# kiwicampus/multicamera_stitching

Hardware: AMD Instinct MI355X
Metric: stitched MPix/sec (4-cam 1080p rig) (higher is better)
Workload: dtype u8; 1 GPU; C2 rig: 4 x 1920x1080 BGR cameras, precomputed homographies, linear warpPerspective + 3-level multi-band blend (SURVEY.md 8 NS-1); blend=multiband, super_mode=False

## Files before the change

### multicamera_stitching_amd/_capi.py

```python
from __future__ import annotations

import ctypes
import os
import threading

import numpy as np

_HERE = os.path.dirname(os.path.abspath(__file__))
LIB_PATH = os.environ.get("MCS_LIBRARY", os.path.join(_HERE, "libmcs.so"))

MCS_OK = 0
MCS_E_INVALID = -1
MCS_E_HIP = -2
MCS_E_NOMEM = -3
MCS_E_SHAPE = -4
MCS_E_UNSUPPORTED = -5
MCS_INTER_NEAREST = 0
MCS_INTER_LINEAR = 1
MCS_BLEND_NONE = 0
MCS_BLEND_FEATHER = 1
MCS_BLEND_MULTIBAND = 2
MCS_BLEND_SEAM = 3
MCS_SEAM_DISTANCE = 0
MCS_SEAM_GRAPHCUT = 1
# ... 380 lines not shown

    @classmethod
    def warp(cls, M, src_w: int, src_h: int, dst_w: int, dst_h: int, channels: int,
             interp: int = MCS_INTER_LINEAR, device: int = 0):
        L = load()
        m = np.ascontiguousarray(np.asarray(M, np.float64).reshape(9))
        h = ctypes.c_void_p()
        check(L.mcs_plan_create_warp(m.ctypes.data_as(ctypes.c_void_p), int(src_w), int(src_h),
                                     int(dst_w), int(dst_h), int(channels), int(interp),
                                     int(device), ctypes.byref(h)))
        return cls(None, 0, 0, channels, interp, device, _handle=h)

    @classmethod
    def undistort(cls, K, dist, w: int, h: int, channels: int, device: int = 0):
        L = load()
        k = np.ascontiguousarray(np.asarray(K, np.float64).reshape(9))
        d = np.ascontiguousarray(np.asarray(dist if dist is not None else [], np.float64)
                                 .reshape(-1))
        hd = ctypes.c_void_p()
        check(L.mcs_plan_create_undistort(k.ctypes.data_as(ctypes.c_void_p),
                                          d.ctypes.data_as(ctypes.c_void_p) if d.size else None,
                                          int(d.size), int(w), int(h), int(channels),
                                          int(device), ctypes.byref(hd)))
        return cls(None, 0, 0, channels, MCS_INTER_LINEAR, device, _handle=hd)

    @property
    def handle(self):
        return self._h

    def close(self):
        if getattr(self, "_h", None) is not None and self._h.value:
            self._lib.mcs_plan_destroy(self._h)
            self._h = None

    def __del__(self):
        try:
            self.close()
        except Exception:
            pass

    def out_shape(self):
        if self.channels == 1:
            return (self.out_h, self.out_w)
        return (self.out_h, self.out_w, self.channels)

    def describe(self) -> dict:
        fd = self.flat
        n = fd.n_stages
        return {
            "n_stages": n,
            "out_w": fd.out_w, "out_h": fd.out_h, "channels": fd.channels,
            "off_x": [fd.st[j].off_x for j in range(n)] + [fd.cam0_off_x],
            "off_y": [fd.st[j].off_y for j in range(n)] + [fd.cam0_off_y],
            "rect": [list(fd.st[j].rect) for j in range(n)],
            "minv": [list(fd.st[j].minv) for j in range(n)],
            "bw0": [fd.st[j].bw0 for j in range(n)],
            "cam": [fd.st[j].cam for j in range(n)],
            "cam_w": [fd.cam_w[i] for i in range(fd.n_cams)],
            "cam_h": [fd.cam_h[i] for i in range(fd.n_cams)],
        }

    def stitch_host(self, cams, sizes=None) -> np.ndarray:
        cams = [np.ascontiguousarray(c, dtype=np.uint8) for c in cams]
        out = np.empty(self.out_shape(), np.uint8)
        ptrs = (ctypes.c_void_p * len(cams))(*[c.ctypes.data for c in cams])
        outp = out.ctypes.data_as(ctypes.c_void_p)
        fd = self.flat
        if sizes is None or all((w, h) == (fd.cam_w[i], fd.cam_h[i])
                                for i, (w, h) in enumerate(sizes)):
            check(self._lib.mcs_stitch_host(self._h, ptrs, outp))
        else:
            ws = (ctypes.c_int * len(sizes))(*[int(w) for w, _ in sizes])
            hs = (ctypes.c_int * len(sizes))(*[int(h) for _, h in sizes])
            check(self._lib.mcs_stitch_host_sized(self._h, ptrs, ws, hs, outp))
        return out

    def find_seams(self, cams=None, method: int = MCS_SEAM_GRAPHCUT, scale_log2: int = 2):
        if cams is None:
            check(self._lib.mcs_plan_find_seams(self._h, None, int(method), int(scale_log2)))
            return
        cams = [np.ascontiguousarray(c, dtype=np.uint8) for c in cams]
        ptrs = (ctypes.c_void_p * len(cams))(*[c.ctypes.data for c in cams])
        check(self._lib.mcs_plan_find_seams(self._h, ptrs, int(method), int(scale_log2)))

    def seam_labels(self):
        w, h = ctypes.c_int(), ctypes.c_int()
        check(self._lib.mcs_plan_seam_labels(self._h, None, ctypes.byref(w), ctypes.byref(h)))
        if w.value == 0:
            return None
        out = np.empty((h.value, w.value), np.uint8)
        check(self._lib.mcs_plan_seam_labels(self._h, out.ctypes.data_as(ctypes.c_void_p),
                                             ctypes.byref(w), ctypes.byref(h)))
        return out

    def seam_stats(self):
        st = np.zeros(5, np.int64)
        check(self._lib.mcs_plan_seam_stats(self._h, st.ctypes.data_as(ctypes.c_void_p)))
        return tuple(int(v) for v in st)

    def stitch_device(self, cam_ptrs, cam_frame_strides, out_ptr: int, out_pitch: int,
                      out_frame_stride: int, n_frames: int, stream: int = 0):
        n = len(cam_ptrs)
        ptrs = (ctypes.c_void_p * n)(*[int(p) for p in cam_ptrs])
        strides = (ctypes.c_int64 * n)(*[int(s) for s in cam_frame_strides])
        check(self._lib.mcs_stitch_device(self._h, ptrs, strides, ctypes.c_void_p(int(out_ptr)),
                                          int(out_pitch), int(out_frame_stride), int(n_frames),
                                          ctypes.c_void_p(int(stream))))

    def stitch_direct(self, cam_ptrs, cam_frame_strides, out_ptr: int, out_pitch: int,
                      out_frame_stride: int, n_frames: int, stream: int = 0):
        n = len(cam_ptrs)
        ptrs = (ctypes.c_void_p * n)(*[int(p) for p in cam_ptrs])
        strides = (ctypes.c_int64 * n)(*[int(s) for s in cam_frame_strides])
        check(self._lib.mcs_stitch_direct(self._h, ptrs, strides, ctypes.c_void_p(int(out_ptr)),
                                          int(out_pitch), int(out_frame_stride), int(n_frames),
                                          ctypes.c_void_p(int(stream))))

    def stitch_device_gained(self, cam_ptrs, cam_frame_strides, out_ptr: int, out_pitch: int,
                             out_frame_stride: int, n_frames: int, stream: int = 0):
        n = len(cam_ptrs)
        ptrs = (ctypes.c_void_p * n)(*[int(p) for p in cam_ptrs])
        strides = (ctypes.c_int64 * n)(*[int(s) for s in cam_frame_strides])
        check(self._lib.mcs_stitch_device_gained(
            self._h, ptrs, strides, ctypes.c_void_p(int(out_ptr)), int(out_pitch),
            int(out_frame_stride), int(n_frames), ctypes.c_void_p(int(stream))))

    def stitch_direct_gained(self, cam_ptrs, cam_frame_strides, out_ptr: int, out_pitch: int,
                             out_frame_stride: int, n_frames: int, stream: int = 0):
        n = len(cam_ptrs)
        ptrs = (ctypes.c_void_p * n)(*[int(p) for p in cam_ptrs])
        strides = (ctypes.c_int64 * n)(*[int(s) for s in cam_frame_strides])
        check(self._lib.mcs_stitch_direct_gained(
            self._h, ptrs, strides, ctypes.c_void_p(int(out_ptr)), int(out_pitch),
            int(out_frame_stride), int(n_frames), ctypes.c_void_p(int(stream))))

    def prepare(self, stream: int = 0):
        check(self._lib.mcs_plan_prepare(self._h, ctypes.c_void_p(int(stream))))

    def tile_tables(self):
        n = self._lib.mcs__plan_tile_tables(self._h, None, None, None, 0)
        if n < 0:
            check(n)
        tiles = (TileHdr * max(n, 1))()
        spans = np.zeros((n, TILE_MAX_JOBS), np.uint16)
        desc = np.zeros((n, TILE_W * TILE_H, TILE_DESC_WORDS), np.uint32)
        if n:
            rc = self._lib.mcs__plan_tile_tables(self._h, ctypes.byref(tiles), spans.ctypes.data,
                                                 desc.ctypes.data, n)
            if rc < 0:
                check(rc)
        return tiles, spans, desc

    def stats(self) -> dict:
        arr = (ctypes.c_int64 * 21)()
        check(self._lib.mcs_plan_stats(self._h, arr, 21))
        return {"prepared": bool(arr[0]), "tiles": arr[1], "lds_tiles": arr[2],
                "direct_tiles": arr[3], "table_bytes": arr[4], "blend": arr[5],
                "blend_tiles": arr[6], "mb_owners": arr[7], "mb_degraded_tiles": arr[8],
                "mb_bands": arr[9], "mb_bands_lds": arr[10], "big_tiles": arr[11],
                "mb_mixed_px": arr[12], "mb_r1_entries": arr[13],
                "dma_bytes_per_capture": arr[14], "box_bytes_per_capture": arr[15],
                "mb_sweep_strips": arr[16], "mb_sweep_px": arr[17],
                "mb_sweep_threads": arr[18], "mb_sweep_desc_rows": arr[19],
                "lens_cams": arr[20]}

    def set_blend(self, mode: int):
        check(self._lib.mcs_plan_set_blend(self._h, int(mode)))
        return self

    def set_lens(self, cam: int, K, dist=None):
        if K is None:
            check(self._lib.mcs_plan_set_lens(self._h, int(cam), None, None, 0))
            return self
        k, d = _lens_args(K, dist)
        check(self._lib.mcs_plan_set_lens(self._h, int(cam), k.ctypes.data_as(ctypes.c_void_p),
                                          d.ctypes.data_as(ctypes.c_void_p) if d.size else None,
                                          int(d.size)))
        return self

    def overlap_stats(self, cam_ptrs, cam_frame_strides, n_frames: int, step_log2: int = 2,
                      stream: int = 0):
        n = self.n_cams
        ptrs = (ctypes.c_void_p * n)(*[int(p) if p else None for p in cam_ptrs])
        strides = (ctypes.c_int64 * n)(*[int(s) for s in cam_frame_strides])
        N = np.zeros((n, n), np.int64)
        S = np.zeros((max(int(n_frames), 0), n, n), np.int64)
        check(self._lib.mcs_plan_overlap_stats(self._h, ptrs, strides, int(n_frames),
                                               int(step_log2), N.ctypes.data, S.ctypes.data,
                                               ctypes.c_void_p(int(stream))))
        return N, S

    def overlap_stats_host(self, cams, step_log2: int = 2):
        cams = [np.ascontiguousarray(c, dtype=np.uint8) for c in cams]
        ptrs = (ctypes.c_void_p * len(cams))(*[c.ctypes.data for c in cams])
        n = self.n_cams
        N = np.zeros((n, n), np.int64)
        S = np.zeros((n, n), np.int64)
        check(self._lib.mcs_plan_overlap_stats_host(self._h, ptrs, int(step_log2), N.ctypes.data,
                                                    S.ctypes.data))
        return N, S

    def set_gains(self, gains):
        if gains is None:
            check(self._lib.mcs_plan_set_gains(self._h, None))
            return self
        g = np.ascontiguousarray(np.asarray(gains, np.float64).reshape(-1))
        if g.size != self.n_cams:
            raise ValueError(f"{g.size} gains for a plan of {self.n_cams} cameras")
        check(self._lib.mcs_plan_set_gains(self._h, g.ctypes.data))
        return self

    def gains(self):
        q = np.zeros(self.n_cams, np.uint16)
        on = ctypes.c_int(0)
        check(self._lib.mcs_plan_gains(self._h, q.ctypes.data, ctypes.byref(on)))
        return q, bool(on.value)

    def footprint(self):
        arr = (ctypes.c_int64 * MCS_MAX_CAMS)()
        check(self._lib.mcs_plan_footprint(self._h, arr, MCS_MAX_CAMS))
        return [int(arr[i]) for i in range(self.n_cams)]


def resize_linear_device(src_ptr: int, src_w: int, src_h: int, dst_ptr: int, dst_w: int,
                         dst_h: int, channels: int, n_frames: int = 1, src_pitch: int = 0,
                         dst_pitch: int = 0, src_frame_stride: int = 0,
                         dst_frame_stride: int = 0, device: int = 0, stream: int = 0):
    L = load()
    check(L.mcs_resize_linear_device(
        src_ptr, src_w, src_h, src_pitch or src_w * channels, src_frame_stride, dst_ptr, dst_w,
        dst_h, dst_pitch or dst_w * channels, dst_frame_stride, channels, n_frames, device,
        stream or None))


def gain_solve(N, S, channels: int, alpha: float = 0.01, beta: float = 100.0) -> np.ndarray:
    N = np.ascontiguousarray(N, dtype=np.int64)
    S = np.ascontiguousarray(S, dtype=np.int64)
    n = N.shape[0]
    if N.shape != (n, n) or S.shape != (n, n):
        raise ValueError(f"N {N.shape} and S {S.shape} must both be (n_cams, n_cams)")
    g = np.ones(n, np.float64)
    check(load().mcs_gain_solve_host(n, N.ctypes.data, S.ctypes.data, int(channels),
                                     float(alpha), float(beta), g.ctypes.data))
    return g


def gain_apply_device(src_ptr: int, dst_ptr: int, nbytes: int, q: int, n_frames: int = 1,
                      src_frame_stride: int = 0, dst_frame_stride: int = 0, device: int = 0,
                      stream: int = 0):
    if not 0 <= int(q) <= 65535:
        raise ValueError(f"q {q} outside 0..65535")
    check(load().mcs_gain_apply_device(src_ptr, dst_ptr, int(nbytes), int(src_frame_stride),
                                       int(dst_frame_stride), int(n_frames), int(q), int(device),
                                       stream or None))


def match_hamming_knn2(query, train, device: int = 0):
    L = load()
    q = np.ascontiguousarray(query, dtype=np.uint8).reshape(-1, 32)
    t = np.ascontiguousarray(train, dtype=np.uint8).reshape(-1, 32)
    idx = np.empty((q.shape[0], 2), np.int32)
    dist = np.empty((q.shape[0], 2), np.int32)
    check(L.mcs_match_hamming_knn2_host(q.ctypes.data, q.shape[0], t.ctypes.data, t.shape[0],
                                        idx.ctypes.data, dist.ctypes.data, device))
    return idx, dist


def match_hamming_knn2_device(q_ptr: int, nq: int, t_ptr: int, nt: int, idx_ptr: int,
                              dist_ptr: int, device: int = 0, stream: int = 0):
    check(load().mcs_match_hamming_knn2(q_ptr, nq, t_ptr, nt, idx_ptr, dist_ptr, device,
                                        stream or None))


def homography_refine(src, dst, mask, H):
    L = load()
    src = np.ascontiguousarray(src, np.float32).reshape(-1, 2)
    dst = np.ascontiguousarray(dst, np.float32).reshape(-1, 2)
    m = np.ascontiguousarray(np.asarray(mask).reshape(-1), np.uint8)
    h = np.ascontiguousarray(np.asarray(H, np.float64).reshape(9)).copy()
    check(L.mcs_homography_refine_host(src.ctypes.data, dst.ctypes.data, src.shape[0],
                                       m.ctypes.data, h.ctypes.data))
    return h.reshape(3, 3)


def ransac_homography(src, dst, thresh: float, iters: int = 2000, seed: int = 0,
                      device: int = 0):
    L = load()
    src = np.ascontiguousarray(src, np.float32).reshape(-1, 2)
    dst = np.ascontiguousarray(dst, np.float32).reshape(-1, 2)
    n = src.shape[0]
    H = np.zeros(9, np.float64)
    mask = np.zeros(n, np.uint8)
    ninl = ctypes.c_int(0)
    check(L.mcs_ransac_homography_host(src.ctypes.data, dst.ctypes.data, n, float(thresh),
                                       int(iters), int(seed) & 0xffffffff, H.ctypes.data,
                                       mask.ctypes.data, ctypes.byref(ninl), device))
    return (H.reshape(3, 3) if ninl.value > 0 else None), mask.reshape(-1, 1)


class StreamPipeline:

    def __init__(self, plan: "Plan", depth: int = 3, use_graphs: bool = True):
        self._lib = load()
        self.plan = plan
        self.depth = depth
        h = ctypes.c_void_p()
        check(self._lib.mcs_stream_create(plan._h, depth, 1 if use_graphs else 0,
                                          ctypes.byref(h)))
        self._h = h

    def _check_frames(self, cams):
        C = self.plan.channels
        if len(cams) != self.plan.n_cams:
            raise ValueError(f"{len(cams)} frames for a plan of {self.plan.n_cams} cameras")
        out = []
        for i, (c, (h, w)) in enumerate(zip(cams, self.plan.cam_shapes)):
            c = np.asarray(c)
# ... 354 lines not shown
```

### multicamera_stitching_amd/build.py

```python
from __future__ import annotations

import hashlib
import os
import struct
import subprocess
import sys

HERE = os.path.dirname(os.path.abspath(__file__))
ROOT = os.path.dirname(HERE)
CSRC = os.path.join(HERE, "csrc")
LIB = os.path.join(HERE, "libmcs.so")
ARCH = os.environ.get("MCS_OFFLOAD_ARCH", "gfx950")
DEVICE = {"stitch": "mcs_kernels.hip", "features": "mcs_features.hip", "sweep": "mcs_sweep.hip"}
HSACO = os.path.join(HERE, f"mcs_kernels.{ARCH}.hsaco")
ROCM = os.environ.get("ROCM_PATH", "/opt/rocm")
HIPCC = os.environ.get("HIPCC", os.path.join(ROCM, "bin", "hipcc"))
CXX = os.environ.get("CXX", "g++")
HOST_SRC = ["mcs_plan.cpp", "hip_rt.cpp", "mcs_runtime.cpp", "mcs_capi.cpp", "mcs_prepare.cpp",
            "mcs_sweep_host.cpp", "mcs_launch.cpp", "mcs_features.cpp", "mcs_stream.cpp",
            "mcs_seam.cpp", "mcs_refine.cpp", "mcs_group.cpp", "mcs_rig.cpp", "mcs_chain.cpp",
            "mcs_gain.cpp"]
HEADERS = ["mcs_kparams.h", "mcs_dev.h", "mcs_fparams.h", "mcs_common.h", "hip_rt.h", "mcs_blend.h",
           "mcs_gain.h", "mcs_ransac_core.h",
           "mcs_orb_core.h", "mcs_orb_pattern.h", "mcs_feat_int.h", "mcs_lens_core.h",
           "mcs_plan_state.h"]
INC = ["-I" + os.path.join(ROOT, "include"), "-I" + CSRC]

DEVICE_FLAGS = [
    f"--offload-arch={ARCH}", "--offload-device-only", "--no-gpu-bundle-output",
    "-O3", "-std=c++17",
    "-ffp-contract=off", "-fno-fast-math", "-Wall",
    "-mllvm", "-instcombine-max-copied-from-constant-users=4096",
]
HOST_FLAGS = [
    "-O2", "-std=c++17", "-fPIC", "-shared", "-Wall", "-Wextra", "-Wno-unused-parameter",
    "-ffp-contract=off", "-fno-fast-math",
    "-D__HIP_PLATFORM_AMD__", "-I" + os.path.join(ROCM, "include"),
]


def _elf_sections(path: str) -> dict:
    with open(path, "rb") as f:
        b = f.read()
    if b[:4] != b"\x7fELF" or b[4] != 2 or b[5] != 1:
        raise ValueError(f"{path}: not an ELF64 little-endian object")
    shoff, = struct.unpack_from("<Q", b, 0x28)
    shentsize, shnum, shstrndx = struct.unpack_from("<HHH", b, 0x3A)
    hdrs = [struct.unpack_from("<IIQQQQIIQQ", b, shoff + i * shentsize) for i in range(shnum)]
    names = hdrs[shstrndx]
    strtab = b[names[4]:names[4] + names[5]]
    out = {}
    for h in hdrs:
        name = strtab[h[0]:strtab.index(b"\0", h[0])].decode()
        out[name] = b"" if h[1] == 8 else b[h[4]:h[4] + h[5]]
    return out


CODE_SECTIONS = (".text", ".rodata", ".note")


def code_id(paths) -> str:
    digest = hashlib.sha256()
    for p in paths:
        secs = _elf_sections(p)
        for name in CODE_SECTIONS:
            data = secs.get(name, b"")
            digest.update(name.encode() + struct.pack("<Q", len(data)) + data)
    return digest.hexdigest()[:16]


def _stale() -> bool:
    if not (os.path.exists(LIB) and os.path.exists(HSACO)):
        return True
    t = os.path.getmtime(LIB)
    deps = [os.path.join(CSRC, s) for s in [*DEVICE.values(), *HOST_SRC, *HEADERS]]
    deps += [os.path.join(ROOT, "include", "mcs.h"), __file__]
    return any(os.path.getmtime(d) > t for d in deps)


def _run(cmd, verbose):
    if verbose:
        print(" ".join(cmd), flush=True)
    subprocess.check_call(cmd)


def build(force: bool = False, verbose: bool = False, lib: str = None, defines=()) -> str:
    if lib is not None:
        return _build_to(lib, HSACO + "." + os.path.basename(lib), list(defines), verbose)
    if not force and not _stale():
        return LIB
    return _build_to(LIB, HSACO, [], verbose)


def _fresh(out: str, src: str) -> bool:
    if not os.path.exists(out):
        return False
    deps = [os.path.join(CSRC, src)] + [os.path.join(CSRC, h) for h in HEADERS]
    deps += [os.path.join(ROOT, "include", "mcs.h"), __file__]
    return all(os.path.getmtime(d) <= os.path.getmtime(out) for d in deps)


def _build_to(LIB: str, HSACO: str, defines, verbose: bool) -> str:
    objs = {}
    for name, src in DEVICE.items():
        out = HSACO if name == "stitch" else HSACO.replace("mcs_kernels", "mcs_" + name)
        if defines or not _fresh(out, src):
            _run([HIPCC, *DEVICE_FLAGS, *["-D" + d for d in defines], *INC, "-o", out + ".tmp",
                  os.path.join(CSRC, src)], verbose)
            os.replace(out + ".tmp", out)
        objs[name] = out
    build_id = code_id([objs[name] for name in sorted(objs)])
    blob = LIB + ".blob.S"
    with open(blob, "w") as f:
        f.write("    .section .rodata\n")
        for name, path in objs.items():
            f.write('    .balign 4096\n    .globl mcs_hsaco_%s_start\nmcs_hsaco_%s_start:\n'
                    '    .incbin "%s"\n    .byte 0\n' % (name, name, path))
        f.write('    .section .note.GNU-stack,"",@progbits\n')
    try:
        _run([CXX, *HOST_FLAGS, *["-D" + d for d in defines], f'-DMCS_BUILD_ID="{build_id}"',
              *INC, "-o", LIB + ".tmp",
              *[os.path.join(CSRC, s) for s in HOST_SRC], blob, "-ldl", "-lpthread"], verbose)
    finally:
        os.remove(blob)
    os.replace(LIB + ".tmp", LIB)
    return LIB


if __name__ == "__main__":
    print(build(force="--force" in sys.argv, verbose=True))
```

### multicamera_stitching_amd/csrc/mcs_blend.h

```cpp
#pragma once

namespace mcs {

template <int INTERP>
__device__ __forceinline__ void slot_xy(const KParams &P, int s, int x, int y, int &x32, int &y32,
                                        int &cam, int &w, int &h)
{
    int X, Y;
    if (s == 0) {
        cam = 0;
        w = P.cam0_w;
        h = P.cam0_h;
        if (!cam0_lensed(P)) {
            x32 = (x + P.cam0_offx) * 32;
            y32 = (y + P.cam0_offy) * 32;
            return;
        }
        cam0_lens_map<INTERP>(P, x, y, X, Y);
    } else {
        const KStage &S = P.st[s - 1];
        cam = S.cam;
        w = S.src_w;
        h = S.src_h;
        stage_map<INTERP>(P, S, x, y, X, Y);
// ... 73 lines not shown
    w = s == 0 ? P.cam0_w : P.st[s - 1].src_w;
    h = s == 0 ? P.cam0_h : P.st[s - 1].src_h;
}

__device__ __forceinline__ int refl(int i, int n)
{
    if (n == 1) return 0;
    while (i < 0 || i >= n) {
        if (i < 0) i = -i;
        if (i >= n) i = 2 * n - 2 - i;
    }
    return i;
}

template <int CN, int INTERP>
__device__ __forceinline__ void seam_sample(const KSeamArgs &a)
{
    const KParams &P = a.P;
    const int q = blockIdx.x * blockDim.x + threadIdx.x;
    if (q >= a.gw * a.gh) return;
    const int x = (q % a.gw) << a.k, y = (q / a.gw) << a.k;
    const int64_t np = (int64_t)a.gw * a.gh;
    const int o = blend_owner<INTERP>(P, x, y, nullptr);
    uint32_t cov = 0;
    for (int s = 0; s <= P.n_stages; s++) {
        int x32, y32, cam, w, h;
        slot_xy<INTERP>(P, s, x, y, x32, y32, cam, w, h);
        if (slot_dist(x32, y32, w, h) < 0) continue;
        cov |= 1u << cam;
        const uint8_t *fb = P.cams[cam];
        const uint32_t v = sample_replicate<CN>(fb, w, h, x32, y32);
        uint8_t *d = a.samples + ((int64_t)cam * np + q) * CN;
#pragma unroll
        for (int k = 0; k < CN; k++) d[k] = (uint8_t)(v >> (8 * k));
    }
    a.cov[q] = (uint16_t)cov;
    int ocam = kBlendNone;
    if (o != kBlendNone) {
        int c, w, h;
        slot_info(P, o, c, w, h);
        ocam = c;
    }
    a.label[q] = (uint8_t)ocam;
}

template <int INTERP>
__device__ __forceinline__ void blend_owner_tile(const KParams &P, uint8_t *owner_map,
                                                 uint32_t *info)
{
    __shared__ uint32_t s_own, s_feather;
    if (threadIdx.x == 0) s_own = s_feather = 0;
    __syncthreads();
    const int X0 = blockIdx.x * kBlendTileW, Y0 = blockIdx.y * kBlendTileH;
    uint32_t own = 0, fea = 0;
    for (int i = threadIdx.x; i < kMbTilePx; i += blockDim.x) {
        const int x = X0 + (i % kBlendTileW), y = Y0 + i / kBlendTileW;
        if (x >= P.out_w || y >= P.out_h) continue;
        uint32_t pm;
        const int o = blend_owner<INTERP>(P, x, y, &pm);
        owner_map[(int64_t)y * P.out_w + x] = (uint8_t)o;
        if (o != kBlendNone) own |= 1u << o;
        if (__popc(pm) >= 2) fea |= pm;
    }
    atomicOr(&s_own, own);
    atomicOr(&s_feather, fea);
    __syncthreads();
    if (threadIdx.x == 0) {
        const int t = blockIdx.y * gridDim.x + blockIdx.x;
        info[2 * t] = s_own;
        info[2 * t + 1] = s_feather;
    }
}

__device__ __forceinline__ void blend_classify(const KParams &P, int mode, const uint8_t *owner,
                                               const uint32_t *info, int *list, int *overflow,
                                               int *list2)
{
    __shared__ uint32_t s_mask;
    const int gx = (P.out_w + kBlendTileW - 1) / kBlendTileW;
    const int t = blockIdx.x, tx = t % gx, ty = t / gx;
    uint32_t mask;
    if (mode == MCS_BLEND_FEATHER) {
        mask = info[2 * t + 1];
    } else {
        if (threadIdx.x == 0) s_mask = 0;
        __syncthreads();
        const int x0 = max(tx * kBlendTileW - kBlendHalo, 0);
        const int x1 = min(tx * kBlendTileW + kBlendTileW + kBlendHalo, P.out_w);
        const int y0 = max(ty * kBlendTileH - kBlendHalo, 0);
        const int y1 = min(ty * kBlendTileH + kBlendTileH + kBlendHalo, P.out_h);
        const int rw = x1 - x0, n = rw * (y1 - y0);
        uint32_t m = 0;
        for (int i = threadIdx.x; i < n; i += blockDim.x) {
            const int o = owner[(int64_t)(y0 + i / rw) * P.out_w + x0 + i % rw];
            if (o != kBlendNone) m |= 1u << o;
        }
        atomicOr(&s_mask, m);
        __syncthreads();
        mask = s_mask;
        if (__popc(mask) < 2) mask = 0;
    }
    if (threadIdx.x == 0 && mode == MCS_BLEND_MULTIBAND && __popc(mask) > kBlendSlots) {
        atomicAdd(overflow, 1);
        const uint32_t fea = info[2 * t + 1];
        if (fea) {
            const int i = atomicAdd(&list2[0], 1);
            list2[1 + 2 * i] = t;
            list2[2 + 2 * i] = (int)fea;
        }
        return;
    }
    if (threadIdx.x == 0 && mask) {
        atomicMax(overflow + 1, __popc(mask));
        const int i = atomicAdd(&list[0], 1);
        list[1 + 2 * i] = t;
        list[2 + 2 * i] = (int)mask;
    }
}

template <int CN, int INTERP, bool GAIN = false>
__device__ __forceinline__ void feather_tile(const KBlendArgs &a)
{
    const KParams &P = a.P;
    const int gx = (P.out_w + kBlendTileW - 1) / kBlendTileW;
    const int t = a.list[1 + 2 * blockIdx.x];
    const uint32_t mask = (uint32_t)a.list[2 + 2 * blockIdx.x];
    const int X0 = (t % gx) * kBlendTileW, Y0 = (t / gx) * kBlendTileH, f = blockIdx.y;
    for (int i = threadIdx.x; i < kMbTilePx; i += blockDim.x) {
        const int x = X0 + (i % kBlendTileW), y = Y0 + i / kBlendTileW;
        if (x >= P.out_w || y >= P.out_h) continue;
        int den = 0, num[CN];
#pragma unroll
        for (int k = 0; k < CN; k++) num[k] = 0;
        for (uint32_t m = mask; m; m &= m - 1) {
            const int s = __ffs(m) - 1;
            int x32, y32, cam, w, h;
            slot_xy<INTERP>(P, s, x, y, x32, y32, cam, w, h);
            const int d = slot_dist(x32, y32, w, h);
            if (d <= 0) continue;
            const uint32_t v = sample_replicate<CN, GAIN>(
                P.cams[cam] + (int64_t)f * P.cam_fstride[cam], w, h, x32, y32,
                GAIN ? gain_q_of(P, cam) : 256u);
            den += d;
#pragma unroll
            for (int k = 0; k < CN; k++) num[k] += d * (int)((v >> (8 * k)) & 0xffu);
        }
        if (den == 0) continue;
        uint8_t *o = P.out + (int64_t)f * P.out_fstride + (int64_t)y * P.out_pitch + x * CN;
#pragma unroll
        for (int k = 0; k < CN; k++) o[k] = (uint8_t)((num[k] + den / 2) / den);
    }
}

constexpr int kMbO1 = 6, kMbO2 = 2, kMbOR = 1;
constexpr int kMbU = kMbUsedX * kMbUsedY;
constexpr int kMbFoot = 28672;
constexpr int kMbFootBufs = 1;
constexpr int kMbRS = kMbO1 - kMbOR;
__device__ __forceinline__ int mb_g1_at(int col, int row) { return row * kMbNRX + col; }
template <int CN>
__device__ __forceinline__ int mb_g2_at(int col, int row, int k)
{
    return (row * kMbN2X + col) * CN + k;
}

template <bool IN>
__device__ __forceinline__ void exp_taps(int x, int n, int *idx, int *wt)
{
    if ((x & 1) == 0) {
        idx[0] = IN ? x / 2 - 1 : refl(x / 2 - 1, n), wt[0] = 1;
        idx[1] = IN ? x / 2 : refl(x / 2, n), wt[1] = 6;
        idx[2] = IN ? x / 2 + 1 : refl(x / 2 + 1, n), wt[2] = 1;
        return;
    }
    idx[0] = IN ? (x - 1) / 2 : refl((x - 1) / 2, n), wt[0] = 4;
    idx[1] = IN ? (x + 1) / 2 : refl((x + 1) / 2, n), wt[1] = 4;
    idx[2] = idx[1], wt[2] = 0;
}

__device__ __forceinline__ int mb_cls(int x, int y) { return (x & 1) | ((y & 1) << 1); }

struct MbGeo {
    int W, H, w1, h1, w2, h2;
    int X0, Y0, RX, RY, X1, Y1, X2, Y2, XR, YR;
    bool interior;
};

__device__ __forceinline__ MbGeo mb_geo(const KParams &P, int t)
{
    MbGeo G;
    G.W = P.out_w;
    G.H = P.out_h;
    G.w1 = (G.W + 1) / 2, G.h1 = (G.H + 1) / 2, G.w2 = (G.w1 + 1) / 2, G.h2 = (G.h1 + 1) / 2;
    const int gx = (G.W + kBlendTileW - 1) / kBlendTileW;
    G.X0 = (t % gx) * kBlendTileW, G.Y0 = (t / gx) * kBlendTileH;
    G.RX = G.X0 - kBlendHalo, G.RY = G.Y0 - kBlendHalo;
    G.X1 = G.X0 / 2 - kMbO1, G.Y1 = G.Y0 / 2 - kMbO1;
    G.X2 = G.X0 / 4 - kMbO2, G.Y2 = G.Y0 / 4 - kMbO2;
    G.XR = G.X0 / 2 - kMbOR, G.YR = G.Y0 / 2 - kMbOR;
    G.interior = G.RX >= 0 && G.RY >= 0 && G.RX + kBlendTileW + 2 * kBlendHalo <= G.W &&
                 G.RY + kBlendTileH + 2 * kBlendHalo <= G.H;
    return G;
}

template <bool IN>
__device__ __forceinline__ int rf(int i, int n) { return IN ? i : refl(i, n); }
template <bool IN>
__device__ __forceinline__ int ix2(int c, int o, int n)
{
    return IN ? c - o : min(max(c - o, 0), n - 1);
}

struct MbSrc {
    int ya, yb, c;
    uint32_t meta;
};

template <int INTERP>
__device__ __forceinline__ MbSrc mb_src(const KParams &P, int s, int x, int y)
{
    int x32, y32, cam, w, h;
    slot_xy<INTERP>(P, s, x, y, x32, y32, cam, w, h);
    const int sx = x32 >> 5, sy = y32 >> 5;
    MbSrc r;
    r.c = w >= 2 ? min(max(sx, 0), w - 2) : 0;
    const bool a_hi = min(max(sx, 0), w - 1) > r.c;
    const bool b_hi = min(max(sx + 1, 0), w - 1) > r.c;
    const uint32_t fx = a_hi ? 32u : (b_hi ? (uint32_t)(x32 & 31) : 0u);
    r.ya = min(max(sy, 0), h - 1);
    r.yb = min(max(sy + 1, 0), h - 1);
    r.meta = fx | ((uint32_t)(y32 & 31) << 6);
    return r;
}

template <int CN>
__device__ __forceinline__ uint2 mb_desc(const MbSrc &q, int w, int h)
{
    const int64_t pitch = (int64_t)w * CN, fbytes = pitch * h;
    const int64_t oa = q.ya * pitch + (int64_t)q.c * CN, ob = oa + (q.yb > q.ya ? pitch : 0);
    const uint32_t d = (uint32_t)min(max(ob + 8 - fbytes, (int64_t)0), (int64_t)7);
    const int64_t e = fbytes - (ob - oa) - 12;
    int64_t o4 = oa & ~(int64_t)3;
    if (o4 > e) o4 = e & ~(int64_t)3;
    const uint32_t sh = (e >= 0 && oa - o4 <= 12 - 2 * CN) ? (uint32_t)(oa - o4) : 15u;
    return make_uint2((uint32_t)oa | (q.yb > q.ya ? 0x80000000u : 0u),
                      q.meta | (d << 12) | (sh << 15));
}

__device__ __forceinline__ uint32_t mad6_u32(uint32_t a, uint32_t b)
{
    uint32_t t, r;
    asm("v_lshl_add_u32 %0, %1, 1, %2" : "=v"(t) : "v"(a), "v"(b));
    asm("v_lshl_add_u32 %0, %1, 2, %2" : "=v"(r) : "v"(a), "v"(t));
    return r;
}

__device__ __forceinline__ uint2 mb_win_shift4(uint3 v, uint32_t sh)
{
    return make_uint2(__builtin_amdgcn_alignbyte(v.y, v.x, sh & 3u),
                      __builtin_amdgcn_alignbyte(v.z, v.y, sh & 3u));
}

template <int CN>
__device__ __forceinline__ uint2 mb_win_shift(uint3 v, uint32_t sh)
{
    const uint32_t s = sh & 3u;
    const uint32_t a = __builtin_amdgcn_alignbyte(v.y, v.x, s);
    const uint32_t b = __builtin_amdgcn_alignbyte(v.z, v.y, s);
    const uint32_t c = __builtin_amdgcn_alignbyte(0u, v.z, s);
    if (CN <= 2 && (sh & 8u)) return make_uint2(c, 0u);
    return (sh & 4u) ? make_uint2(b, c) : make_uint2(a, b);
}

struct MbFoot {
    int rmin, rows, cal, stride, e, fits, pad0, pad1;
};

__device__ __forceinline__ uint32_t mb_foot_off(const MbFoot &F, int row, int byte, int h)
{
    return (uint32_t)((row - F.rmin) * F.stride + byte - F.cal + (row == h - 1 ? F.e : 0));
}

__device__ __forceinline__ void mb_weights(uint32_t meta, uint32_t &wa, uint32_t &wb)
{
    const uint32_t fx = meta & 63u, fy = (meta >> 6) & 31u;
    const uint32_t wx = (32u - fx) | (fx << 16);
    wa = wx * ((32u - fy) << 5);
    wb = wx * (fy << 5);
}

__device__ __forceinline__ void mb_weights2(uint32_t meta, uint32_t &wa, uint32_t &wb)
{
    const uint32_t fx = meta & 63u, fy = (meta >> 6) & 31u;
    const uint32_t ya = (32u - fy) << 6, yb = fy << 6;
    wa = min((32u - fx) * ya, 65535u) | (min(fx * ya, 65535u) << 16);
    wb = min((32u - fx) * yb, 65535u) | (min(fx * yb, 65535u) << 16);
}

template <int CN, bool GAIN = false>
__device__ __forceinline__ uint32_t mb_tap(uint2 r0, uint2 r1, uint32_t wa, uint32_t wb, int k,
                                           uint32_t d, GainQ g = GainQ())
{
    typedef unsigned short us2 __attribute__((ext_vector_type(2)));
    const uint32_t sel = ((uint32_t)k | (0x0cu << 8) | ((uint32_t)(CN + k) << 16) | (0x0cu << 24)) +
                         d * 0x00010001u;
    uint32_t a0 = __builtin_amdgcn_perm(r0.y, r0.x, sel);
    uint32_t a1 = __builtin_amdgcn_perm(r1.y, r1.x, sel);
// ... 448 lines not shown
        } else {
            for (int i = tid; i < n_s; i += NT) {
                const uint64_t v = dsc[i];
                const uint32_t o = (uint32_t)v & 0x7fffffffu;
                const uint32_t ob = o + (((uint32_t)v >> 31) ? (uint32_t)pitch : 0u);
                const uint2 r0 = load8<2 * CN>(fb, o, fbytes), r1 = load8<2 * CN>(fb, ob, fbytes);
                uint32_t wa, wb, px = 0;
                mb_weights((uint32_t)(v >> 32), wa, wb);
#pragma unroll
                for (int k = 0; k < CN; k++) px |= mb_tap<CN, GAIN>(r0, r1, wa, wb, k, 0u, gq) << (8 * k);
                L.g0[(uint32_t)(v >> 48) & 0x1fffu] = px;
            }
        }
        __syncthreads();
        if (kMbFootBufs == 1 && staged && fl + 1 < fl1) stage(fl + 1, 0);
        const int64_t job = ((int64_t)bt * a.slots + j) * a.chunk + fl;
        uint2 *og1 = reinterpret_cast<uint2 *>(a.g1) + job * (kMbNRX * kMbNRY);
        int32_t *og2 = a.g2 + job * (kMbN2X * kMbN2Y * CN);
        if (G.interior) {
            {
                constexpr int IT = (kMbUsedY * kMbN1X + NT - 1) / NT;
                const int n = kMbUsedY * w1;
                uint2 res[IT];
#pragma unroll
                for (int q = 0; q < IT; q++) {
                    const int i = min(tid + q * NT, n - 1);
                    const int r = (int)(__umul24((unsigned)i, d1m) >> 16);
                    const int e = a1 + i - (int)__umul24((unsigned)r, (unsigned)w1);
                    const uint32_t *g = &L.g0[r * kMbUsedX + 2 * e];
                    uint32_t lo = 0, hi = 0;
#pragma unroll
                    for (int v = 0; v < 5; v++) {
                        const uint32_t t = g[v];
                        lo += (uint32_t)w5[v] * (t & 0x00ff00ffu);
                        hi += (uint32_t)w5[v] * ((t >> 8) & 0x00ff00ffu);
                    }
                    res[q] = make_uint2(lo, hi);
                }
#pragma unroll
                for (int q = 0; q < IT; q++) {
                    const int i = tid + q * NT;
                    const int r = (int)(__umul24((unsigned)i, d1m) >> 16);
                    L.hs[i < n ? r * kMbN1X + a1 + i - (int)__umul24((unsigned)r, (unsigned)w1)
                               : kMbUsedY * kMbN1X] = res[q];
                }
            }
            __syncthreads();
            {
                constexpr int IT = (kMbN1Y * kMbN1X + NT - 1) / NT;
                const int n = kMbN1Y * w1;
                uint2 res[IT];
#pragma unroll
                for (int q = 0; q < IT; q++) {
                    const int i = min(tid + q * NT, n - 1);
                    const int ey = (int)(__umul24((unsigned)i, d1m) >> 16);
                    const int ex = a1 + i - (int)__umul24((unsigned)ey, (unsigned)w1);
                    uint32_t lo = 0, hi = 0;
#pragma unroll
                    for (int u = 0; u < 5; u++) {
                        const uint2 t = L.hs[(2 * ey + u) * kMbN1X + ex];
                        lo += (uint32_t)w5[u] * t.x;
                        hi += (uint32_t)w5[u] * t.y;
                    }
                    res[q] = make_uint2(lo, hi);
                }
#pragma unroll
                for (int q = 0; q < IT; q++) {
                    const int i = tid + q * NT;
                    const int ey = (int)(__umul24((unsigned)i, d1m) >> 16);
                    L.g1[i < n ? ey * kMbN1X + a1 + i - (int)__umul24((unsigned)ey, (unsigned)w1)
                               : kMbN1X * kMbN1Y] = res[q];
                }
            }
            __syncthreads();
            for (int i = tid; i < kMbN1Y * w2; i += NT) {
                const int r = (int)(__umul24((unsigned)i, d2m) >> 16);
                const int e = a2 + i - (int)__umul24((unsigned)r, (unsigned)w2);
                int acc[4] = {0, 0, 0, 0};
#pragma unroll
                for (int v = 0; v < 5; v++) {
                    const uint2 t = L.g1[r * kMbN1X + 2 * e + v];
#pragma unroll
                    for (int k = 0; k < CN; k++) acc[k] += w5[v] * ch16(t, k);
                }
                L.hs2[r * kMbN2X + e] = make_int4(acc[0], acc[1], acc[2], acc[3]);
            }
            __syncthreads();
            for (int i = tid; i < kMbN2Y * w2; i += NT) {
                const int ey = (int)(__umul24((unsigned)i, d2m) >> 16);
                const int ex = a2 + i - (int)__umul24((unsigned)ey, (unsigned)w2);
                int acc[4] = {0, 0, 0, 0};
#pragma unroll
                for (int u = 0; u < 5; u++) {
                    const int4 t = L.hs2[(2 * ey + u) * kMbN2X + ex];
                    acc[0] += w5[u] * t.x;
                    acc[1] += w5[u] * t.y;
                    acc[2] += w5[u] * t.z;
                    acc[3] += w5[u] * t.w;
                }
#pragma unroll
                for (int k = 0; k < CN; k++) og2[mb_g2_at<CN>(ex, ey, k)] = acc[k];
            }
        } else {
            const int RX2 = G.RX + kMbFirst, RY2 = G.RY + kMbFirst;
            for (int e = tid; e < kMbN1X * kMbN1Y; e += NT) {
                const int qx = refl(G.X1 + e % kMbN1X, G.w1), qy = refl(G.Y1 + e / kMbN1X, G.h1);
                uint32_t lo = 0, hi = 0;
                for (int u = 0; u < 5; u++) {
                    const int cy = ix2<false>(refl(2 * qy + u - 2, G.H), RY2, kMbUsedY);
#pragma unroll
                    for (int v = 0; v < 5; v++) {
                        const int cx = ix2<false>(refl(2 * qx + v - 2, G.W), RX2, kMbUsedX);
                        const uint32_t t = L.g0[cy * kMbUsedX + cx], wt = w5[u] * w5[v];
                        lo += wt * (t & 0x00ff00ffu);
                        hi += wt * ((t >> 8) & 0x00ff00ffu);
                    }
                }
                L.g1[e] = make_uint2(lo, hi);
            }
            __syncthreads();
            for (int e = tid; e < kMbN2X * kMbN2Y; e += NT) {
                const int zx = refl(G.X2 + e % kMbN2X, G.w2), zy = refl(G.Y2 + e / kMbN2X, G.h2);
                int acc[4] = {0, 0, 0, 0};
                for (int u = 0; u < 5; u++) {
                    const int qy = ix2<false>(refl(2 * zy + u - 2, G.h1), G.Y1, kMbN1Y);
#pragma unroll
                    for (int v = 0; v < 5; v++) {
                        const int qx = ix2<false>(refl(2 * zx + v - 2, G.w1), G.X1, kMbN1X);
                        const uint2 t = L.g1[qy * kMbN1X + qx];
                        const int wt = w5[u] * w5[v];
#pragma unroll
                        for (int k = 0; k < CN; k++) acc[k] += wt * ch16(t, k);
                    }
                }
#pragma unroll
                for (int k = 0; k < CN; k++) og2[mb_g2_at<CN>(e % kMbN2X, e / kMbN2X, k)] = acc[k];
            }
        }
        for (int e = tid; e < kMbNRX * kMbNRY; e += NT)
            og1[mb_g1_at(e % kMbNRX, e / kMbNRX)] =
                L.g1[(e / kMbNRX + kMbRS) * kMbN1X + e % kMbNRX + kMbRS];
        __syncthreads();
    }
}

template <int CN, int INTERP>
__device__ __forceinline__ void mb_bdesc(const KMbBandArgs &a)
{
    const KParams &P = a.P;
    const MbBand B = a.bands[blockIdx.x];
    int cam, w, h;
    slot_info(P, B.slot, cam, w, h);
    const int y0 = B.row * kBlendTileH - kBlendHalo + kMbFirst;
    uint64_t *o = a.bdesc + (int64_t)blockIdx.x * kMbBandDescRows * kMbBandLanes;
    for (int i = threadIdx.x; i < kMbBandDescRows * kMbBandLanes; i += blockDim.x) {
        const int r = i / kMbBandLanes, l = i % kMbBandLanes;
        const int x = refl(B.c0 + l, P.out_w), y = refl(y0 + r, P.out_h);
        const uint2 v = mb_desc<CN>(mb_src<INTERP>(P, B.slot, x, y), w, h);
        o[i] = (uint64_t)v.x | ((uint64_t)v.y << 32);
    }
}

__device__ __forceinline__ uint32_t lane_next(uint32_t v)
{
    return (uint32_t)__builtin_amdgcn_update_dpp(0, (int)v, 0x130, 0xf, 0xf, true);
}
__device__ __forceinline__ uint32_t lane_prev(uint32_t v)
{
    return (uint32_t)__builtin_amdgcn_update_dpp(0, (int)v, 0x138, 0xf, 0xf, true);
}
__device__ __forceinline__ int lane_at(int v, int src4)
{
    return __builtin_amdgcn_ds_bpermute(src4, v);
}

template <int I, int N, class F>
__device__ __forceinline__ void static_for_(F &&f)
{
    if constexpr (I < N) {
        f(std::integral_constant<int, I>());
        static_for_<I + 1, N>(f);
    }
}
template <int N, class F>
__device__ __forceinline__ void static_for(F &&f) { static_for_<0, N>(f); }

template <int CN>
__device__ __forceinline__ void mb_store_ch(__attribute__((address_space(1))) uint8_t *p,
                                            const int (&v)[CN])
{
    typedef __attribute__((address_space(1))) int gi;
    typedef int i3 __attribute__((ext_vector_type(3), aligned(4)));
    typedef int i4 __attribute__((ext_vector_type(4), aligned(4)));
    if (CN == 3) {
        i3 t;
        t.x = v[0], t.y = v[CN > 1 ? 1 : 0], t.z = v[CN > 2 ? 2 : 0];
        *(__attribute__((address_space(1))) i3 *)p = t;
    } else if (CN == 4) {
        i4 t;
        t.x = v[0], t.y = v[CN > 1 ? 1 : 0], t.z = v[CN > 2 ? 2 : 0], t.w = v[CN > 3 ? 3 : 0];
        *(__attribute__((address_space(1))) i4 *)p = t;
    } else {
#pragma unroll
        for (int k = 0; k < CN; k++) ((gi *)p)[k] = v[k];
    }
}

struct MbTarget {
    int base[2], col[2];
};
static_assert(kBlendTileW == 32, "mb_bands: tile columns are found by shifts");

__device__ __forceinline__ void mb_target(const KMbBandArgs &a, int s, int row, int tx, int col,
                                          MbTarget &T, int k)
{
    T.base[k] = -1;
    T.col[k] = 0;
    if (tx < 0 || tx >= a.gxb) return;
    const int bt = a.tile_bt[row * a.gxb + tx];
    if (bt < 0) return;
    const uint32_t mask = (uint32_t)a.list[2 + 2 * bt];
    if (!((mask >> s) & 1u)) return;
    const int j = __popc(mask & ((1u << s) - 1u));
    T.base[k] = (bt * a.slots + j) * a.chunk;
    T.col[k] = col;
}

__device__ __forceinline__ bool xcd_unit(int nx, int ny, int &x, int &y)
{
    const int n = nx * ny, per = (n + 7) >> 3;
    const int u = (int)(blockIdx.x & 7) * per + (int)(blockIdx.x >> 3);
    if (u >= n) return false;
    x = u / ny;
    y = u - x * ny;
    return true;
}

template <int CN>
__device__ __forceinline__ void mb_buffer_store_ch(__amdgpu_buffer_rsrc_t rs, uint32_t off,
                                                   const int (&v)[CN])
{
    typedef unsigned int u2v __attribute__((ext_vector_type(2)));
    typedef unsigned int u3v __attribute__((ext_vector_type(3)));
    typedef unsigned int u4v __attribute__((ext_vector_type(4)));
    if constexpr (CN == 1) {
        __builtin_amdgcn_raw_buffer_store_b32((uint32_t)v[0], rs, off, 0, 0);
    } else if constexpr (CN == 2) {
        const u2v t = {(uint32_t)v[0], (uint32_t)v[CN > 1 ? 1 : 0]};
        __builtin_amdgcn_raw_buffer_store_b64(t, rs, off, 0, 0);
    } else if constexpr (CN == 3) {
        const u3v t = {(uint32_t)v[0], (uint32_t)v[CN > 1 ? 1 : 0], (uint32_t)v[CN > 2 ? 2 : 0]};
        __builtin_amdgcn_raw_buffer_store_b96(t, rs, off, 0, 0);
    } else {
        const u4v t = {(uint32_t)v[0], (uint32_t)v[CN > 1 ? 1 : 0], (uint32_t)v[CN > 2 ? 2 : 0],
                       (uint32_t)v[CN > 3 ? 3 : 0]};
        __builtin_amdgcn_raw_buffer_store_b128(t, rs, off, 0, 0);
    }
}

template <int FR>
constexpr int mb_lds_ops(int ph)
{
    return ((ph & 1) ? 2 * FR : 0) + (ph % 4 == 1 ? 2 * FR : 0) + (ph % 4 == 0 ? FR : 0) + 1;
}
template <int FR, int NL>
constexpr int mb_lds_wait(int ph, bool first)
{
    int d = 0, g = 1;
    for (int j = 1; j < NL; j++) d += mb_lds_ops<FR>((ph - j + 12) % 12);
    for (int j = 1; j < kMbLdsGLead; j++) g += mb_lds_ops<FR>((ph - j + 12) % 12);
    int w = d < g ? d : g;
    if (first) {
        int w0 = NL - 1 - ph;
        for (int j = 0; j < ph; j++) w0 += mb_lds_ops<FR>(j);
        w = w0 < w ? w0 : w;
    }
    return w > 63 ? 63 : w;
}

template <int CN, int FR, bool BR, int WM, bool GAIN = false>
__device__ __forceinline__ void mb_bands_body(const KMbBandArgs &a, int bi, lds_u8 *ring, int pr)
{
    constexpr bool AL = WM >= 1, LD = WM == 2;
    typedef __attribute__((address_space(1))) const uint8_t gu8;
    struct __attribute__((packed)) U2 {
        uint32_t x, y;
    };
    struct U3 {
        uint32_t x, y, z;
    };
    typedef __attribute__((address_space(1))) const U2 gu2;
    typedef __attribute__((address_space(1))) const U3 gu3;
    typedef std::conditional_t<AL, uint3, uint2> Win;
    typedef __attribute__((address_space(1))) uint2 g2u;
    const KParams &P = a.P;
    const int l = threadIdx.x;
    const MbBand B = a.bands[bi];
    const int fl0 = pr * FR;
    if (fl0 >= a.nf) return;
    int cam, w, h;
    slot_info(P, B.slot, cam, w, h);
    const GainQ gq = GAIN ? gain_pair(gain_q_of(P, cam)) : GainQ();
    const uint32_t pitch = (uint32_t)(w * CN);
    const gu8 *fb[FR];
#pragma unroll
    for (int i = 0; i < FR; i++)
        fb[i] = (const gu8 *)(P.cams[cam] +
                              (int64_t)(a.f0 + min(fl0 + i, a.nf - 1)) * P.cam_fstride[cam]);
    const int W = P.out_w, H = P.out_h;
    const int w1 = (W + 1) / 2, h1 = (H + 1) / 2, w2 = (w1 + 1) / 2, h2 = (h1 + 1) / 2;
    const int Y0 = B.row * kBlendTileH, Y1 = Y0 / 2 - kMbO1, Y2 = Y0 / 4 - kMbO2;
    const int x = B.c0 + l;
    MbTarget T1, T2;
    T1.base[0] = T1.base[1] = T2.base[0] = T2.base[1] = -1;
    T1.col[0] = T1.col[1] = T2.col[0] = T2.col[1] = 0;
    if ((l & 1) == 0 && l >= 2 && l <= 61 && x >= 0 && (x >> 1) < w1) {
        const int qx = x >> 1, tx = (qx + kMbOR) >> 4;
        mb_target(a, B.slot, B.row, tx, qx - (tx * (kBlendTileW / 2) - kMbOR), T1, 0);
        if (((qx + kMbOR) & 15) < kMbNRX - 16)
            mb_target(a, B.slot, B.row, tx - 1, qx - ((tx - 1) * (kBlendTileW / 2) - kMbOR), T1, 1);
    }
    if ((l & 3) == 0 && l >= 8 && l <= 56 && x >= 0 && (x >> 2) < w2) {
        const int z = x >> 2, tx = (z + kMbO2) >> 3;
        mb_target(a, B.slot, B.row, tx, z - (tx * (kBlendTileW / 4) - kMbO2), T2, 0);
        if (((z + kMbO2) & 7) < kMbN2X - 8)
            mb_target(a, B.slot, B.row, tx - 1, z - ((tx - 1) * (kBlendTileW / 4) - kMbO2), T2, 1);
    }
    int src[4];
#pragma unroll
    for (int t = 0; t < 4; t++) {
        int q = (x >> 1) + (t < 2 ? t - 2 : t - 1);
        if (BR && q >= w1) q = 2 * w1 - 2 - q;
        src[t] = min(max(2 * q - B.c0, 0), kMbBandLanes - 1) * 4;
    }
    uint32_t o1[2], o2[2];
#pragma unroll
    for (int k = 0; k < 2; k++) {
        o1[k] = T1.base[k] < 0 ? 0u : (uint32_t)((T1.base[k] + fl0) * (kMbNRX * kMbNRY) +
                                                 mb_g1_at(T1.col[k], 0)) * 8u;
        o2[k] = T2.base[k] < 0 ? 0u : (uint32_t)((T2.base[k] + fl0) * (kMbN2X * kMbN2Y * CN) +
                                                 mb_g2_at<CN>(T2.col[k], 0, 0)) * 4u;
    }
    typedef __attribute__((address_space(1))) uint8_t g8;
    g8 *const g1b = (g8 *)a.g1, *const g2b = (g8 *)a.g2;
    const uint64_t *dsc = a.bdesc + (int64_t)bi * kMbBandDescRows * kMbBandLanes + l;
    const int nst = min(FR, a.nf - fl0);
    uint32_t Vl[FR][3], Vh[FR][3];
    int V2[FR][3][CN];
    uint32_t hl[FR][BR ? 4 : 1], hh[FR][BR ? 4 : 1];
#pragma unroll
    for (int i = 0; i < FR; i++)
#pragma unroll
        for (int q = 0; q < 3; q++) {
            Vl[i][q] = Vh[i][q] = 0u;
#pragma unroll
            for (int k = 0; k < CN; k++) V2[i][q][k] = 0;
            if (q < (BR ? 4 : 1)) hl[i][q] = hh[i][q] = 0u;
        }
    if (BR) {
#pragma unroll
        for (int i = 0; i < FR; i++) hl[i][BR ? 3 : 0] = hh[i][BR ? 3 : 0] = 0u;
    }
    auto load_win = [&](uint64_t dv, Win (&r0)[FR], Win (&r1)[FR]) {
        if constexpr (LD) return;
        const uint32_t dx = (uint32_t)dv;
        const uint32_t d = AL ? (uint32_t)(dv >> 47) & 15u : (uint32_t)(dv >> 44) & 7u;
        uint32_t o = (dx & 0x7fffffffu) - d, ob = o + ((dx >> 31) ? pitch : 0u);
#pragma unroll
        for (int i = 0; i < FR; i++) {
            if constexpr (AL) {
                const U3 ra = *(const gu3 *)(fb[i] + o), rb = *(const gu3 *)(fb[i] + ob);
                r0[i] = make_uint3(ra.x, ra.y, ra.z);
                r1[i] = make_uint3(rb.x, rb.y, rb.z);
            } else {
                const U2 ra = *(const gu2 *)(fb[i] + o), rb = *(const gu2 *)(fb[i] + ob);
                r0[i] = make_uint2(ra.x, ra.y);
                r1[i] = make_uint2(rb.x, rb.y);
            }
        }
    };
    int pend1 = -1, pend2 = -1;
    uint32_t p1l[FR], p1h[FR];
    int p2[FR][CN];
    bool ok1 = false, ok2 = false;
    const __amdgpu_buffer_rsrc_t rs1 = __builtin_amdgcn_make_buffer_rsrc((void *)a.g1, 0, 0x7fffffff, 0x00020000);
    const __amdgpu_buffer_rsrc_t rs2 = __builtin_amdgcn_make_buffer_rsrc((void *)a.g2, 0, 0x7fffffff, 0x00020000);
    auto flush_ld = [&](auto PHc) {
        constexpr int ph = decltype(PHc)::value;
        constexpr uint32_t none = 0xfffffff0u;
        if constexpr (ph & 1) {
#pragma unroll
            for (int f = 0; f < FR; f++) {
                const uint32_t ro =
                    (uint32_t)(f * (kMbNRX * kMbNRY) + mb_g1_at(0, pend1 - kMbRS)) * 8u;
                typedef unsigned int u2v __attribute__((ext_vector_type(2)));
                const u2v v = {p1l[f], p1h[f]};
#pragma unroll
                for (int k = 0; k < 2; k++)
                    __builtin_amdgcn_raw_buffer_store_b64(
                        v, rs1, (ok1 && f < nst && T1.base[k] >= 0) ? o1[k] + ro : none, 0, 0);
            }
        }
        if constexpr (ph % 4 == 1) {
#pragma unroll
            for (int f = 0; f < FR; f++) {
                const uint32_t ro =
                    (uint32_t)(f * (kMbN2X * kMbN2Y * CN) + mb_g2_at<CN>(0, pend2, 0)) * 4u;
#pragma unroll
                for (int q = 0; q < 2; q++) {
                    const uint32_t off = (ok2 && f < nst && T2.base[q] >= 0) ? o2[q] + ro : none;
                    mb_buffer_store_ch<CN>(rs2, off, p2[f]);
                }
            }
        }
    };
    auto flush = [&]() {
        if (pend1 >= 0) {
#pragma unroll
            for (int f = 0; f < FR; f++) {
                if (f >= nst) break;
                const uint32_t ro =
                    (uint32_t)(f * (kMbNRX * kMbNRY) + mb_g1_at(0, pend1 - kMbRS)) * 8u;
#pragma unroll
                for (int k = 0; k < 2; k++)
                    if (T1.base[k] >= 0) *(g2u *)(g1b + (o1[k] + ro)) = make_uint2(p1l[f], p1h[f]);
            }
            pend1 = -1;
        }
        if (pend2 >= 0) {
#pragma unroll
            for (int f = 0; f < FR; f++) {
                if (f >= nst) break;
                const uint32_t ro =
                    (uint32_t)(f * (kMbN2X * kMbN2Y * CN) + mb_g2_at<CN>(0, pend2, 0)) * 4u;
#pragma unroll
                for (int q = 0; q < 2; q++)
                    if (T2.base[q] >= 0) mb_store_ch<CN>(g2b + (o2[q] + ro), p2[f]);
            }
            pend2 = -1;
        }
    };
    auto level1_done = [&](int i, auto P2c, auto M3c, int f, uint32_t vl, uint32_t vh) {
        constexpr int P2 = decltype(P2c)::value, M3 = decltype(M3c)::value;
        const uint32_t l1 = lane_prev(vl), l2 = lane_prev(l1), r1 = lane_next(vl),
                       r2 = lane_next(r1);
        const uint32_t h1_ = lane_prev(vh), h2_ = lane_prev(h1_), s1 = lane_next(vh),
                       s2 = lane_next(s1);
        uint32_t gl = mad6_u32(vl, (l2 + r2) + 4u * (l1 + r1));
        uint32_t gh = mad6_u32(vh, (h2_ + s2) + 4u * (h1_ + s1));
        const int qy = Y1 + i;
        if constexpr (LD) {
            pend1 = i;
            ok1 = qy >= 0 && qy < h1 && i >= kMbRS && i < kMbRS + kMbNRY;
            p1l[f] = gl;
            p1h[f] = gh;
        } else if (qy >= 0 && qy < h1 && i >= kMbRS && i < kMbRS + kMbNRY) {
            pend1 = i;
            p1l[f] = gl;
            p1h[f] = gh;
        }
        if (BR) {
            if (qy >= h1) {
                const bool d0 = qy == h1;
                gl = d0 ? hl[f][1] : hl[f][BR ? 3 : 0];
                gh = d0 ? hh[f][1] : hh[f][BR ? 3 : 0];
            }
#pragma unroll
            for (int q = (BR ? 3 : 0); q > 0; q--) hl[f][q] = hl[f][q - 1], hh[f][q] = hh[f][q - 1];
            hl[f][0] = gl, hh[f][0] = gh;
        }
        int g[CN];
#pragma unroll
        for (int k = 0; k < CN; k++)
            g[k] = (int)((((k & 1) ? gh : gl) >> ((k & 2) ? 16 : 0)) & 0xffffu);
        if (P2 == 0) {
#pragma unroll
            for (int k = 0; k < CN; k++) V2[f][(M3 + 1) % 3][k] += g[k];
            const int e = (i >> 1) - 2, zy = Y2 + e;
            if (LD) {
                pend2 = e;
                ok2 = e >= 0 && e < kMbN2Y && zy < h2;
            }
            if (LD || (e >= 0 && e < kMbN2Y && zy < h2)) {
                pend2 = e;
#pragma unroll
                for (int k = 0; k < CN; k++) {
                    const int v = V2[f][(M3 + 1) % 3][k];
                    p2[f][k] = (lane_at(v, src[0]) + lane_at(v, src[3])) +
                               4 * (lane_at(v, src[1]) + lane_at(v, src[2])) + 6 * v;
                }
            }
#pragma unroll
            for (int k = 0; k < CN; k++) {
                V2[f][(M3 + 2) % 3][k] += 6 * g[k];
                V2[f][M3][k] = g[k];
            }
        } else {
#pragma unroll
            for (int k = 0; k < CN; k++) {
                V2[f][(M3 + 2) % 3][k] += 4 * g[k];
                V2[f][M3][k] += 4 * g[k];
            }
        }
    };
    constexpr int NB = kMbBandBufs, A = kMbBandAhead, ND = kMbBandDescRing;
    uint64_t dq[ND];
    Win wq0[NB][FR], wq1[NB][FR];
    const uint32_t *grp = a.bgrp + (int64_t)bi * kMbLdsGroups * kMbBandLanes + l;
    typedef __attribute__((address_space(3))) const uint32_t lu32;
    lds_u8 *const dring = ring + kMbLdsDescOff;
    constexpr int NL = kMbLdsDescRing;
    const uint4 *d16 = a.bdesc16 + (int64_t)bi * kMbLdsDescRows * kMbBandLanes + l;
    auto issue_desc = [&](int row) {
        __builtin_amdgcn_global_load_lds(d16 + row * kMbBandLanes,
                                         dring + (row % NL) * kMbBandLanes * 16, 16, 0, 0);
        asm volatile("" ::: "memory");
    };
    __amdgpu_buffer_rsrc_t rsf[FR];
#pragma unroll
    for (int f = 0; f < FR; f++)
        rsf[f] = __builtin_amdgcn_make_buffer_rsrc((void *)fb[f], 0, (int)(pitch * (uint32_t)h),
                                                   0x00020000);
    auto issue_group = [&](int g, uint32_t off) {
#pragma unroll
        for (int f = 0; f < FR; f++)
            __builtin_amdgcn_raw_ptr_buffer_load_lds(
                rsf[f], ring + f * kMbLdsRingBytes + ((4 * g) % kMbLdsRows) * kMbLdsSpan, 16, off, 0,
                0, 0);
        asm volatile("" ::: "memory");
    };
    if constexpr (LD) {
        uint32_t go[kMbLdsLead / 4 + 1];
#pragma unroll
        for (int g = 0; g <= kMbLdsLead / 4; g++) go[g] = grp[g * kMbBandLanes];
#pragma unroll
        for (int g = 0; g <= kMbLdsLead / 4; g++) issue_group(g, go[g]);
#pragma unroll
        for (int i = 0; i < NL; i++) issue_desc(i);
    } else {
#pragma unroll
        for (int i = 0; i < ND; i++) dq[i] = dsc[i * kMbBandLanes];
    }
#pragma unroll
    for (int i = 0; i < A; i++) load_win(dq[i], wq0[i], wq1[i]);
    for (int r12 = 0; r12 < kMbBandRows; r12 += 12) {
        static_for<12>([&](auto PHc) {
            constexpr int ph = decltype(PHc)::value;
            const int r = r12 + ph;
            constexpr int b0 = ph % NB, bA = (ph + A) % NB, d0 = ph % ND, dA = (ph + A) % ND;
            uint32_t wa, wb, meta, dxr;
            if constexpr (LD) {
                if (ph < NL && r12 == 0)
                    asm volatile("s_waitcnt vmcnt(%0)" ::"n"(mb_lds_wait<FR, NL>(ph, true)) : "memory");
                else
                    asm volatile("s_waitcnt vmcnt(%0)" ::"n"(mb_lds_wait<FR, NL>(ph, false)) : "memory");
                const lu32 *dd = (const lu32 *)(dring + (ph % NL) * kMbBandLanes * 16 + l * 16);
                dxr = dd[0];
                wa = dd[1];
                wb = dd[3];
                meta = 0u;
            } else {
                dxr = (uint32_t)dq[d0];
                meta = (uint32_t)(dq[d0] >> 32);
                mb_weights2(meta, wa, wb);
            }
            const uint32_t dd = AL ? 0u : (meta >> 12) & 7u;
            uint32_t pls[FR], phs[FR];
#pragma unroll
            for (int f = 0; f < FR; f++) {
                uint2 r0, r1;
                if constexpr (LD) {
                    const uint32_t dx = dxr, sh = (dx >> 14) & 3u;
                    const lu32 *pa = (const lu32 *)(ring + f * kMbLdsRingBytes + (dx & 0x3fffu));
                    const lu32 *pb = (const lu32 *)(ring + f * kMbLdsRingBytes + (dx >> 16));
                    r0 = mb_win_shift4(make_uint3(pa[0], pa[1], pa[2]), sh);
                    r1 = mb_win_shift4(make_uint3(pb[0], pb[1], pb[2]), sh);
                } else if constexpr (AL) {
                    const uint32_t sh = (meta >> 15) & 15u;
                    r0 = mb_win_shift<CN>(wq0[b0][f], sh);
                    r1 = mb_win_shift<CN>(wq1[b0][f], sh);
                } else {
                    r0 = wq0[b0][f];
                    r1 = wq1[b0][f];
                }
                uint32_t t[4];
#pragma unroll
                for (int c = 0; c < 4; c++) t[c] = c < CN ? mb_tap2<CN, GAIN>(r0, r1, wa, wb, c, dd, gq) : 0u;
                if constexpr (CN >= 3) pls[f] = __builtin_amdgcn_perm(t[2], t[0], 0x0c060c02u);
                else pls[f] = (t[0] >> 16) & 0xffu;
                if constexpr (CN >= 4) phs[f] = __builtin_amdgcn_perm(t[3], t[1], 0x0c060c02u);
                else if constexpr (CN == 2 || CN == 3) phs[f] = (t[1] >> 16) & 0xffu;
                else phs[f] = 0u;
            }
            if constexpr (LD) flush_ld(PHc);
            else flush();
            load_win(dq[dA], wq0[bA], wq1[bA]);
            if constexpr (LD) {
                asm volatile("s_waitcnt lgkmcnt(0)" ::: "memory");
                if constexpr (ph % 4 == 0) {
                    const lu32 *dd = (const lu32 *)(dring + (ph % NL) * kMbBandLanes * 16 + l * 16);
                    issue_group(r / 4 + kMbLdsLead / 4 + 1, dd[2]);
                }
                issue_desc(r + NL);
            } else {
                dq[d0] = dsc[(r + ND) * kMbBandLanes];
            }
            constexpr int K3 = (ph / 2) % 3;
            constexpr int q = ph / 2 - 2, P2 = q & 1, M3 = ((q - P2) / 2 + 3) % 3;
            const int k = r >> 1;
#pragma unroll
            for (int f = 0; f < FR; f++) {
                const uint32_t pl = pls[f], ph_ = phs[f];
                if ((ph & 1) == 0) {
                    Vl[f][(K3 + 1) % 3] += pl;
                    Vh[f][(K3 + 1) % 3] += ph_;
                    level1_done(k - 2, std::integral_constant<int, P2>(),
                                std::integral_constant<int, M3>(), f, Vl[f][(K3 + 1) % 3],
                                Vh[f][(K3 + 1) % 3]);
                    Vl[f][(K3 + 2) % 3] += __umul24(pl, 6u);
                    Vh[f][(K3 + 2) % 3] += __umul24(ph_, 6u);
                    Vl[f][K3] = pl;
                    Vh[f][K3] = ph_;
                } else {
                    Vl[f][(K3 + 2) % 3] += 4u * pl;
                    Vh[f][(K3 + 2) % 3] += 4u * ph_;
                    Vl[f][K3] += 4u * pl;
                    Vh[f][K3] += 4u * ph_;
                }
            }
        });
    }
    if constexpr (!LD) flush();
}

template <int CN, int FR, bool BR, bool AL, bool GAIN = false>
__device__ __forceinline__ void mb_bands(const KMbBandArgs &a, int bi, lds_u8 *ring, int pr)
{
    if constexpr (AL) {
        const int lds = __builtin_amdgcn_readfirstlane(a.bands[bi].pad_) & 1;
        if (lds) mb_bands_body<CN, FR, BR, 2, GAIN>(a, bi, ring, pr);
        else mb_bands_body<CN, FR, BR, 1, GAIN>(a, bi, ring, pr);
    } else {
        mb_bands_body<CN, FR, BR, 0, GAIN>(a, bi, ring, pr);
    }
}

template <int CN, int S>
struct MbBlLds {
    uint2 g1[S][kMbNRX * kMbNRY];
    int32_t g2[S][CN][kMbN2X * kMbN2Y];
    double b2[CN][kMbN2X * kMbN2Y];
    double r1[CN][kMbNRX * kMbNRY];
};

constexpr int kMbPQ = kMbTilePx / kMbBlThreads;
template <int CN>
struct MbPix {
    int i[kMbPQ];
    int own[kMbPQ];
    uint32_t v[kMbPQ];
};

template <int CN, int S, bool IN>
__device__ __forceinline__ void mb_blend_tile(const KMbArgs &a, const MbGeo &G, MbBlLds<CN, S> &L,
                                              const MbPix<CN> &px, uint32_t mask, int ns, int f,
                                              int bt)
{
    const KParams &P = a.P;
    const int tid = threadIdx.x, nt = blockDim.x;
    const int32_t *tab = a.tab + (int64_t)bt * mb_tab_words(a.slots);
    const int32_t *t_m1 = tab, *t_m2 = tab + a.slots * kMbNRX * kMbNRY;
    const int32_t *t_d1 = t_m2 + a.slots * kMbN2X * kMbN2Y, *t_d2 = t_d1 + kMbNRX * kMbNRY;
    auto i2 = [&](int cx, int cy) {
        return (int)__umul24((unsigned)ix2<IN>(cy, G.Y2, kMbN2Y), kMbN2X) + ix2<IN>(cx, G.X2, kMbN2X);
    };
    auto ir = [&](int cx, int cy) {
        return (int)__umul24((unsigned)ix2<IN>(cy, G.YR, kMbNRY), kMbNRX) + ix2<IN>(cx, G.XR, kMbNRX);
    };
    const int n_r1 = t_d2[kMbN2X * kMbN2Y + 1];
    const uint16_t *t_r1 =
        reinterpret_cast<const uint16_t *>(t_d2 + kMbN2X * kMbN2Y + kMbTabCounts) + kMbTilePx;
    for (int e = tid; e < kMbN2X * kMbN2Y; e += nt) {
        double num[CN];
#pragma unroll
        for (int k = 0; k < CN; k++) num[k] = 0.0;
        for (int j = 0; j < ns; j++) {
            const double m = (double)t_m2[__umul24((unsigned)j, kMbN2X * kMbN2Y) + e];
#pragma unroll
            for (int k = 0; k < CN; k++) num[k] += m * (double)L.g2[j][k][e];
        }
        const int den = t_d2[e];
#pragma unroll
        for (int k = 0; k < CN; k++)
            L.b2[k][e] = den ? num[k] / ((double)den * 65536.0) : 0.0;
    }
    __syncthreads();
    for (int l = tid; l < n_r1; l += nt) {
        const int e = t_r1[l];
        const int ey = div_small<kMbNRX>(e), ex = e - (int)__umul24((unsigned)ey, kMbNRX);
        const int qx = rf<IN>(G.XR + ex, G.w1), qy = rf<IN>(G.YR + ey, G.h1);
        int iy[3], wy[3], ix[3], wx[3];
        exp_taps<IN>(qy, G.h2, iy, wy);
        exp_taps<IN>(qx, G.w2, ix, wx);
        const bool y3 = wy[2] != 0, x3 = wx[2] != 0;
        int tp[9], tw[9];
#pragma unroll
        for (int u = 0; u < 3; u++)
#pragma unroll
            for (int v = 0; v < 3; v++) {
                tp[3 * u + v] = i2(ix[v], iy[u]);
                tw[3 * u + v] = wy[u] * wx[v];
            }
        const int p1 = ir(qx, qy);
        double num[CN];
#pragma unroll
        for (int k = 0; k < CN; k++) num[k] = 0.0;
        for (int j = 0; j < ns; j++) {
            int e2[CN];
#pragma unroll
            for (int k = 0; k < CN; k++) e2[k] = 0;
#pragma unroll
            for (int t = 0; t < 9; t++) {
                if ((t >= 6 && !y3) || (t % 3 == 2 && !x3)) continue;
#pragma unroll
                for (int k = 0; k < CN; k++)
                    e2[k] += (int)__umul24((unsigned)tw[t], (unsigned)L.g2[j][k][tp[t]]);
            }
            const uint2 g1 = L.g1[j][p1];
            const double m = (double)t_m1[__umul24((unsigned)j, kMbNRX * kMbNRY) + p1];
#pragma unroll
            for (int k = 0; k < CN; k++) num[k] += m * (double)(16384 * ch16(g1, k) - e2[k]);
        }
        const int den = t_d1[p1];
        double acc[CN];
#pragma unroll
        for (int k = 0; k < CN; k++) acc[k] = 0.0;
#pragma unroll
        for (int t = 0; t < 9; t++) {
            if ((t >= 6 && !y3) || (t % 3 == 2 && !x3)) continue;
            const double wt = (double)tw[t];
#pragma unroll
            for (int k = 0; k < CN; k++) acc[k] += wt * L.b2[k][tp[t]];
        }
#pragma unroll
        for (int k = 0; k < CN; k++) {
            const double b1 = den ? num[k] / ((double)den * 4194304.0) : 0.0;
            L.r1[k][e] = b1 + acc[k] / 64.0;
        }
    }
    __syncthreads();
#pragma unroll
    for (int q = 0; q < kMbPQ; q++) {
        const int i = px.i[q];
        if (i < 0) continue;
        const int x = G.X0 + (i % kBlendTileW), y = G.Y0 + i / kBlendTileW;
        typedef __attribute__((address_space(1))) uint8_t gu8;
        gu8 *po = (gu8 *)(P.out + (int64_t)f * P.out_fstride + (int64_t)y * P.out_pitch + x * CN);
        const int o = px.own[q];
        if (o == kBlendNone) {
#pragma unroll
            for (int k = 0; k < CN; k++) po[k] = 0;
            continue;
        }
        const int s = __popc(mask & ((1u << o) - 1u));
        int iy[3], wy[3], ix[3], wx[3];
        exp_taps<IN>(y, G.h1, iy, wy);
        exp_taps<IN>(x, G.w1, ix, wx);
        int e1[CN];
        double acc[CN];
#pragma unroll
        for (int k = 0; k < CN; k++) e1[k] = 0, acc[k] = 0.0;
#pragma unroll
        for (int u = 0; u < 3; u++) {
            if (u == 2 && wy[2] == 0) break;
#pragma unroll
            for (int v = 0; v < 3; v++) {
                if (v == 2 && wx[2] == 0) break;
                const int p = ir(ix[v], iy[u]), wt = wy[u] * wx[v];
                const uint2 g1 = L.g1[s][p];
                const double wd = (double)wt;
#pragma unroll
                for (int k = 0; k < CN; k++) {
                    e1[k] += wt * ch16(g1, k);
                    acc[k] += wd * L.r1[k][p];
                }
            }
        }
#pragma unroll
        for (int k = 0; k < CN; k++) {
            const int l0 = 16384 * (int)((px.v[q] >> (8 * k)) & 0xffu) - e1[k];
            const double r0 = (double)l0 / 16384.0 + acc[k] / 64.0;
            const double vf = floor(r0 + 0.5);
            po[k] = (uint8_t)(vf < 0.0 ? 0.0 : (vf > 255.0 ? 255.0 : vf));
        }
    }
}

template <int CN, int S>
__device__ __forceinline__ void mb_blend(const KMbArgs &a, MbBlLds<CN, S> &L)
{
    typedef __attribute__((address_space(1))) const uint8_t cgu8;
    typedef __attribute__((address_space(1))) const uint2 cgu2;
    typedef __attribute__((address_space(1))) const int32_t cgi32;
    const KParams &P = a.P;
    int ux, fl;
    if (!xcd_unit(a.n_list, a.nf, ux, fl)) return;
    const int bt = a.list0 + ux, tid = threadIdx.x;
    const uint32_t mask = (uint32_t)a.list[2 + 2 * bt];
    const int ns = __popc(mask), f = a.f0 + fl;
    const MbGeo G = mb_geo(P, a.list[1 + 2 * bt]);
    MbPix<CN> px;
    int n_px;
    {
        const cgi32 *tc = (const cgi32 *)a.tab + (int64_t)bt * mb_tab_words(a.slots) +
                          a.slots * (kMbNRX * kMbNRY + kMbN2X * kMbN2Y) + kMbNRX * kMbNRY +
                          kMbN2X * kMbN2Y;
        typedef __attribute__((address_space(1))) const uint16_t cgu16;
        n_px = tc[0];
        const cgu16 *lp = (const cgu16 *)(tc + kMbTabCounts);
#pragma unroll
        for (int q = 0; q < kMbPQ; q++) {
            const int l = tid + q * kMbBlThreads;
            px.i[q] = l < n_px ? (int)lp[l] : -1;
        }
    }
    if (n_px == 0) return;
#pragma unroll
    for (int q = 0; q < kMbPQ; q++) {
        const int i = px.i[q];
        const int x = G.X0 + (i % kBlendTileW), y = G.Y0 + i / kBlendTileW;
        px.own[q] = kBlendNone;
        px.v[q] = 0;
        if (i >= 0) {
            px.own[q] = ((cgu8 *)a.owner)[(int64_t)y * G.W + x];
            const cgu8 *po = (const cgu8 *)(P.out + (int64_t)f * P.out_fstride +
                                            (int64_t)y * P.out_pitch + x * CN);
#pragma unroll
            for (int k = 0; k < CN; k++) px.v[q] |= (uint32_t)po[k] << (8 * k);
        }
    }
    constexpr int N1 = (kMbNRX * kMbNRY + kMbBlThreads - 1) / kMbBlThreads;
    constexpr int N2 = (kMbN2X * kMbN2Y * CN + kMbBlThreads - 1) / kMbBlThreads;
    uint2 r1[S][N1];
    int32_t r2[S][N2];
#pragma unroll
    for (int j = 0; j < S; j++) {
        if (j >= ns) break;
        const int64_t job = ((int64_t)bt * a.slots + j) * a.chunk + fl;
        const cgu2 *s1 = (const cgu2 *)a.g1 + job * (kMbNRX * kMbNRY);
        const cgi32 *s2 = (const cgi32 *)a.g2 + job * (kMbN2X * kMbN2Y * CN);
#pragma unroll
        for (int q = 0; q < N1; q++)
            r1[j][q] = s1[min(tid + q * kMbBlThreads, kMbNRX * kMbNRY - 1)];
#pragma unroll
        for (int q = 0; q < N2; q++)
            r2[j][q] = s2[min(tid + q * kMbBlThreads, kMbN2X * kMbN2Y * CN - 1)];
    }
#pragma unroll
    for (int j = 0; j < S; j++) {
        if (j >= ns) break;
#pragma unroll
        for (int q = 0; q < N1; q++)
            if (tid + q * kMbBlThreads < kMbNRX * kMbNRY) L.g1[j][tid + q * kMbBlThreads] = r1[j][q];
#pragma unroll
        for (int q = 0; q < N2; q++) {
            const int e = tid + q * kMbBlThreads;
            if (e < kMbN2X * kMbN2Y * CN) L.g2[j][e % CN][e / CN] = r2[j][q];
        }
    }
    __syncthreads();
    if (G.interior) mb_blend_tile<CN, S, true>(a, G, L, px, mask, ns, f, bt);
    else mb_blend_tile<CN, S, false>(a, G, L, px, mask, ns, f, bt);
}

}
```

### multicamera_stitching_amd/csrc/mcs_capi.cpp

```cpp
#include <cmath>
#include <cstdlib>
#include <cstring>
#include <new>
#include <vector>

#include "mcs_common.h"
#include "mcs_plan_state.h"

int mcs::plan_device(const mcs_plan *plan) { return plan ? plan->device : 0; }

#define MCS_VERSION_STRING "mcs 0.1.0 (gfx950 code object, HIP module launch)"

using namespace mcs::host;
using mcs::DeviceGuard;
using mcs::kMaxDevices;

namespace mcs {
namespace host {

int ensure_stream(const Api *A, mcs_plan *p)
{
    if (!p->stream) HIP_TRY(A->hipStreamCreateWithFlags(&p->stream, hipStreamNonBlocking));
    return MCS_OK;
}
// ... 679 lines not shown
    if (rc == MCS_OK) rc = ensure_host_buffers(A, p);
    if (rc == MCS_OK) rc = upload_plan_tables(A, p, p->stream);
    const Kernels *k = nullptr;
    if (rc == MCS_OK) rc = kernels(A, p->device, &k);
    if (rc) return rc;
    const int C = p->fd.channels, n = p->fd.n_cams;
    for (int i = 0; i < n; i++) {
        if (!cams[i]) return mcs::fail(MCS_E_INVALID, "NULL cams[%d]", i);
        HIP_TRY(A->hipMemcpyAsync(p->d_cams[i], cams[i],
                                  (size_t)p->fd.cam_w[i] * p->fd.cam_h[i] * C,
                                  hipMemcpyHostToDevice, p->stream));
    }
    const int kk = scale_log2;
    const int gw = (p->fd.out_w + (1 << kk) - 1) >> kk, gh = (p->fd.out_h + (1 << kk) - 1) >> kk;
    const size_t np = (size_t)gw * gh;
    mcs::KSeamArgs a;
    memset(&a, 0, sizeof(a));
    a.P = p->kp;
    for (int i = 0; i < n; i++) {
        a.P.cams[i] = p->d_cams[i];
        a.P.cam_fstride[i] = 0;
    }
    a.gw = gw;
    a.gh = gh;
    a.k = kk;
    std::vector<uint8_t> lab(np), smp;
    std::vector<uint16_t> cov(np);
    hipError_t e = A->hipMalloc((void **)&a.label, np);
    if (e == hipSuccess) e = A->hipMalloc((void **)&a.cov, np * sizeof(uint16_t));
    if (e == hipSuccess) e = A->hipMalloc((void **)&a.samples, np * C * n);
    if (e == hipSuccess) e = A->hipMemsetAsync(a.samples, 0, np * C * n, p->stream);
    if (e == hipSuccess) {
        rc = launch_args(A, k->seam_sample[C][p->fd.interp], (unsigned)((np + 255) / 256), 1,
                         256, 1, &a, sizeof(a), p->stream);
        if (rc) e = hipErrorLaunchFailure;
    }
    static const bool host_flow =
        getenv("MCS_SEAM_FLOW") && !strcmp(getenv("MCS_SEAM_FLOW"), "host");
    if (e == hipSuccess)
        e = A->hipMemcpyAsync(cov.data(), a.cov, np * 2, hipMemcpyDeviceToHost, p->stream);
    if (host_flow) {
        if (e == hipSuccess)
            e = A->hipMemcpyAsync(lab.data(), a.label, np, hipMemcpyDeviceToHost, p->stream);
        smp.resize(np * C * n);
        if (e == hipSuccess)
            e = A->hipMemcpyAsync(smp.data(), a.samples, np * C * n, hipMemcpyDeviceToHost,
                                  p->stream);
    }
    if (e == hipSuccess) e = A->hipStreamSynchronize(p->stream);
    if (e == hipSuccess && rc == MCS_OK) {
        if (host_flow) {
            rc = mcs::seam_graphcut(n, gw, gh, lab.data(), cov.data(), smp.data(), C);
            if (rc == MCS_OK)
                e = A->hipMemcpyAsync(a.label, lab.data(), np, hipMemcpyHostToDevice, p->stream);
        } else {
            rc = mcs::seam_graphcut_device(p->device, p->stream, n, gw, gh, a.label, a.cov,
                                           a.samples, C, cov.data(), p->seam_stats);
            if (rc == MCS_OK)
                e = A->hipMemcpyAsync(lab.data(), a.label, np, hipMemcpyDeviceToHost, p->stream);
        }
        if (e == hipSuccess) e = A->hipStreamSynchronize(p->stream);
    }
    for (void *q : {(void *)a.cov, (void *)a.samples})
        if (q) (void)A->hipFree(q);
    if (rc || e != hipSuccess) {
        if (a.label) (void)A->hipFree(a.label);
        if (rc) return rc;
        return mcs::fail(MCS_E_HIP, "seam finding: %s", A->hipGetErrorString(e));
    }
    p->d_seam = a.label;
    p->seam_lab.swap(lab);
    p->seam_w = gw;
    p->seam_h = gh;
    p->seam_k = kk;
    p->kp.seam_hint = p->d_seam;
    p->kp.seam_w = gw;
    p->kp.seam_shift = kk;
    return MCS_OK;
}

int mcs_seam_graphcut_host(int n_cams, int gw, int gh, uint8_t *labels, const uint16_t *cover,
                           const uint8_t *samples, int channels)
{
    mcs::clear_error();
    if (!labels || !cover || !samples) return mcs::fail(MCS_E_INVALID, "NULL input");
    if (n_cams < 1 || n_cams > 16 || gw < 1 || gh < 1 || channels < 1 || channels > 4 ||
        (int64_t)gw * gh > (int64_t)1 << 28)
        return mcs::fail(MCS_E_INVALID, "n_cams %d, grid %dx%d, channels %d", n_cams, gw, gh,
                         channels);
    return mcs::seam_graphcut(n_cams, gw, gh, labels, cover, samples, channels);
}

int mcs_seam_graphcut_device(int n_cams, int gw, int gh, uint8_t *labels, const uint16_t *cover,
                             const uint8_t *samples, int channels, int device, int64_t *stats)
{
    mcs::clear_error();
    if (!labels || !cover || !samples) return mcs::fail(MCS_E_INVALID, "NULL input");
    if (n_cams < 1 || n_cams > 16 || gw < 1 || gh < 1 || channels < 1 || channels > 4 ||
        (int64_t)gw * gh > (int64_t)1 << 28)
        return mcs::fail(MCS_E_INVALID, "n_cams %d, grid %dx%d, channels %d", n_cams, gw, gh,
                         channels);
    const Api *A = mcs::rt::api();
    if (!A) return MCS_E_HIP;
    DeviceGuard g(A, device);
    if (g.err != hipSuccess)
        return mcs::fail(MCS_E_HIP, "hipSetDevice(%d): %s", device, A->hipGetErrorString(g.err));
    const size_t np = (size_t)gw * gh, sb = np * n_cams * channels;
    uint8_t *buf = nullptr;
    hipStream_t s = nullptr;
    HIP_TRY(A->hipStreamCreateWithFlags(&s, hipStreamNonBlocking));
    hipError_t e = A->hipMalloc((void **)&buf, np * 3 + sb + 16);
    uint8_t *d_lab = buf, *d_smp = buf + np * 3 + 16;
    uint16_t *d_cov = reinterpret_cast<uint16_t *>(buf + ((np + 7) & ~(size_t)7));
    if (e == hipSuccess) e = A->hipMemcpyAsync(d_lab, labels, np, hipMemcpyHostToDevice, s);
    if (e == hipSuccess) e = A->hipMemcpyAsync(d_cov, cover, np * 2, hipMemcpyHostToDevice, s);
    if (e == hipSuccess) e = A->hipMemcpyAsync(d_smp, samples, sb, hipMemcpyHostToDevice, s);
    int rc = MCS_OK;
    if (e == hipSuccess)
        rc = mcs::seam_graphcut_device(device, s, n_cams, gw, gh, d_lab, d_cov, d_smp, channels,
                                       cover, stats);
    if (e == hipSuccess && rc == MCS_OK)
        e = A->hipMemcpyAsync(labels, d_lab, np, hipMemcpyDeviceToHost, s);
    if (e == hipSuccess) e = A->hipStreamSynchronize(s);
    (void)A->hipStreamSynchronize(s);
    if (buf) (void)A->hipFree(buf);
    (void)A->hipStreamDestroy(s);
    if (rc) return rc;
    if (e != hipSuccess) return mcs::fail(MCS_E_HIP, "seam graph cut: %s", A->hipGetErrorString(e));
    return MCS_OK;
}

int mcs_plan_seam_stats(const mcs_plan *p, int64_t *stats)
{
    if (!p || !stats) return mcs::fail(MCS_E_INVALID, "NULL plan/stats");
    for (int j = 0; j < 5; j++) stats[j] = p->seam_stats[j];
    return MCS_OK;
}

int mcs_plan_seam_labels(const mcs_plan *p, uint8_t *out, int *w, int *h)
{
    if (!p) return mcs::fail(MCS_E_INVALID, "NULL plan");
    if (w) *w = p->seam_w;
    if (h) *h = p->seam_h;
    if (out && !p->seam_lab.empty()) memcpy(out, p->seam_lab.data(), p->seam_lab.size());
    return MCS_OK;
}

int mcs_plan_stats(const mcs_plan *p, int64_t *stats, int n)
{
    if (!p || !stats) return mcs::fail(MCS_E_INVALID, "NULL plan/stats");
    const int64_t tiles = (int64_t)p->gx * p->gy;
    int lens_cams = 0;
    for (int c = 0; c < MCS_MAX_CAMS; c++) lens_cams += (p->kp.lens_mask >> c) & 1u;
    const int64_t v[21] = {p->t.prepared ? 1 : 0, tiles, tiles - p->t.n_fallback, p->t.n_fallback,
                           tiles * (int64_t)(sizeof(mcs::TileHdr) +
                                             mcs::kTilePx * (mcs::kDescWords + 1) * 4),
                           p->blend, p->t.n_blend, p->t.mb_slots, p->t.n_degraded, p->t.n_bands,
                           p->t.n_bands_lds, p->t.n_big, p->t.mb_mixed_px, p->t.mb_r1,
                           p->t.dma_bytes, p->t.box_bytes, p->t.n_strips, p->t.sw_px,
                           (int64_t)mcs::kSwCols * p->t.sw_jb, p->t.sw_desc_rows, lens_cams};
    for (int i = 0; i < n; i++) stats[i] = i < 21 ? v[i] : 0;
    return MCS_OK;
}

int mcs_plan_footprint(mcs_plan *p, int64_t *touched_px, int n_cams)
{
    if (!p || !touched_px) return mcs::fail(MCS_E_INVALID, "NULL plan/touched_px");
    if (n_cams < p->fd.n_cams)
        return mcs::fail(MCS_E_INVALID, "n_cams %d < %d", n_cams, p->fd.n_cams);
    const Api *A = mcs::rt::api();
    if (!A) return MCS_E_HIP;
    DeviceGuard g(A, p->device);
    if (g.err != hipSuccess)
        return mcs::fail(MCS_E_HIP, "hipSetDevice(%d): %s", p->device, A->hipGetErrorString(g.err));
    int rc = ensure_stream(A, p);
    if (rc) return rc;
    const Kernels *k = nullptr;
    rc = kernels(A, p->device, &k);
    if (rc) return rc;
    rc = upload_plan_tables(A, p, p->stream);
    if (rc) return rc;
    const int n = p->fd.n_cams;
    uint8_t *masks[MCS_MAX_CAMS] = {};
    uint8_t **d_masks = nullptr;
    unsigned long long *d_counts = nullptr;
    unsigned long long counts[MCS_MAX_CAMS] = {};
    hipError_t e = hipSuccess;
    for (int i = 0; i < n && e == hipSuccess; i++) {
        const size_t bytes = ((size_t)p->fd.cam_w[i] * p->fd.cam_h[i] + 3) / 4 * 4;
        e = A->hipMalloc((void **)&masks[i], bytes > 0 ? bytes : 4);
        if (e == hipSuccess) e = A->hipMemsetAsync(masks[i], 0, bytes > 0 ? bytes : 4, p->stream);
    }
    if (e == hipSuccess) e = A->hipMalloc((void **)&d_masks, sizeof(masks));
    if (e == hipSuccess) e = A->hipMalloc((void **)&d_counts, sizeof(counts));
    if (e == hipSuccess)
        e = A->hipMemcpyAsync(d_masks, masks, sizeof(masks), hipMemcpyHostToDevice, p->stream);
    if (e == hipSuccess) e = A->hipMemsetAsync(d_counts, 0, sizeof(counts), p->stream);
    if (e == hipSuccess && p->fd.out_w > 0 && p->fd.out_h > 0) {
        mcs::KFootprintArgs args;
        args.P = p->kp;
        args.masks = d_masks;
        args.counts = d_counts;
        rc = launch_args(A, k->footprint[p->fd.interp], (p->fd.out_w + 255) / 256, p->fd.out_h,
                         256, 1, &args, sizeof(args), p->stream);
    }
    if (rc) e = hipErrorLaunchFailure;
    if (e == hipSuccess)
        e = A->hipMemcpyAsync(counts, d_counts, sizeof(counts), hipMemcpyDeviceToHost, p->stream);
    if (e == hipSuccess) e = A->hipStreamSynchronize(p->stream);
    for (int i = 0; i < n; i++)
        if (masks[i]) (void)A->hipFree(masks[i]);
    if (d_masks) (void)A->hipFree(d_masks);
    if (d_counts) (void)A->hipFree(d_counts);
    if (rc) return rc;
    if (e != hipSuccess) return mcs::fail(MCS_E_HIP, "footprint: %s", A->hipGetErrorString(e));
    for (int i = 0; i < n_cams; i++) touched_px[i] = i < n ? (int64_t)counts[i] : 0;
    return MCS_OK;
}

}

extern "C" int mcs__plan_tile_tables(const mcs_plan *p, void *tiles_out, uint16_t *spans_out,
                                     uint32_t *desc_out, int max_tiles)
{
    mcs::clear_error();
    if (!p) return mcs::fail(MCS_E_INVALID, "NULL plan");
    if (!p->t.prepared) return mcs::fail(MCS_E_INVALID, "the plan is not prepared");
    const Api *A = mcs::rt::api();
    if (!A) return MCS_E_HIP;
    const size_t tiles = (size_t)p->gx * p->gy;
    if (!tiles_out || !spans_out || !desc_out || (size_t)std::max(max_tiles, 0) < tiles ||
        tiles == 0)
        return (int)tiles;
    DeviceGuard g(A, p->device);
    if (g.err != hipSuccess)
        return mcs::fail(MCS_E_HIP, "hipSetDevice(%d): %s", p->device, A->hipGetErrorString(g.err));
    HIP_TRY(A->hipMemcpyAsync(tiles_out, p->t.d_tiles, tiles * sizeof(mcs::TileHdr),
                              hipMemcpyDeviceToHost, nullptr));
    HIP_TRY(A->hipMemcpyAsync(spans_out, p->t.d_spans,
                              tiles * mcs::kMaxTileJobs * sizeof(uint16_t), hipMemcpyDeviceToHost,
                              nullptr));
    HIP_TRY(A->hipMemcpyAsync(desc_out, p->t.d_desc,
                              tiles * mcs::kTilePx * mcs::kDescWords * sizeof(uint32_t),
                              hipMemcpyDeviceToHost, nullptr));
    HIP_TRY(A->hipStreamSynchronize(nullptr));
    return (int)tiles;
}
```

### multicamera_stitching_amd/csrc/mcs_kparams.h

```cpp
#pragma once

#include <stdint.h>

#include "mcs.h"

namespace mcs {

struct KStage {
    double m[9];
    int rx0, ry0, rx1, ry1;
    int offx, offy;
    int bw0;
    int bw_shift;
    int cam;
    int src_w, src_h;
    int kind;
    double f, cx, cy;
};

constexpr int kStageHomography = 0;
constexpr int kStageCylinder = 1;
constexpr int kStageTable = 2;

struct KParams {
    int n_stages;
    int out_w, out_h;
    int cam0_offx, cam0_offy;
    int cam0_w, cam0_h;
    int blend;
    const double *cyl_tab;
    const uint8_t *seam_hint;
    int seam_w, seam_shift;
    const int32_t *map_tab;
    const uint8_t *skip;
    const uint8_t *cams[MCS_MAX_CAMS];
    int64_t cam_fstride[MCS_MAX_CAMS];
    uint8_t *out;
    int64_t out_pitch;
    int64_t out_fstride;
    const uint8_t *base;
    int cam_w[MCS_MAX_CAMS], cam_h[MCS_MAX_CAMS];
    KStage st[MCS_MAX_STAGES];
    const double *lens_tab;
    uint32_t lens_mask;
    int lens_pad_;
    uint16_t gain_q[MCS_MAX_CAMS];
};

struct KFootprintArgs {
    KParams P;
    uint8_t *const *masks;
    unsigned long long *counts;
};

#ifndef MCS_ROWS_PER_WAVE
#define MCS_ROWS_PER_WAVE 2
#endif
constexpr int kPx = 4;
constexpr int kWave = 64;
constexpr int kWavesPerBlock = 8;
constexpr int kRowsPerWave = MCS_ROWS_PER_WAVE;
constexpr int kLanesPerRow = kWave / kRowsPerWave;
constexpr int kTileW = kPx * kLanesPerRow;
constexpr int kTileH = kWavesPerBlock * kRowsPerWave;

constexpr int kTileCams = 4;
constexpr int kTilePx = kTileW * kTileH;
constexpr int kDescWords = 3;

constexpr uint32_t kCwLastRow1 = 1u << 28;
constexpr uint32_t kCwZero = 1u << 29;
constexpr uint32_t kCwFull = 1u << 30;
constexpr uint32_t kCwOneRow = 1u << 31;
constexpr uint32_t kCwSkip = 0xffffffffu;
struct TileHdr {
    int fits;
    int ncam, njobs, ring, buf_bytes;
    int cam[kTileCams], rmin[kTileCams], cal[kTileCams], stride[kTileCams], base[kTileCams];
    int jobstart[kTileCams + 1];
    int last_shift;
    int pad_;
};
static_assert(sizeof(TileHdr) == 128, "TileHdr layout");

constexpr int kMaxTileJobs = 128;
struct KPrepareArgs {
    KParams P;
    TileHdr *tiles;
    uint32_t *desc;
    uint32_t *desc4;
    int *fallback;
    int *big;
    uint16_t *spans;
};
struct KStreamArgs {
    KParams P;
    const TileHdr *tiles;
    const uint32_t *desc;
    const uint32_t *desc4;
    const uint16_t *spans;
    int n_frames;
    int parts;
    const int *order;
    int n_order;
    int pad2_;
};
struct KDirectArgs {
    KParams P;
    const int *fallback;
    int n_frames;
    int pad_;
};

struct KResizeArgs {
    const uint8_t *src;
    uint8_t *dst;
    int64_t src_pitch, src_fstride, dst_pitch, dst_fstride;
    double scale_x, scale_y;
    int sw, sh, dw, dh;
    int n_frames;
    int area2x;
};
constexpr int kResizeBlock = 256;

#ifndef MCS_BLEND_TILE_H
#define MCS_BLEND_TILE_H 64
#endif
constexpr int kBlendTileW = 32;
constexpr int kBlendTileH = MCS_BLEND_TILE_H;
constexpr int kBlendHalo = 16;
constexpr int kBlendSlots = 8;
constexpr int kBlendNone = 255;
constexpr int kMbPrepThreads = 256;
#ifndef MCS_MB_LV_THREADS
#define MCS_MB_LV_THREADS 512
#endif
constexpr int kMbLvThreads = MCS_MB_LV_THREADS;
#ifndef MCS_MB_LV_FRAMES
#define MCS_MB_LV_FRAMES 8
#endif
constexpr int kMbLvFrames = MCS_MB_LV_FRAMES;
#ifndef MCS_MB_BL_THREADS
#define MCS_MB_BL_THREADS 256
#endif
constexpr int kMbBlThreads = MCS_MB_BL_THREADS;
constexpr int64_t kMbScratchBytes = 1ll << 30;
constexpr int kMbUsedX = kBlendTileW + 25, kMbUsedY = kBlendTileH + 25;
constexpr int kMbFirst = 2;
constexpr int kMbN1X = kBlendTileW / 2 + 11, kMbN1Y = kBlendTileH / 2 + 11;
constexpr int kMbN2X = kBlendTileW / 4 + 4, kMbN2Y = kBlendTileH / 4 + 4;
constexpr int kMbNRX = kBlendTileW / 2 + 2, kMbNRY = kBlendTileH / 2 + 2;
constexpr int kMbTilePx = kBlendTileW * kBlendTileH;
constexpr int kMbTabRanges = 8;
constexpr int kMbTabCounts = kMbTabRanges + 4 * kBlendSlots;
constexpr int kMbTabLists = kMbTabCounts + kMbTilePx / 2 + (kMbNRX * kMbNRY + 1) / 2;
constexpr int mb_tab_words(int slots)
{
    return slots * (kMbNRX * kMbNRY + kMbN2X * kMbN2Y) + kMbNRX * kMbNRY + kMbN2X * kMbN2Y +
           kMbTabLists;
}
struct KBlendPrepArgs {
    KParams P;
    uint8_t *owner;
    uint32_t *info;
    int *list;
    int *overflow;
    int *list2;
    int mode, pad_;
};
struct KMbArgs {
    KParams P;
    const uint8_t *owner;
    const int *list;
    uint64_t *desc;
    int32_t *tab;
    int32_t *foot;
    uint16_t *g1;
    int32_t *g2;
    int slots;
    int chunk;
    int f0, nf;
    int list0;
    int n_list;
};

struct MbBand {
    int slot, row, c0, pad_;
};
constexpr int kMbBandLanes = 64;
constexpr int kMbBandRows = (kMbUsedY + 11) / 12 * 12;
#ifndef MCS_MB_BAND_AHEAD
#define MCS_MB_BAND_AHEAD 2
#endif
constexpr int kMbBandAhead = MCS_MB_BAND_AHEAD;
constexpr int kMbBandBufs = kMbBandAhead + 1;
static_assert(12 % kMbBandBufs == 0, "band pass: buffers must divide the 12-row body");
#ifndef MCS_MB_DESC_RING
#define MCS_MB_DESC_RING 3
#endif
constexpr int kMbBandDescRing = MCS_MB_DESC_RING;
static_assert(12 % kMbBandDescRing == 0 && kMbBandDescRing >= kMbBandBufs,
              "band pass: descriptor ring must divide the 12-row body and hold the window rows");
constexpr int kMbBandDescRows = kMbBandRows + kMbBandDescRing;
constexpr int kMbBandStride = 52;
#ifndef MCS_MB_BAND_FRAMES
#define MCS_MB_BAND_FRAMES 2
#endif
constexpr int kMbBandFrames = MCS_MB_BAND_FRAMES;
#define MCS_STR_(x) #x
#define MCS_STR(x) MCS_STR_(x)
#ifndef MCS_MB_LDS_DESC
#define MCS_MB_LDS_DESC 3
#endif
#ifndef MCS_MB_LDS_GLEAD
#define MCS_MB_LDS_GLEAD 3
#endif
constexpr int kMbLdsSpan = 256;
#ifndef MCS_MB_LDS_ROWS
#define MCS_MB_LDS_ROWS 16
#endif
#ifndef MCS_MB_LDS_LEAD
#define MCS_MB_LDS_LEAD 4
#endif
constexpr int kMbLdsRows = MCS_MB_LDS_ROWS;
constexpr int kMbLdsLead = MCS_MB_LDS_LEAD;
constexpr int kMbLdsGLead = MCS_MB_LDS_GLEAD;
constexpr int kMbLdsRingBytes = kMbLdsRows * kMbLdsSpan;
static_assert(kMbLdsRingBytes <= (1 << 14), "LDS band ring: offsets must fit the 14-bit field");
constexpr int kMbLdsDescRing = MCS_MB_LDS_DESC;
constexpr int kMbLdsDescRows = kMbBandRows + kMbLdsDescRing;
constexpr int kMbLdsDescOff = kMbBandFrames * kMbLdsRingBytes;
constexpr int kMbLdsBytes = kMbLdsDescOff + kMbLdsDescRing * kMbBandLanes * 16 + 16;
static_assert(12 % kMbLdsDescRing == 0 && kMbLdsGLead >= 1 && kMbLdsGLead <= kMbLdsDescRing,
              "LDS band ring: descriptor ring divides the 12-row body; groups led by <= its rows");
constexpr int kMbLdsGroups = kMbBandRows / 4 + kMbLdsLead / 4 + 3;
static_assert(kMbLdsRows % 4 == 0 && kMbLdsLead % 4 == 0 && kMbLdsRows / 4 > kMbLdsLead / 4 + 1,
              "LDS band ring: whole groups, the prologue's groups never evicted by the loop's first");
struct KMbBandArgs {
    KParams P;
    const int *list;
    const int *tile_bt;
    const MbBand *bands;
    uint64_t *bdesc;
    uint16_t *g1;
    int32_t *g2;
    const uint32_t *bgrp;
    const uint4 *bdesc16;
    int slots, chunk, f0, nf;
    int gxb;
    int band0;
    int n_in;
    int band1;
    int nb;
};
struct KBlendArgs {
    KParams P;
    const uint8_t *owner;
    const int *list;
    int n_frames, pad_;
};

constexpr int kSwCols = 128;
constexpr int kSwMaxOwners = 4;
constexpr int kSwMargin = 16;
constexpr int kSwValid = 100;
constexpr int kSwLead = 16;
constexpr int kSwDescPad = 12;
constexpr int kSwNG0 = 24, kSwNG1 = 10, kSwNG2 = 4, kSwNB2 = 4, kSwNR1 = 4;
constexpr int kSwMaxR1 = 64, kSwMaxB2 = 32;
struct MbStrip {
    int c0;
    int r0;
    int nsteps;
    int ya, yb;
    int ns;
    int reg;
    int dsc;
    int e1lo, e1n, z2lo, z2n;
    int slot[kSwMaxOwners];
};
static_assert(sizeof(MbStrip) == 64, "MbStrip layout");
struct KMbSweepArgs {
    KParams P;
    const MbStrip *strips;
    uint64_t *sdesc;
    const int *region;
    const uint8_t *owner;
    int n_strips, f0, nf, pad_;
};

constexpr int kDirectFrames = 4;
#ifndef MCS_JOBS_PER_WAVE
#define MCS_JOBS_PER_WAVE 8
#endif
constexpr int kJobsPerWave = MCS_JOBS_PER_WAVE;
constexpr int kLdsSlack = 16;
constexpr int kMaxRing = 6;
#ifndef MCS_STREAM_LDS
#define MCS_STREAM_LDS 40960
#endif
constexpr int lds_stream_bytes(int cn) { return cn >= 3 ? MCS_STREAM_LDS : 40960; }
constexpr int lds_ring_bytes(int cn) { return lds_stream_bytes(cn) - (int)sizeof(TileHdr); }
constexpr int kBigJobsPerWave = 16;
static_assert(kBigJobsPerWave * kWavesPerBlock <= kMaxTileJobs, "row spans per tile");
constexpr int kBigStreamLds = 120 * 1024;
constexpr int big_ring_bytes() { return kBigStreamLds - (int)sizeof(TileHdr); }
constexpr int lds_row_pitch(int bytes) { return (bytes + 127) & ~127; }


struct KSeamArgs {
    KParams P;
    uint8_t *label;
    uint16_t *cov;
    uint8_t *samples;
    int gw, gh, k, pad_;
};

constexpr int kOvSegs = MCS_MAX_CAMS * MCS_MAX_CAMS;
constexpr int kOvPrepThreads = 256;
struct KOverlapPrepArgs {
    KParams P;
    uint32_t *count;
    uint32_t *cursor;
    const int64_t *seg_off;
    uint8_t *table;
    int gw, gh, k, mode;
};
constexpr int kOvSumThreads = 256;
constexpr int kOvLaneEntries = 8;
constexpr int kOvUnitEntries = kOvSumThreads * kOvLaneEntries;
constexpr int kOvFrames = 4;
struct OvUnit {
    int64_t off;
    int cam_a, cam_b;
    int n;
    int pad_;
};
static_assert(sizeof(OvUnit) == 24, "OvUnit layout");
struct KOverlapSumArgs {
    const uint8_t *cams[MCS_MAX_CAMS];
    int64_t cam_fstride[MCS_MAX_CAMS];
    int cam_w[MCS_MAX_CAMS], cam_h[MCS_MAX_CAMS];
    const uint8_t *table;
    const OvUnit *units;
    unsigned long long *S;
    int n_cams, n_frames;
};

constexpr int kGainThreads = 256;
constexpr int kGainVecs = 4;
constexpr int kGainChunk = kGainThreads * kGainVecs * 16;
struct KGainArgs {
    const uint8_t *src;
    uint8_t *dst;
    int64_t bytes, src_fstride, dst_fstride;
    const uint16_t *q_tab;
    uint32_t q;
    int pad_;
};

}
```

### multicamera_stitching_amd/csrc/mcs_launch.cpp

```cpp
#include <algorithm>
#include <cstdlib>

#include "mcs_common.h"
#include "mcs_plan_state.h"

namespace mcs {
namespace host {

void need_mask(const mcs_flat_desc &fd, bool *need)
{
    for (int i = 0; i < MCS_MAX_CAMS; i++) need[i] = false;
    need[0] = true;
    for (int j = 0; j < fd.n_stages; j++) need[fd.st[j].cam] = true;
}

static int g_force_off64 = 0;

bool offset_base(const mcs_plan *p, const mcs::KParams &kp, const uint8_t **base)
{
    bool need[MCS_MAX_CAMS];
    need_mask(p->fd, need);
    uintptr_t lo = UINTPTR_MAX, hi = 0;
    for (int i = 0; i < p->fd.n_cams; i++) {
        if (!need[i]) continue;
        const uintptr_t a = (uintptr_t)kp.cams[i];
        const uintptr_t e = a + (uintptr_t)p->fd.cam_w[i] * p->fd.cam_h[i] * p->fd.channels;
        lo = a < lo ? a : lo;
        hi = e > hi ? e : hi;
    }
    const bool off32 = !g_force_off64 && hi - lo < (uintptr_t(1) << 32);
    *base = off32 ? (const uint8_t *)lo : nullptr;
    return off32;
}

static bool stream_base(const mcs_plan *p, const mcs::KParams &kp, int n_frames,
                        const uint8_t **base)
{
    bool need[MCS_MAX_CAMS];
    need_mask(p->fd, need);
    uintptr_t lo = UINTPTR_MAX, hi = 0;
    const uintptr_t span = (uintptr_t)(n_frames > 0 ? n_frames - 1 : 0) * kp.cam_fstride[0];
    for (int i = 0; i < p->fd.n_cams; i++) {
        if (!need[i]) continue;
        const uintptr_t a = (uintptr_t)kp.cams[i];
        const uintptr_t e = a + span + (uintptr_t)p->fd.cam_w[i] * p->fd.cam_h[i] * p->fd.channels;
        lo = a < lo ? a : lo;
        hi = e > hi ? e : hi;
    }
    const bool b32 = !g_force_off64 && lo <= hi && hi - lo < (uintptr_t(1) << 32);
    *base = b32 ? (const uint8_t *)lo : kp.base;
    return b32;
}

int launch_args(const Api *A, hipFunction_t f, unsigned gx, unsigned gy, unsigned bx,
                unsigned by, void *args, size_t sz, hipStream_t s, unsigned gz, unsigned lds)
{
    void *cfg[] = {HIP_LAUNCH_PARAM_BUFFER_POINTER, args, HIP_LAUNCH_PARAM_BUFFER_SIZE, &sz,
                   HIP_LAUNCH_PARAM_END};
    HIP_TRY(A->hipModuleLaunchKernel(f, gx, gy, gz, bx, by, 1, lds, s, nullptr, cfg));
    return MCS_OK;
}

void mb_args(const mcs_plan *p, const mcs::KParams &P, mcs::KMbArgs &a)
{
    a.P = P;
    a.owner = p->t.d_owner;
    a.list = p->t.d_blist;
    a.desc = p->t.d_mbdesc;
    a.tab = p->t.d_mbtab;
    a.foot = p->t.d_mbfoot;
    a.g1 = p->t.d_mbg1;
    a.g2 = p->t.d_mbg2;
    a.slots = p->t.mb_slots;
    a.chunk = p->t.mb_chunk;
    a.f0 = 0;
    a.nf = 0;
    a.list0 = 0;
    a.n_list = p->t.n_blend;
}

void band_args(const mcs_plan *p, const mcs::KParams &P, mcs::KMbBandArgs &a)
{
    a.P = P;
    a.list = p->t.d_blist;
    a.tile_bt = p->t.d_tile_bt;
    a.bands = p->t.d_bands;
    a.bdesc = p->t.d_bdesc;
    a.bgrp = p->t.d_bgrp;
    a.bdesc16 = p->t.d_bdesc16;
    a.g1 = p->t.d_mbg1;
    a.g2 = p->t.d_mbg2;
    a.slots = p->t.mb_slots;
    a.chunk = p->t.mb_chunk;
    a.f0 = 0;
    a.nf = 0;
    a.gxb = p->t.gxb;
    a.band0 = 0;
    a.n_in = p->t.n_bands_in;
    a.band1 = p->t.n_bands_in;
    a.nb = p->t.n_bands;
}

static unsigned xcd_grid(int64_t n) { return 8u * (unsigned)((n + 7) / 8); }

static int band_form(const mcs_plan *p, const mcs::KParams &P)
{
    bool need[MCS_MAX_CAMS];
    need_mask(p->fd, need);
    const int C = p->fd.channels;
    for (int i = 0; i < p->fd.n_cams; i++) {
        if (!need[i]) continue;
        const int64_t pitch = (int64_t)p->fd.cam_w[i] * C, fb = pitch * p->fd.cam_h[i];
        if (pitch % 4 || fb % 4 || fb < pitch + 12 || P.cam_fstride[i] % 4 ||
            (uintptr_t)P.cams[i] % 4)
            return 0;
    }
    return 1;
}

static int launch_mb_levels(const Api *A, const mcs_plan *p, const Kernels *k, mcs::KMbArgs &m,
                            int f0, int nf, hipStream_t s, bool gained)
{
    m.f0 = f0;
    m.nf = nf;
    if (p->t.n_bands > 0) {
        mcs::KMbBandArgs b;
        band_args(p, m.P, b);
        b.f0 = f0;
        b.nf = nf;
        const unsigned gy = (unsigned)((nf + mcs::kMbBandFrames - 1) / mcs::kMbBandFrames);
        const int form = band_form(p, b.P);
        const int kind = p->t.n_bands_in == 0 ? 1 : (p->t.n_bands > p->t.n_bands_in ? 2 : 0);
        if (kind == 1) b.band0 = 0;
        return launch_args(A, (gained ? k->mb_bands_g : k->mb_bands)[p->fd.channels][form][kind],
                           xcd_grid((int64_t)p->t.n_bands * gy), 1, mcs::kMbBandLanes, 1, &b,
                           sizeof(b), s);
    }
    const unsigned gz = (unsigned)((nf + mcs::kMbLvFrames - 1) / mcs::kMbLvFrames);
    return launch_args(A, (gained ? k->mb_levels_g : k->mb_levels)[p->fd.channels],
                       (unsigned)p->t.n_blend,
                       (unsigned)p->t.mb_slots, mcs::kMbLvThreads, 1, &m, sizeof(m), s, gz);
}

static int launch_dense(const Api *A, const mcs_plan *p, const Kernels *k, const mcs::KParams &P,
                        int n_frames, hipStream_t s, bool gained)
{
    if (p->blend != MCS_BLEND_MULTIBAND || p->t.n_dense <= 0) return MCS_OK;
    mcs::KBlendArgs b;
    b.P = P;
    b.owner = p->t.d_owner;
    b.list = p->t.d_dense;
    b.n_frames = n_frames;
    b.pad_ = 0;
    return launch_args(A, (gained ? k->feather_g : k->feather)[p->fd.channels][p->fd.interp],
                       p->t.n_dense, n_frames, 256, 1, &b, sizeof(b), s);
}

static int launch_mb_blend(const Api *A, const mcs_plan *p, const Kernels *k, mcs::KMbArgs &m,
                           int f0, int nf, hipStream_t s)
{
    m.f0 = f0;
    m.nf = nf;
    const int v = p->t.mb_slots <= 2 ? 0 : (p->t.mb_slots <= 4 ? 1 : 2);
    m.list0 = 0;
    m.n_list = p->t.n_blend;
    return launch_args(A, k->mb_blend[p->fd.channels][v], xcd_grid((int64_t)p->t.n_blend * nf), 1,
                       mcs::kMbBlThreads, 1, &m, sizeof(m), s);
}

static int big_parts(bool multiband)
{
    static const int v = [] {
        const char *e = getenv("MCS_BIG_PARTS");
        const int n = e ? atoi(e) : 0;
        return n >= 1 && n <= 64 ? n : 0;
    }();
    return v ? v : multiband ? 1 : 8;
}

static int launch_pair(const Api *A, const mcs_plan *p, const Kernels *k, mcs::KParams &P,
                       int n_frames, hipStream_t s, bool gained)
{
    const bool sweep = p->blend == MCS_BLEND_MULTIBAND && p->t.n_strips > 0;
    const bool mb = !sweep && p->blend == MCS_BLEND_MULTIBAND && p->t.n_blend > 0;
    const bool aside = p->t.n_fallback > 0 || p->t.n_big > 0;
    const bool fork = aside || mb || sweep;
    mcs::KMbArgs m;
    if (mb) mb_args(p, P, m);
    mcs::KStreamArgs args;
    args.P = P;
    const bool b32 = stream_base(p, P, n_frames, &args.P.base);
    args.tiles = p->t.d_tiles;
    args.desc = p->t.d_desc;
    args.desc4 = p->t.d_desc4;
    args.spans = p->t.d_spans;
    args.n_frames = n_frames;
    args.parts = 1;
    args.pad2_ = 0;
    if (fork) HIP_TRY(A->hipEventRecord(p->ev_fork, s));
    if (aside) HIP_TRY(A->hipStreamWaitEvent(p->side, p->ev_fork, 0));
    auto big_launch = [&](hipStream_t q) -> int {
        mcs::KStreamArgs bg = args;
        bg.order = p->t.d_big + 1;
        bg.n_order = p->t.n_big;
        bg.parts = std::max(1, std::min(big_parts(mb || sweep), n_frames));
        const auto &big = gained ? k->stream_big_g : k->stream_big;
        return launch_args(A, big[p->fd.channels][b32 ? 1 : 0],
                           8u * (((unsigned)(p->t.n_big * bg.parts) + 7u) / 8u), 1, mcs::kWave,
                           mcs::kWavesPerBlock, &bg, sizeof(bg), q, 1,
                           (unsigned)mcs::kBigStreamLds);
    };
    if (p->t.n_big > 0) {
        const int rc = big_launch(p->side);
        if (rc) return rc;
    }
    if (p->t.n_fallback > 0) {
        mcs::KDirectArgs da;
        da.P = P;
        const bool off32 = offset_base(p, da.P, &da.P.base);
        da.fallback = p->t.d_fallback;
        da.n_frames = n_frames;
        da.pad_ = 0;
        const unsigned gy = (unsigned)((n_frames + mcs::kDirectFrames - 1) / mcs::kDirectFrames);
        const int rc = launch_args(
            A, (gained ? k->direct_g : k->direct)[p->fd.channels][p->fd.interp][off32 ? 1 : 0],
            p->t.n_fallback, gy, mcs::kWave, mcs::kWavesPerBlock, &da, sizeof(da), p->side);
        if (rc) return rc;
    }
    if (aside) HIP_TRY(A->hipEventRecord(p->ev_join, p->side));
    const bool split = mb && p->t.d_order && p->t.n_early > 0 && n_frames <= p->t.mb_chunk;
    if (sweep) {
        HIP_TRY(A->hipStreamWaitEvent(p->side2, p->ev_fork, 0));
        mcs::KMbSweepArgs a;
        a.P = P;
        a.strips = p->t.d_strips;
        a.sdesc = p->t.d_sdesc;
        a.region = p->t.d_region;
        a.owner = p->t.d_owner;
        a.n_strips = p->t.n_strips;
        a.f0 = 0;
        a.nf = n_frames;
        a.pad_ = 0;
        const int al = band_form(p, P);
        int rc = launch_args(A, k->mb_sweep[p->fd.channels][al][p->t.sw_jb == 4 ? 1 : 0],
                             xcd_grid((int64_t)p->t.n_strips * n_frames), 1,
                             (unsigned)(mcs::kSwCols * p->t.sw_jb), 1, &a, sizeof(a), p->side2);
        if (rc) return rc;
        HIP_TRY(A->hipEventRecord(p->ev_join2, p->side2));
    }
    if (mb) {
        HIP_TRY(A->hipStreamWaitEvent(p->side2, p->ev_fork, 0));
        int rc = launch_mb_levels(A, p, k, m, 0, std::min(p->t.mb_chunk, n_frames), p->side2,
                                  gained);
// ... 168 lines not shown
```

### multicamera_stitching_amd/csrc/mcs_plan_state.h

```cpp
#pragma once

#include <stdint.h>

#include <algorithm>
#include <vector>

#include "hip_rt.h"
#include "mcs.h"
#include "mcs_kparams.h"
#include "mcs_lens_core.h"

struct mcs_plan {
    struct Tables {
        std::vector<void *> owned;
        bool prepared = false;
        int n_fallback = 0;
        int n_big = 0;
        int *d_big = nullptr;
        mcs::TileHdr *d_tiles = nullptr;
        uint32_t *d_desc = nullptr;
        uint32_t *d_desc4 = nullptr;
        uint16_t *d_spans = nullptr;
        int *d_fallback = nullptr;
        int *d_order = nullptr;
        int n_early = 0;
        int n_list = 0;
        int n_blend = 0, mb_slots = 0;
        int n_dense = 0, n_degraded = 0;
        int *d_dense = nullptr;
        uint8_t *d_owner = nullptr;
        uint32_t *d_binfo = nullptr;
        int *d_blist = nullptr;
        uint64_t *d_mbdesc = nullptr;
        int32_t *d_mbtab = nullptr;
        int32_t *d_mbfoot = nullptr;
        uint16_t *d_mbg1 = nullptr;
        int32_t *d_mbg2 = nullptr;
        int mb_chunk = 0;
        int n_bands = 0, n_bands_in = 0, gxb = 0;
        mcs::MbBand *d_bands = nullptr;
        int *d_tile_bt = nullptr;
        uint64_t *d_bdesc = nullptr;
        uint32_t *d_bgrp = nullptr;
        uint4 *d_bdesc16 = nullptr;
        int n_bands_lds = 0;
        int64_t mb_mixed_px = 0, mb_r1 = 0;
        int n_strips = 0, sw_jb = 0;
        mcs::MbStrip *d_strips = nullptr;
        int *d_region = nullptr;
        uint64_t *d_sdesc = nullptr;
        uint8_t *d_skip = nullptr;
        int64_t sw_px = 0, sw_desc_rows = 0;
        int64_t dma_bytes = 0, box_bytes = 0;

        template <class T>
        hipError_t alloc(const mcs::rt::Api *A, T **ptr, size_t count)
        {
            void *q = nullptr;
            const hipError_t e = A->hipMalloc(&q, count * sizeof(T));
            if (e != hipSuccess) return e;
            owned.push_back(q);
            *ptr = static_cast<T *>(q);
            return hipSuccess;
        }
        template <class T>
        void drop(const mcs::rt::Api *A, T **ptr)
        {
            const auto it = std::find(owned.begin(), owned.end(), static_cast<void *>(*ptr));
            if (it != owned.end()) {
                (void)A->hipFree(*it);
                owned.erase(it);
            }
            *ptr = nullptr;
        }
    };

    mcs_flat_desc fd;
    mcs::KParams kp;
    int device = 0;
    hipStream_t stream = nullptr;
    uint8_t *d_cams[MCS_MAX_CAMS] = {};
    uint8_t *d_out = nullptr;
    int64_t out_pitch = 0;
    Tables t;
    int gx = 0, gy = 0;
    hipStream_t side = nullptr;
    hipEvent_t ev_fork = nullptr, ev_join = nullptr;
    hipStream_t side2 = nullptr;
    hipEvent_t ev_join2 = nullptr;
    hipEvent_t ev_early = nullptr;
    uint8_t *d_raw[MCS_MAX_CAMS] = {};
    size_t raw_bytes[MCS_MAX_CAMS] = {};
    int blend = MCS_BLEND_NONE;
    bool cyl = false;
    std::vector<double> cyl_tab;
    double *d_cyl = nullptr;
    std::vector<uint8_t> seam_lab;
    int seam_w = 0, seam_h = 0, seam_k = 0;
    int64_t seam_stats[5] = {0, 0, 0, 0, 0};
    uint8_t *d_seam = nullptr;
    bool single = false;
    std::vector<int32_t> map_tab;
    int32_t *d_map = nullptr;
    mcs::Lens lens[MCS_MAX_CAMS] = {};
    double *d_lens = nullptr;
    bool lens_stale = false;
    bool gains_on = false;
    uint16_t gain_q[MCS_MAX_CAMS] = {};
    struct Overlap {
        int step = -1;
        uint8_t *d_table = nullptr;
        mcs::OvUnit *d_units = nullptr;
        int n_units = 0;
        int64_t table_bytes = 0;
        int64_t N[MCS_MAX_CAMS * MCS_MAX_CAMS] = {};
        unsigned long long *d_S = nullptr;
        size_t s_bytes = 0;
    } ov;
};

namespace mcs {
namespace host {

using rt::Api;

struct Kernels {
    bool loaded = false;
    hipFunction_t prepare[5][2] = {};
    hipFunction_t stream[5][2] = {};
    hipFunction_t stream_big[5][2] = {};
    hipFunction_t direct[5][2][2] = {};
    hipFunction_t footprint[2] = {};
    hipFunction_t resize[5] = {};
    hipFunction_t blend_owner[2] = {};
    hipFunction_t blend_classify = nullptr;
    hipFunction_t seam_sample[5][2] = {};
    hipFunction_t feather[5][2] = {};
    hipFunction_t mb_prep[5][2] = {};
    hipFunction_t mb_levels[5] = {};
    hipFunction_t mb_blend[5][3] = {};
    hipFunction_t mb_bands[5][2][3] = {};
    hipFunction_t mb_bdesc[5][2] = {};
    hipFunction_t mb_sweep[4][2][2] = {};
    hipFunction_t mb_sweep_desc[4][2] = {};
    hipFunction_t overlap_prep[2] = {};
    hipFunction_t overlap_sum[5] = {};
    hipFunction_t gain_apply = nullptr;
    hipFunction_t stream_g[5][2] = {};
    hipFunction_t stream_big_g[5][2] = {};
    hipFunction_t direct_g[5][2][2] = {};
    hipFunction_t feather_g[5][2] = {};
    hipFunction_t mb_levels_g[5] = {};
    hipFunction_t mb_bands_g[5][2][3] = {};
};

int kernels(const Api *A, int device, const Kernels **out);
int upload_plan_tables(const Api *A, mcs_plan *p, hipStream_t s);
int prepare(const Api *A, mcs_plan *p, hipStream_t s);
void release_tables(const Api *A, mcs_plan *p);

int ensure_stream(const Api *A, mcs_plan *p);
int ensure_host_buffers(const Api *A, mcs_plan *p);

void drop_overlap(const Api *A, mcs_plan *p);
int launch_gain(const Api *A, const Kernels *k, const uint8_t *src, uint8_t *dst, int64_t bytes,
                int64_t src_fstride, int64_t dst_fstride, int n_frames, uint32_t q,
                const uint16_t *d_q, hipStream_t s);

int prepare_sweep(const Api *A, mcs_plan *p, const Kernels *k, hipStream_t s);

int launch_args(const Api *A, hipFunction_t f, unsigned gx, unsigned gy, unsigned bx, unsigned by,
                void *args, size_t sz, hipStream_t s, unsigned gz = 1, unsigned lds = 0);
void need_mask(const mcs_flat_desc &fd, bool *need);
bool offset_base(const mcs_plan *p, const KParams &kp, const uint8_t **base);
void mb_args(const mcs_plan *p, const KParams &P, KMbArgs &a);
void band_args(const mcs_plan *p, const KParams &P, KMbBandArgs &a);
int launch_resize(const Api *A, const Kernels *k, const uint8_t *src, int sw, int sh,
                  int64_t src_pitch, int64_t src_fstride, uint8_t *dst, int dw, int dh,
                  int64_t dst_pitch, int64_t dst_fstride, int C, int n_frames, hipStream_t s);
int launch_stitch(const Api *A, mcs_plan *p, const KParams &kp, int n_frames, hipStream_t s,
                  bool gained = false);
bool gains_active(const mcs_plan *p);
void fill_gain_q(const mcs_plan *p, KParams *kp);

}
}
```

### multicamera_stitching_amd/csrc/mcs_prepare.cpp

```cpp
#include <algorithm>
#include <cstdio>
#include <mutex>
#include <vector>

#include "mcs_common.h"
#include "mcs_plan_state.h"

namespace mcs {
namespace host {

static Kernels g_k[kMaxDevices];
static std::mutex g_k_mu;

int kernels(const Api *A, int device, const Kernels **out)
{
    if (device < 0 || device >= kMaxDevices) return mcs::fail(MCS_E_INVALID, "device %d", device);
    std::lock_guard<std::mutex> lk(g_k_mu);
    Kernels &k = g_k[device];
    if (!k.loaded) {
        auto fn = [&](const char *name, hipFunction_t *f) {
            return mcs::module_function(A, device, mcs::kModStitch, name, f);
        };
        char name[64];
        int rc = MCS_OK;
        for (int c = 1; c <= 4 && rc == MCS_OK; c++) {
            snprintf(name, sizeof(name), "mcs_stream_c%d", c);
            rc = fn(name, &k.stream[c][0]);
            snprintf(name, sizeof(name), "mcs_stream_c%d_b32", c);
            if (rc == MCS_OK) rc = fn(name, &k.stream[c][1]);
            snprintf(name, sizeof(name), "mcs_stream_big_c%d", c);
            if (rc == MCS_OK) rc = fn(name, &k.stream_big[c][0]);
            snprintf(name, sizeof(name), "mcs_stream_big_c%d_b32", c);
            if (rc == MCS_OK) rc = fn(name, &k.stream_big[c][1]);
            for (int b = 0; b < 2; b++) {
                snprintf(name, sizeof(name), "mcs_stream_c%d%s_g", c, b ? "_b32" : "");
                if (rc == MCS_OK) rc = fn(name, &k.stream_g[c][b]);
                snprintf(name, sizeof(name), "mcs_stream_big_c%d%s_g", c, b ? "_b32" : "");
                if (rc == MCS_OK) rc = fn(name, &k.stream_big_g[c][b]);
            }
            snprintf(name, sizeof(name), "mcs_mb_levels_c%d_g", c);
            if (rc == MCS_OK) rc = fn(name, &k.mb_levels_g[c]);
            snprintf(name, sizeof(name), "mcs_resize_c%d", c);
            if (rc == MCS_OK) rc = fn(name, &k.resize[c]);
            snprintf(name, sizeof(name), "mcs_mb_levels_c%d", c);
            if (rc == MCS_OK) rc = fn(name, &k.mb_levels[c]);
            for (int al = 0; al < 2; al++) {
                const char *sfx = al ? "_a" : "";
                snprintf(name, sizeof(name), "mcs_mb_bands%s_c%d", sfx, c);
                if (rc == MCS_OK) rc = fn(name, &k.mb_bands[c][al][0]);
                snprintf(name, sizeof(name), "mcs_mb_bands_br%s_c%d", sfx, c);
                if (rc == MCS_OK) rc = fn(name, &k.mb_bands[c][al][1]);
                snprintf(name, sizeof(name), "mcs_mb_bands_all%s_c%d", sfx, c);
                if (rc == MCS_OK) rc = fn(name, &k.mb_bands[c][al][2]);
                snprintf(name, sizeof(name), "mcs_mb_bands%s_c%d_g", sfx, c);
                if (rc == MCS_OK) rc = fn(name, &k.mb_bands_g[c][al][0]);
                snprintf(name, sizeof(name), "mcs_mb_bands_br%s_c%d_g", sfx, c);
                if (rc == MCS_OK) rc = fn(name, &k.mb_bands_g[c][al][1]);
                snprintf(name, sizeof(name), "mcs_mb_bands_all%s_c%d_g", sfx, c);
                if (rc == MCS_OK) rc = fn(name, &k.mb_bands_g[c][al][2]);
            }
            snprintf(name, sizeof(name), "mcs_mb_blend_c%d_s2", c);
            if (rc == MCS_OK) rc = fn(name, &k.mb_blend[c][0]);
            snprintf(name, sizeof(name), "mcs_mb_blend_c%d_s4", c);
            if (rc == MCS_OK) rc = fn(name, &k.mb_blend[c][1]);
            snprintf(name, sizeof(name), "mcs_mb_blend_c%d_s8", c);
            if (rc == MCS_OK) rc = fn(name, &k.mb_blend[c][2]);
            for (int i = 0; i < 2 && rc == MCS_OK; i++) {
                snprintf(name, sizeof(name), "mcs_prepare_c%d_i%d", c, i);
                rc = fn(name, &k.prepare[c][i]);
                snprintf(name, sizeof(name), "mcs_feather_c%d_i%d", c, i);
                if (rc == MCS_OK) rc = fn(name, &k.feather[c][i]);
                snprintf(name, sizeof(name), "mcs_feather_c%d_i%d_g", c, i);
                if (rc == MCS_OK) rc = fn(name, &k.feather_g[c][i]);
                snprintf(name, sizeof(name), "mcs_mb_prep_c%d_i%d", c, i);
                if (rc == MCS_OK) rc = fn(name, &k.mb_prep[c][i]);
                snprintf(name, sizeof(name), "mcs_mb_bdesc_c%d_i%d", c, i);
                if (rc == MCS_OK) rc = fn(name, &k.mb_bdesc[c][i]);
                snprintf(name, sizeof(name), "mcs_seam_sample_c%d_i%d", c, i);
                if (rc == MCS_OK) rc = fn(name, &k.seam_sample[c][i]);
                for (int o = 0; o < 2 && rc == MCS_OK; o++) {
                    snprintf(name, sizeof(name), "mcs_direct_c%d_i%d_o%d", c, i, o ? 32 : 64);
                    rc = fn(name, &k.direct[c][i][o]);
                    snprintf(name, sizeof(name), "mcs_direct_c%d_i%d_o%d_g", c, i, o ? 32 : 64);
                    if (rc == MCS_OK) rc = fn(name, &k.direct_g[c][i][o]);
                }
            }
        }
        for (int c = 1; c <= 3 && rc == MCS_OK; c++)
            for (int al = 0; al < 2 && rc == MCS_OK; al++) {
                for (int jb = 0; jb < 2 && rc == MCS_OK; jb++) {
                    snprintf(name, sizeof(name), "mcs_mb_sweep%s_c%d_j%d", al ? "_a" : "", c,
                             jb ? 4 : 2);
                    rc = mcs::module_function(A, device, mcs::kModSweep, name,
                                              &k.mb_sweep[c][al][jb]);
                }
                snprintf(name, sizeof(name), "mcs_mb_sweep_desc_c%d_i%d", c, al);
                if (rc == MCS_OK)
                    rc = mcs::module_function(A, device, mcs::kModSweep, name,
                                              &k.mb_sweep_desc[c][al]);
            }
        if (rc == MCS_OK) rc = fn("mcs_footprint_i0", &k.footprint[0]);
        if (rc == MCS_OK) rc = fn("mcs_footprint_i1", &k.footprint[1]);
        if (rc == MCS_OK) rc = fn("mcs_blend_owner_i0", &k.blend_owner[0]);
        if (rc == MCS_OK) rc = fn("mcs_blend_owner_i1", &k.blend_owner[1]);
        if (rc == MCS_OK) rc = fn("mcs_blend_classify", &k.blend_classify);
        if (rc == MCS_OK) rc = fn("mcs_overlap_prep_i0", &k.overlap_prep[0]);
        if (rc == MCS_OK) rc = fn("mcs_overlap_prep_i1", &k.overlap_prep[1]);
        for (int c = 1; c <= 4 && rc == MCS_OK; c++) {
            snprintf(name, sizeof(name), "mcs_overlap_sum_c%d", c);
            rc = fn(name, &k.overlap_sum[c]);
        }
        if (rc == MCS_OK) rc = fn("mcs_gain_apply", &k.gain_apply);
        if (rc) return rc;
        k.loaded = true;
    }
    *out = &k;
    return MCS_OK;
}

static std::vector<int> launch_list(const std::vector<int> &tiles)
{
    const size_t n = tiles.size(), per = (n + 7) / 8;
    std::vector<int> out(8 * per, -1);
    for (size_t i = 0; i < n; i++) out[i] = tiles[i];
    return out;
}

static int band_lds_tables(const Api *A, mcs_plan *p, std::vector<mcs::MbBand> &bands,
                           hipStream_t s)
{
    const size_t nb = bands.size();
    const int C = p->fd.channels, R = mcs::kMbBandRows, DR = mcs::kMbBandDescRows;
    const int L = mcs::kMbBandLanes, NG = mcs::kMbLdsGroups, K = mcs::kMbLdsRows;
    const int SP = mcs::kMbLdsSpan, D4 = mcs::kMbLdsLead / 4;
    p->t.n_bands_lds = 0;
    std::vector<uint64_t> desc(nb * DR * L);
    HIP_TRY(A->hipMemcpyAsync(desc.data(), p->t.d_bdesc, desc.size() * sizeof(uint64_t),
                              hipMemcpyDeviceToHost, s));
    HIP_TRY(A->hipStreamSynchronize(s));
    std::vector<uint32_t> grp(nb * NG * L, 0u);
    const int DL = mcs::kMbLdsDescRows;
    std::vector<uint4> d16(nb * DL * L, make_uint4(0u, 0u, 0u, 0u));
    auto issue = [&](int g) { return g <= D4 ? -mcs::kMbLdsDescRing : 4 * (g - D4 - 1); };
    for (size_t i = 0; i < nb; i++) {
        const int slot = bands[i].slot;
        const int w = slot == 0 ? p->kp.cam0_w : p->kp.st[slot - 1].src_w;
        const int h = slot == 0 ? p->kp.cam0_h : p->kp.st[slot - 1].src_h;
        const int64_t pitch = (int64_t)w * C, fb = pitch * h;
        if (pitch % 4 || pitch < SP) continue;
        uint64_t *d = desc.data() + i * DR * L;
        int y0 = INT32_MAX, y1 = -1;
        bool ok = true;
        for (int e = 0; e < R * L && ok; e++) {
            const uint32_t dx = (uint32_t)d[e], sh = (uint32_t)(d[e] >> 47) & 15u;
            const int64_t oa = dx & 0x7fffffffu;
            const int ya = (int)(oa / pitch), yb = ya + (int)(dx >> 31);
            ok = sh != 15u && yb < h;
            y0 = std::min(y0, ya);
            y1 = std::max(y1, yb);
        }
        if (!ok || y1 - y0 + 1 > 4 * (NG - 2)) continue;
        const int nr = y1 - y0 + 1;
        std::vector<int64_t> lo(nr, INT64_MAX), hi(nr, -1), bs(nr, 0);
        std::vector<int> glo(R, INT32_MAX), ghi(R, -1);
        for (int r = 0; r < R; r++)
            for (int l = 0; l < L; l++) {
                const uint32_t dx = (uint32_t)d[r * L + l];
                const int64_t oa = dx & 0x7fffffffu, cb = oa % pitch;
                const int ya = (int)(oa / pitch) - y0, yb = ya + (int)(dx >> 31);
                for (int y : {ya, yb}) {
                    lo[y] = std::min(lo[y], cb);
                    hi[y] = std::max(hi[y], cb + 2 * C);
                }
                glo[r] = std::min(glo[r], ya / 4);
                ghi[r] = std::max(ghi[r], yb / 4);
            }
        for (int y = 0; y < nr && ok; y++) {
            const int64_t room = fb - (int64_t)(y0 + y) * pitch - SP;
            bs[y] = std::min(hi[y] < 0 ? 0 : lo[y] & ~(int64_t)15, room);
            ok = bs[y] >= 0 && (hi[y] < 0 || hi[y] - bs[y] <= SP);
        }
        if (!ok) continue;
        for (int r = 0; r < R && ok; r++)
            ok = issue(ghi[r]) <= r - mcs::kMbLdsGLead && issue(glo[r] + K / 4) >= r;
        if (!ok) continue;
       
        uint32_t *gt = grp.data() + i * NG * L;
        for (int g = 0; g < NG; g++)
            for (int l = 0; l < L; l++) {
                const int y = 4 * g + l / 16, c = l % 16;
                const bool need = y < nr && hi[y] >= 0 && 16 * c < hi[y] - bs[y];
                gt[g * L + l] = need ? (uint32_t)((int64_t)(y0 + y) * pitch + bs[y] + 16 * c)
                                     : 0xfffffff0u;
            }
        for (int r = 0; r < DR; r++)
            for (int l = 0; l < L; l++) {
                const uint64_t v = d[std::min(r, R - 1) * L + l];
                const uint32_t dx = (uint32_t)v, dy = (uint32_t)(v >> 32);
                const int64_t oa = dx & 0x7fffffffu, cb = oa % pitch;
                const int ya = (int)(oa / pitch) - y0, yb = ya + (int)(dx >> 31);
                const uint32_t wa = (uint32_t)((ya % K) * SP + ((cb & ~(int64_t)3) - bs[ya]));
                const uint32_t wb = (uint32_t)((yb % K) * SP + ((cb & ~(int64_t)3) - bs[yb]));
                const uint32_t ny = (dy & ~(15u << 15)) | ((uint32_t)(cb & 3) << 15);
                d[r * L + l] = (uint64_t)(wa | (wb << 16)) | ((uint64_t)ny << 32);
            }
        for (int r = 0; r < DL; r++)
            for (int l = 0; l < L; l++) {
                const uint64_t v = d[std::min(r, R - 1) * L + l];
                const uint32_t x = (uint32_t)v, meta = (uint32_t)(v >> 32);
                const uint32_t sh = (meta >> 15) & 3u, fx = meta & 63u, fy = (meta >> 6) & 31u;
                const uint32_t ya = (32u - fy) << 6, yb = fy << 6;
                const uint32_t wa = std::min((32u - fx) * ya, 65535u) |
                                    (std::min(fx * ya, 65535u) << 16);
                const uint32_t wb = std::min((32u - fx) * yb, 65535u) |
                                    (std::min(fx * yb, 65535u) << 16);
                const int g = r / 4 + D4 + 1;
                const uint32_t z = (r < R && r % 4 == 0 && g < NG) ? gt[g * L + l] : 0u;
                d16[(i * DL + r) * L + l] = make_uint4(x | (sh << 14), wa, z, wb);
            }
        bands[i].pad_ |= 1;
        p->t.n_bands_lds++;
    }
    if (p->t.n_bands_lds == 0) return MCS_OK;
    HIP_TRY(p->t.alloc(A, &p->t.d_bgrp, grp.size()));
    HIP_TRY(A->hipMemcpyAsync(p->t.d_bgrp, grp.data(), grp.size() * sizeof(uint32_t),
                              hipMemcpyHostToDevice, s));
    HIP_TRY(p->t.alloc(A, &p->t.d_bdesc16, d16.size()));
    HIP_TRY(A->hipMemcpyAsync(p->t.d_bdesc16, d16.data(), d16.size() * sizeof(uint4),
                              hipMemcpyHostToDevice, s));
    HIP_TRY(A->hipMemcpyAsync(p->t.d_bands, bands.data(), nb * sizeof(mcs::MbBand),
                              hipMemcpyHostToDevice, s));
    HIP_TRY(A->hipStreamSynchronize(s));
    return MCS_OK;
}

static int prepare_bands(const Api *A, mcs_plan *p, const Kernels *k, hipStream_t s)
{
    const int n = p->t.n_blend, S = p->t.mb_slots, C = p->fd.channels;
    const int W = p->fd.out_w, H = p->fd.out_h;
    p->t.gxb = (W + mcs::kBlendTileW - 1) / mcs::kBlendTileW;
    const int gyb = (H + mcs::kBlendTileH - 1) / mcs::kBlendTileH;
    const mcs::KParams &P = p->kp;
    for (int c = 0; c <= P.n_stages; c++) {
        if (c == 0 && P.cam0_w == 0) continue;
        const int64_t w = c == 0 ? P.cam0_w : P.st[c - 1].src_w;
        const int64_t h = c == 0 ? P.cam0_h : P.st[c - 1].src_h;
        if ((h - 1) * w * C < 16) return MCS_OK;
    }
    if (W < 128 || H < 128) return MCS_OK;
    std::vector<int> list(1 + 2 * (size_t)n);
    std::vector<int> cnt((size_t)n * mcs::kMbTabCounts);
    const size_t words = (size_t)mcs::mb_tab_words(S);
    const size_t cnt_at = (size_t)S * (mcs::kMbNRX * mcs::kMbNRY + mcs::kMbN2X * mcs::kMbN2Y) +
                          mcs::kMbNRX * mcs::kMbNRY + mcs::kMbN2X * mcs::kMbN2Y;
    HIP_TRY(A->hipMemcpyAsync(list.data(), p->t.d_blist, list.size() * sizeof(int),
                              hipMemcpyDeviceToHost, s));
    HIP_TRY(A->hipMemcpy2DAsync(cnt.data(), mcs::kMbTabCounts * sizeof(int), p->t.d_mbtab + cnt_at,
                                words * sizeof(int), mcs::kMbTabCounts * sizeof(int), (size_t)n,
                                hipMemcpyDeviceToHost, s));
    HIP_TRY(A->hipStreamSynchronize(s));
    struct Need { int q1lo, q1hi, z2lo, z2hi; };
    constexpr int kSlots = 32;
    std::vector<std::vector<Need>> need((size_t)kSlots * gyb);
    std::vector<int> tile_bt((size_t)p->t.gxb * gyb, -1);
    for (int i = 0; i < n; i++) {
        const int t = list[1 + 2 * i];
        const uint32_t mask = (uint32_t)list[2 + 2 * i];
        tile_bt[t] = i;
        const int Y0 = (t / p->t.gxb) * mcs::kBlendTileH;
        const int *c = cnt.data() + (size_t)i * mcs::kMbTabCounts + mcs::kMbTabRanges;
        uint32_t m = mask;
        for (int j = 0; m; j++, m &= m - 1) {
            const int slot = __builtin_ctz(m);
            Need q{c[4 * j], c[4 * j + 1], c[4 * j + 2], c[4 * j + 3]};
            if (q.q1lo > q.q1hi && q.z2lo > q.z2hi) continue;
            need[(size_t)slot * gyb + Y0 / mcs::kBlendTileH].push_back(q);
        }
    }
    p->t.mb_mixed_px = p->t.mb_r1 = 0;
    for (int i = 0; i < n; i++) {
        p->t.mb_mixed_px += cnt[(size_t)i * mcs::kMbTabCounts];
        p->t.mb_r1 += cnt[(size_t)i * mcs::kMbTabCounts + 1];
    }
    std::vector<mcs::MbBand> bands;
    const int big = 1 << 30;
    for (int slot = 0; slot < kSlots; slot++)
        for (int row = 0; row < gyb; row++) {
            std::vector<Need> &v = need[(size_t)slot * gyb + row];
            if (v.empty()) continue;
            auto lo0 = [&](const Need &q) {
                return std::min(q.z2lo <= q.z2hi ? 4 * q.z2lo : big,
                                q.q1lo <= q.q1hi ? 2 * q.q1lo : big);
            };
            std::sort(v.begin(), v.end(), [&](const Need &a, const Need &b) {
                return lo0(a) < lo0(b);
            });
            size_t i = 0;
            while (i < v.size()) {
                Need u = v[i++];
                auto hi0 = [&](const Need &q) {
                    return std::max(q.z2lo <= q.z2hi ? 4 * q.z2hi : -big,
                                    q.q1lo <= q.q1hi ? 2 * q.q1hi : -big);
                };
                while (i < v.size() && lo0(v[i]) <= hi0(u) + 2 * mcs::kMbBandStride) {
                    const Need &q = v[i++];
                    if (q.q1lo <= q.q1hi)
                        u.q1lo = std::min(u.q1lo, q.q1lo), u.q1hi = std::max(u.q1hi, q.q1hi);
                    if (q.z2lo <= q.z2hi)
                        u.z2lo = std::min(u.z2lo, q.z2lo), u.z2hi = std::max(u.z2hi, q.z2hi);
                }
                int c0 = std::min(u.z2lo <= u.z2hi ? 4 * (u.z2lo - 2) : big,
                                  u.q1lo <= u.q1hi ? 2 * (u.q1lo - 1) : big);
                c0 = c0 >= 0 ? c0 & ~3 : -((-c0 + 3) & ~3);
                for (;;) {
                    bands.push_back(mcs::MbBand{slot, row, c0, 0});
                    const bool z_ok = u.z2lo > u.z2hi || c0 / 4 + 14 >= u.z2hi;
                    const bool q_ok = u.q1lo > u.q1hi || c0 / 2 + 30 >= u.q1hi;
                    if (z_ok && q_ok) break;
                    c0 += mcs::kMbBandStride;
                }
            }
        }
    if (bands.empty()) return MCS_OK;
    {
        std::vector<char> early((size_t)p->gx * p->gy, 0);
        for (int i = 0; i < n; i++) {
            if (cnt[(size_t)i * mcs::kMbTabCounts] == 0) continue;
            const int t = list[1 + 2 * i];
            const int X0 = (t % p->t.gxb) * mcs::kBlendTileW;
            const int Y0 = (t / p->t.gxb) * mcs::kBlendTileH;
            const int x1 = std::min(X0 + mcs::kBlendTileW, W) - 1;
            const int y1 = std::min(Y0 + mcs::kBlendTileH, H) - 1;
            for (int ty = Y0 / mcs::kTileH; ty <= y1 / mcs::kTileH; ty++)
                for (int tx = X0 / mcs::kTileW; tx <= x1 / mcs::kTileW; tx++)
                    early[(size_t)ty * p->gx + tx] = 1;
        }
        std::vector<int> first, late;
        for (size_t t = 0; t < early.size(); t++)
            (early[t] ? first : late).push_back((int)t);
        std::vector<int> order = launch_list(first);
        p->t.n_early = (int)order.size();
        const std::vector<int> rest = launch_list(late);
        order.insert(order.end(), rest.begin(), rest.end());
        p->t.n_list = (int)order.size();
        p->t.drop(A, &p->t.d_order);
        HIP_TRY(p->t.alloc(A, &p->t.d_order, order.size()));
        HIP_TRY(A->hipMemcpyAsync(p->t.d_order, order.data(), order.size() * sizeof(int),
                                  hipMemcpyHostToDevice, s));
    }
    auto br = [&](const mcs::MbBand &b) {
        return b.row * mcs::kBlendTileH - mcs::kBlendHalo + mcs::kMbFirst + mcs::kMbUsedY > H ||
               b.c0 + mcs::kMbBandLanes > W;
    };
    std::stable_sort(bands.begin(), bands.end(),
                     [](const mcs::MbBand &a, const mcs::MbBand &b) { return a.row < b.row; });
    std::stable_partition(bands.begin(), bands.end(), [&](const mcs::MbBand &b) { return !br(b); });
    p->t.n_bands_in = (int)(std::find_if(bands.begin(), bands.end(), br) - bands.begin());
    const size_t nb = bands.size();
    HIP_TRY(p->t.alloc(A, &p->t.d_bands, nb));
    HIP_TRY(p->t.alloc(A, &p->t.d_tile_bt, tile_bt.size()));
    HIP_TRY(p->t.alloc(A, &p->t.d_bdesc, nb * mcs::kMbBandDescRows * mcs::kMbBandLanes));
    HIP_TRY(A->hipMemcpyAsync(p->t.d_bands, bands.data(), nb * sizeof(mcs::MbBand),
                              hipMemcpyHostToDevice, s));
    HIP_TRY(A->hipMemcpyAsync(p->t.d_tile_bt, tile_bt.data(), tile_bt.size() * sizeof(int),
                              hipMemcpyHostToDevice, s));
    p->t.n_bands = (int)nb;
    mcs::KMbBandArgs a;
    band_args(p, p->kp, a);
    int rc = launch_args(A, k->mb_bdesc[C][p->fd.interp], (unsigned)nb, 1, 256, 1, &a, sizeof(a),
                         s);
    if (rc) return rc;
    rc = band_lds_tables(A, p, bands, s);
    if (rc) return rc;
    const size_t slots = (size_t)n * S * p->t.mb_chunk;
    HIP_TRY(A->hipMemsetAsync(p->t.d_mbg1, 0, slots * mcs::kMbNRX * mcs::kMbNRY * 8, s));
    HIP_TRY(A->hipMemsetAsync(p->t.d_mbg2, 0, slots * mcs::kMbN2X * mcs::kMbN2Y * C * 4, s));
    HIP_TRY(A->hipStreamSynchronize(s));
    return MCS_OK;
}

static int prepare_multiband(const Api *A, mcs_plan *p, const Kernels *k, hipStream_t s)
{
    const int n = p->t.n_blend, S = p->t.mb_slots, C = p->fd.channels;
    const mcs::KParams &P = p->kp;
    for (int c = 0; c <= P.n_stages; c++) {
        const int64_t w = c == 0 ? P.cam0_w : P.st[c - 1].src_w;
        const int64_t h = c == 0 ? P.cam0_h : P.st[c - 1].src_h;
        if (w * h * C >= (int64_t(1) << 31))
            return mcs::fail(MCS_E_UNSUPPORTED, "multi-band: camera frames must be < 2 GiB");
    }
    const int64_t per_f = (int64_t)n * S * (mcs::kMbNRX * mcs::kMbNRY * 8 +
                                            mcs::kMbN2X * mcs::kMbN2Y * C * 4);
    int chunk = (int)std::max<int64_t>(1, std::min<int64_t>(64, mcs::kMbScratchBytes / per_f));
    if (chunk > mcs::kMbLvFrames) chunk -= chunk % mcs::kMbLvFrames;
    const int64_t samples = (int64_t)mcs::kMbUsedX * mcs::kMbUsedY;
    HIP_TRY(p->t.alloc(A, &p->t.d_mbdesc, (size_t)(n * S * samples)));
    HIP_TRY(p->t.alloc(A, &p->t.d_mbtab, (size_t)n * mcs::mb_tab_words(S)));
    HIP_TRY(p->t.alloc(A, &p->t.d_mbfoot, (size_t)n * S * 8));
    HIP_TRY(p->t.alloc(A, &p->t.d_mbg1, (size_t)n * S * chunk * mcs::kMbNRX * mcs::kMbNRY * 4));
    HIP_TRY(p->t.alloc(A, &p->t.d_mbg2, (size_t)n * S * chunk * mcs::kMbN2X * mcs::kMbN2Y * C));
    p->t.mb_chunk = chunk;
    mcs::KMbArgs a;
    mb_args(p, p->kp, a);
    int rc = launch_args(A, k->mb_prep[C][p->fd.interp], (unsigned)n, 1,
                         mcs::kMbPrepThreads, 1, &a, sizeof(a), s);
    if (rc) return rc;
    rc = prepare_sweep(A, p, k, s);
    if (rc || p->t.n_strips > 0) return rc;
    return prepare_bands(A, p, k, s);
}

static int prepare_blend(const Api *A, mcs_plan *p, const Kernels *k, hipStream_t s)
{
    const int W = p->fd.out_w, H = p->fd.out_h;
    const int bx = (W + mcs::kBlendTileW - 1) / mcs::kBlendTileW;
    const int by = (H + mcs::kBlendTileH - 1) / mcs::kBlendTileH;
    const size_t nt = (size_t)bx * by;
    HIP_TRY(p->t.alloc(A, &p->t.d_owner, (size_t)W * H));
    HIP_TRY(p->t.alloc(A, &p->t.d_binfo, nt * 2));
    HIP_TRY(p->t.alloc(A, &p->t.d_blist, 4 * nt + 4));
    HIP_TRY(A->hipMemsetAsync(p->t.d_blist, 0, (4 * nt + 4) * sizeof(int), s));
    mcs::KBlendPrepArgs a;
    a.P = p->kp;
    a.owner = p->t.d_owner;
    a.info = p->t.d_binfo;
    a.list = p->t.d_blist;
    a.overflow = p->t.d_blist + 2 * nt + 1;
    a.list2 = p->t.d_blist + 2 * nt + 3;
    a.mode = p->blend;
    a.pad_ = 0;
    int rc = launch_args(A, k->blend_owner[p->fd.interp], bx, by, 256, 1, &a, sizeof(a), s);
    if (rc == MCS_OK) rc = launch_args(A, k->blend_classify, (unsigned)nt, 1, 256, 1, &a,
                                       sizeof(a), s);
    if (rc) return rc;
    int n = 0, tail[3] = {0, 0, 0};
    HIP_TRY(A->hipMemcpyAsync(&n, p->t.d_blist, sizeof(int), hipMemcpyDeviceToHost, s));
    HIP_TRY(A->hipMemcpyAsync(tail, p->t.d_blist + 2 * nt + 1, 3 * sizeof(int),
                              hipMemcpyDeviceToHost, s));
    HIP_TRY(A->hipStreamSynchronize(s));
    if (n > 1) {
        std::vector<int> l(1 + 2 * (size_t)n);
        HIP_TRY(A->hipMemcpyAsync(l.data(), p->t.d_blist, l.size() * sizeof(int),
                                  hipMemcpyDeviceToHost, s));
        HIP_TRY(A->hipStreamSynchronize(s));
        std::vector<std::pair<int, int>> e((size_t)n);
        for (int i = 0; i < n; i++) e[i] = {l[1 + 2 * i], l[2 + 2 * i]};
        std::sort(e.begin(), e.end());
        for (int i = 0; i < n; i++) l[1 + 2 * i] = e[i].first, l[2 + 2 * i] = e[i].second;
        HIP_TRY(A->hipMemcpyAsync(p->t.d_blist, l.data(), l.size() * sizeof(int),
                                  hipMemcpyHostToDevice, s));
        HIP_TRY(A->hipStreamSynchronize(s));
    }
    p->t.mb_slots = tail[1];
    p->t.n_degraded = p->blend == MCS_BLEND_MULTIBAND ? tail[0] : 0;
    p->t.n_dense = tail[2];
    p->t.d_dense = p->t.d_blist + 2 * nt + 3;
    p->t.n_blend = n;
    if (p->blend == MCS_BLEND_MULTIBAND && n > 0) return prepare_multiband(A, p, k, s);
    return MCS_OK;
}

void release_tables(const Api *A, mcs_plan *p)
{
    if (p->stream) (void)A->hipStreamSynchronize(p->stream);
    if (p->side) (void)A->hipStreamSynchronize(p->side);
    if (p->side2) (void)A->hipStreamSynchronize(p->side2);
    for (void *q : p->t.owned) (void)A->hipFree(q);
    p->t = mcs_plan::Tables{};
    p->kp.skip = nullptr;
}

int upload_plan_tables(const Api *A, mcs_plan *p, hipStream_t s)
{
    if (p->kp.lens_mask && (!p->d_lens || p->lens_stale)) {
        if (!p->d_lens) HIP_TRY(A->hipMalloc((void **)&p->d_lens, sizeof(p->lens)));
        HIP_TRY(A->hipMemcpyAsync(p->d_lens, p->lens, sizeof(p->lens), hipMemcpyHostToDevice, s));
        HIP_TRY(A->hipStreamSynchronize(s));
        p->lens_stale = false;
        p->kp.lens_tab = p->d_lens;
    }
    if (!p->map_tab.empty() && !p->d_map) {
        const size_t bytes = p->map_tab.size() * sizeof(int32_t);
        HIP_TRY(A->hipMalloc((void **)&p->d_map, bytes));
        HIP_TRY(A->hipMemcpyAsync(p->d_map, p->map_tab.data(), bytes, hipMemcpyHostToDevice, s));
        HIP_TRY(A->hipStreamSynchronize(s));
        p->kp.map_tab = p->d_map;
    }
    if (!p->cyl || p->d_cyl) return MCS_OK;
    const size_t bytes = p->cyl_tab.size() * sizeof(double);
    HIP_TRY(A->hipMalloc((void **)&p->d_cyl, bytes));
    HIP_TRY(A->hipMemcpyAsync(p->d_cyl, p->cyl_tab.data(), bytes, hipMemcpyHostToDevice, s));
    HIP_TRY(A->hipStreamSynchronize(s));
    p->kp.cyl_tab = p->d_cyl;
    return MCS_OK;
}

static int build_tables(const Api *A, mcs_plan *p, hipStream_t s)
{
    const Kernels *k = nullptr;
    int rc = kernels(A, p->device, &k);
    if (rc) return rc;
    p->gx = (p->fd.out_w + mcs::kTileW - 1) / mcs::kTileW;
    p->gy = (p->fd.out_h + mcs::kTileH - 1) / mcs::kTileH;
    const size_t tiles = (size_t)p->gx * p->gy;
    if (tiles == 0) {
        p->t.prepared = true;
        return MCS_OK;
    }
    rc = upload_plan_tables(A, p, s);
    if (rc) return rc;
    if (p->blend == MCS_BLEND_FEATHER || p->blend == MCS_BLEND_MULTIBAND) {
        rc = prepare_blend(A, p, k, s);
        if (rc) return rc;
    }
    HIP_TRY(p->t.alloc(A, &p->t.d_tiles, tiles));
    HIP_TRY(p->t.alloc(A, &p->t.d_desc, tiles * mcs::kTilePx * mcs::kDescWords));
    HIP_TRY(p->t.alloc(A, &p->t.d_desc4, tiles * mcs::kTilePx));
    HIP_TRY(p->t.alloc(A, &p->t.d_spans, tiles * mcs::kMaxTileJobs));
    HIP_TRY(p->t.alloc(A, &p->t.d_fallback, 2 * (tiles + 1)));
    p->t.d_big = p->t.d_fallback + tiles + 1;
    HIP_TRY(A->hipMemsetAsync(p->t.d_fallback, 0, sizeof(int), s));
    HIP_TRY(A->hipMemsetAsync(p->t.d_big, 0, sizeof(int), s));
    mcs::KPrepareArgs args;
    args.P = p->kp;
    args.tiles = p->t.d_tiles;
    args.desc = p->t.d_desc;
    args.desc4 = p->t.d_desc4;
    args.fallback = p->t.d_fallback;
    args.big = p->t.d_big;
// ... 59 lines not shown
```

Baseline: 560,100 MPix/s.

## Store multi-band pyramid levels in band-owned scratch and stack adjacent band rows

Moves the level-1 and level-2 pyramid scratch from per-tile slots into band-owned contiguous buffers. Band kernels now write each lane's output directly at a band offset instead of resolving up to two target tiles through tile lookups, and consumers read through per-tile source descriptors. A new host planner can also merge two adjacent tile rows into one taller band when that needs fewer rows in total, with fallback passes for bands that get refused. This cuts duplicated writes, per-lane lookup work and band count, in exchange for a more complex planner, variable-height descriptor tables and larger prepare time.

```diff
diff --git a/multicamera_stitching_amd/_capi.py b/multicamera_stitching_amd/_capi.py
--- a/multicamera_stitching_amd/_capi.py
+++ b/multicamera_stitching_amd/_capi.py
@@ -556,8 +556,8 @@
         return tiles, spans, desc
 
     def stats(self) -> dict:
-        arr = (ctypes.c_int64 * 21)()
-        check(self._lib.mcs_plan_stats(self._h, arr, 21))
+        arr = (ctypes.c_int64 * 22)()
+        check(self._lib.mcs_plan_stats(self._h, arr, 22))
         return {"prepared": bool(arr[0]), "tiles": arr[1], "lds_tiles": arr[2],
                 "direct_tiles": arr[3], "table_bytes": arr[4], "blend": arr[5],
                 "blend_tiles": arr[6], "mb_owners": arr[7], "mb_degraded_tiles": arr[8],
@@ -566,7 +566,7 @@
                 "dma_bytes_per_capture": arr[14], "box_bytes_per_capture": arr[15],
                 "mb_sweep_strips": arr[16], "mb_sweep_px": arr[17],
                 "mb_sweep_threads": arr[18], "mb_sweep_desc_rows": arr[19],
-                "lens_cams": arr[20]}
+                "lens_cams": arr[20], "mb_band_rows": arr[21]}
 
     def set_blend(self, mode: int):
         check(self._lib.mcs_plan_set_blend(self._h, int(mode)))
diff --git a/multicamera_stitching_amd/build.py b/multicamera_stitching_amd/build.py
--- a/multicamera_stitching_amd/build.py
+++ b/multicamera_stitching_amd/build.py
@@ -23,7 +23,7 @@
 HEADERS = ["mcs_kparams.h", "mcs_dev.h", "mcs_fparams.h", "mcs_common.h", "hip_rt.h", "mcs_blend.h",
            "mcs_gain.h", "mcs_ransac_core.h",
            "mcs_orb_core.h", "mcs_orb_pattern.h", "mcs_feat_int.h", "mcs_lens_core.h",
-           "mcs_plan_state.h"]
+           "mcs_plan_state.h", "mcs_band_plan.h"]
 INC = ["-I" + os.path.join(ROOT, "include"), "-I" + CSRC]
 
 DEVICE_FLAGS = [
diff --git a/multicamera_stitching_amd/csrc/mcs_band_plan.h b/multicamera_stitching_amd/csrc/mcs_band_plan.h
--- /dev/null
+++ b/multicamera_stitching_amd/csrc/mcs_band_plan.h
@@ -0,0 +1,230 @@
+#pragma once
+
+#include <algorithm>
+#include <string>
+#include <utility>
+#include <vector>
+
+#include "mcs_kparams.h"
+
+namespace mcs {
+
+struct MbTileNeed {
+    int tile, slot;
+    int q1lo, q1hi, z2lo, z2hi;
+};
+
+struct MbBandPlan {
+    std::vector<MbBand> bands;
+    int n_in = 0;
+    std::vector<MbTileSrc> src;
+    int64_t g1_bytes = 0, g2_bytes = 0;
+    int64_t rows = 0;
+    int dsc_rows = 0, grp_rows = 0, d16_rows = 0;
+};
+
+namespace band_plan {
+
+constexpr int kBig = 1 << 30;
+struct Need {
+    int q1lo, q1hi, z2lo, z2hi;
+};
+struct Win {
+    int c0, q1lo, q1hi, z2lo, z2hi;
+};
+
+inline std::vector<Win> windows(std::vector<Need> v)
+{
+    std::vector<Win> out;
+    auto lo0 = [](const Need &q) {
+        return std::min(q.z2lo <= q.z2hi ? 4 * q.z2lo : kBig, q.q1lo <= q.q1hi ? 2 * q.q1lo : kBig);
+    };
+    auto hi0 = [](const Need &q) {
+        return std::max(q.z2lo <= q.z2hi ? 4 * q.z2hi : -kBig,
+                        q.q1lo <= q.q1hi ? 2 * q.q1hi : -kBig);
+    };
+    std::stable_sort(v.begin(), v.end(),
+                     [&](const Need &a, const Need &b) { return lo0(a) < lo0(b); });
+    size_t i = 0;
+    while (i < v.size()) {
+        Need u = v[i++];
+        while (i < v.size() && lo0(v[i]) <= hi0(u) + 2 * kMbBandStride) {
+            const Need &q = v[i++];
+            if (q.q1lo <= q.q1hi) {
+                const bool e = u.q1lo > u.q1hi;
+                u.q1lo = e ? q.q1lo : std::min(u.q1lo, q.q1lo);
+                u.q1hi = e ? q.q1hi : std::max(u.q1hi, q.q1hi);
+            }
+            if (q.z2lo <= q.z2hi) {
+                const bool e = u.z2lo > u.z2hi;
+                u.z2lo = e ? q.z2lo : std::min(u.z2lo, q.z2lo);
+                u.z2hi = e ? q.z2hi : std::max(u.z2hi, q.z2hi);
+            }
+        }
+        int c0 = std::min(u.z2lo <= u.z2hi ? 4 * (u.z2lo - 2) : kBig,
+                          u.q1lo <= u.q1hi ? 2 * (u.q1lo - 1) : kBig);
+        c0 = c0 >= 0 ? c0 & ~3 : -((-c0 + 3) & ~3);
+        for (;;) {
+            const bool z_ok = u.z2lo > u.z2hi || c0 / 4 + 14 >= u.z2hi;
+            const bool q_ok = u.q1lo > u.q1hi || c0 / 2 + 30 >= u.q1hi;
+            const bool last = z_ok && q_ok;
+            Win w;
+            w.c0 = c0;
+            w.q1lo = std::max(u.q1lo, c0 / 2 + 1);
+            w.q1hi = std::min(u.q1hi, last ? c0 / 2 + kMbBandN1X : (c0 + kMbBandStride) / 2);
+            w.z2lo = std::max(u.z2lo, c0 / 4 + 2);
+            w.z2hi = std::min(u.z2hi, c0 / 4 + 1 + kMbBandN2X);
+            out.push_back(w);
+            if (last) break;
+            c0 += kMbBandStride;
+        }
+    }
+    return out;
+}
+
+inline int used_rows(int rows) { return rows == kMbBandRows ? kMbUsedY : kMbUsedY + kBlendTileH; }
+inline int first_row(int row) { return row * kBlendTileH - kBlendHalo + kMbFirst; }
+inline bool is_br(const MbBand &b, int W, int H)
+{
+    return first_row(b.row) + used_rows(b.rows) > H || b.c0 + kMbBandLanes > W;
+}
+
+}
+
+inline int mb_plan_bands(int W, int H, int CN, int chunk, bool stack,
+                         const std::vector<MbTileNeed> &needs,
+                         const std::vector<std::pair<int, int>> &single, MbBandPlan &out,
+                         std::string &err)
+{
+    using namespace band_plan;
+    out = MbBandPlan();
+    const int gxb = (W + kBlendTileW - 1) / kBlendTileW, gyb = (H + kBlendTileH - 1) / kBlendTileH;
+    constexpr int kSlots = 32;
+    std::vector<std::vector<Need>> need((size_t)kSlots * gyb);
+    for (const MbTileNeed &t : needs) {
+        if (t.slot < 0 || t.slot >= kSlots || t.tile < 0 || t.tile >= gxb * gyb) {
+            err = "band plan: tile or slot out of range";
+            return -1;
+        }
+        if (t.q1lo > t.q1hi && t.z2lo > t.z2hi) continue;
+        need[(size_t)t.slot * gyb + t.tile / gxb].push_back(Need{t.q1lo, t.q1hi, t.z2lo, t.z2hi});
+    }
+    auto add = [&](int slot, int row, int rows, const std::vector<Win> &ws) {
+        for (const Win &w : ws) {
+            MbBand b = {};
+            b.slot = slot, b.row = row, b.c0 = w.c0, b.rows = rows;
+            const int tr = rows == kMbBandRows ? 1 : 2;
+            b.n1 = kMbNRY + (tr - 1) * (kBlendTileH / 2);
+            b.n2 = kMbN2Y + (tr - 1) * (kBlendTileH / 4);
+            b.q1lo = w.q1lo, b.q1hi = w.q1hi, b.z2lo = w.z2lo, b.z2hi = w.z2hi;
+            out.bands.push_back(b);
+        }
+    };
+    for (int slot = 0; slot < kSlots; slot++)
+        for (int row = 0; row < gyb; row++) {
+            const std::vector<Need> &v = need[(size_t)slot * gyb + row];
+            if (v.empty()) continue;
+            const std::vector<Win> w0 = windows(v);
+            bool pair = stack && row >= 1 && row + 2 < gyb &&
+                        first_row(row) + kMbUsedY + kBlendTileH <= H &&
+                        !need[(size_t)slot * gyb + row + 1].empty() &&
+                        std::find(single.begin(), single.end(), std::make_pair(slot, row)) ==
+                            single.end();
+            if (pair) {
+                const std::vector<Need> &v1 = need[(size_t)slot * gyb + row + 1];
+                std::vector<Need> u = v;
+                u.insert(u.end(), v1.begin(), v1.end());
+                const std::vector<Win> wu = windows(u);
+                for (const Win &w : wu) pair = pair && w.c0 + kMbBandLanes <= W;
+                pair = pair && wu.size() * kMbBandRows2 <
+                                   (w0.size() + windows(v1).size()) * kMbBandRows;
+                if (pair) {
+                    add(slot, row, kMbBandRows2, wu);
+                    row++;
+                    continue;
+                }
+            }
+            add(slot, row, kMbBandRows, w0);
+        }
+    std::stable_sort(out.bands.begin(), out.bands.end(),
+                     [](const MbBand &a, const MbBand &b) { return a.row < b.row; });
+    std::stable_partition(out.bands.begin(), out.bands.end(),
+                          [&](const MbBand &b) { return !is_br(b, W, H); });
+    int64_t o1 = 0, o2 = 0, dsc = 0, grp = 0, d16 = 0;
+    for (MbBand &b : out.bands) {
+        if (!is_br(b, W, H)) out.n_in++;
+        b.o1 = (uint32_t)o1, b.o2 = (uint32_t)o2;
+        b.dsc = (int)dsc, b.grp = (int)grp, b.d16 = (int)d16;
+        o1 += (int64_t)chunk * b.n1 * kMbBandN1X * 8;
+        o2 += (int64_t)chunk * b.n2 * kMbBandN2X * CN * 4;
+        dsc += b.rows + kMbBandDescRing;
+        grp += mb_lds_groups(b.rows);
+        d16 += b.rows + kMbLdsDescRing;
+        out.rows += b.rows;
+        if (o1 >= (int64_t(1) << 31) || o2 >= (int64_t(1) << 31) ||
+            d16 * kMbBandLanes >= (int64_t(1) << 31)) {
+            err = "band plan: level scratch or descriptor tables past 2 GiB";
+            return -1;
+        }
+    }
+    out.g1_bytes = o1, out.g2_bytes = o2;
+    out.dsc_rows = (int)dsc, out.grp_rows = (int)grp, out.d16_rows = (int)d16;
+    out.src.assign(needs.size(), MbTileSrc());
+    for (size_t i = 0; i < needs.size(); i++) {
+        const MbTileNeed &t = needs[i];
+        const int row = t.tile / gxb, tx = t.tile % gxb;
+        MbTileSrc &s = out.src[i];
+        for (int lv = 1; lv <= 2; lv++) {
+            const int X = lv == 1 ? tx * (kBlendTileW / 2) - kMbOR : tx * (kBlendTileW / 4) - kMbO2;
+            const int N = lv == 1 ? kMbNRX : kMbN2X;
+            int *off = lv == 1 ? s.off1 : s.off2, *cs = lv == 1 ? s.cs1 : s.cs2;
+            int *lo = lv == 1 ? s.lo1 : s.lo2, *hi = lv == 1 ? s.hi1 : s.hi2;
+            int n = 0;
+            for (int k = 0; k < 2; k++) off[k] = cs[k] = 0, lo[k] = kBig, hi[k] = -1;
+            std::vector<const MbBand *> hit;
+            for (const MbBand &b : out.bands) {
+                const bool rows2 = b.rows != kMbBandRows;
+                if (b.slot != t.slot || (b.row != row && !(rows2 && b.row + 1 == row))) continue;
+                const int blo = lv == 1 ? b.q1lo : b.z2lo, bhi = lv == 1 ? b.q1hi : b.z2hi;
+                if (blo > bhi || bhi < X || blo > X + N - 1) continue;
+                hit.push_back(&b);
+            }
+            std::sort(hit.begin(), hit.end(), [&](const MbBand *a, const MbBand *b) {
+                return (lv == 1 ? a->q1lo : a->z2lo) < (lv == 1 ? b->q1lo : b->z2lo);
+            });
+            if (hit.size() > 2) {
+                err = "band plan: a tile's arrays lie in more than two bands";
+                return -1;
+            }
+            for (const MbBand *b : hit) {
+                const int blo = lv == 1 ? b->q1lo : b->z2lo, bhi = lv == 1 ? b->q1hi : b->z2hi;
+                const int ro = row - b->row;
+                if (lv == 1) {
+                    cs[n] = b->n1 * kMbBandN1X;
+                    off[n] = (int)(b->o1 / 8) + ro * (kBlendTileH / 2) * kMbBandN1X +
+                             (X - (b->c0 / 2 + 1));
+                } else {
+                    cs[n] = b->n2 * kMbBandN2X;
+                    off[n] = (int)(b->o2 / (4 * CN)) + ro * (kBlendTileH / 4) * kMbBandN2X +
+                             (X - (b->c0 / 4 + 2));
+                }
+                lo[n] = std::max(0, blo - X);
+                hi[n] = std::min(N - 1, bhi - X);
+                n++;
+            }
+            const int nlo = lv == 1 ? t.q1lo : t.z2lo, nhi = lv == 1 ? t.q1hi : t.z2hi;
+            for (int c = nlo; c <= nhi; c++) {
+                const int x = c - X;
+                const bool ok = x >= 0 && x < N &&
+                                ((x >= lo[0] && x <= hi[0]) || (x >= lo[1] && x <= hi[1]));
+                if (!ok) {
+                    err = "band plan: a needed column lies in no band of its tile";
+                    return -1;
+                }
+            }
+        }
+    }
+    return 0;
+}
+
+}
diff --git a/multicamera_stitching_amd/csrc/mcs_blend.h b/multicamera_stitching_amd/csrc/mcs_blend.h
--- a/multicamera_stitching_amd/csrc/mcs_blend.h
+++ b/multicamera_stitching_amd/csrc/mcs_blend.h
@@ -249,7 +249,6 @@
     }
 }
 
-constexpr int kMbO1 = 6, kMbO2 = 2, kMbOR = 1;
 constexpr int kMbU = kMbUsedX * kMbUsedY;
 constexpr int kMbFoot = 28672;
 constexpr int kMbFootBufs = 1;
@@ -1004,8 +1003,8 @@
     int cam, w, h;
     slot_info(P, B.slot, cam, w, h);
     const int y0 = B.row * kBlendTileH - kBlendHalo + kMbFirst;
-    uint64_t *o = a.bdesc + (int64_t)blockIdx.x * kMbBandDescRows * kMbBandLanes;
-    for (int i = threadIdx.x; i < kMbBandDescRows * kMbBandLanes; i += blockDim.x) {
+    uint64_t *o = a.bdesc + (int64_t)B.dsc * kMbBandLanes;
+    for (int i = threadIdx.x; i < (B.rows + kMbBandDescRing) * kMbBandLanes; i += blockDim.x) {
         const int r = i / kMbBandLanes, l = i % kMbBandLanes;
         const int x = refl(B.c0 + l, P.out_w), y = refl(y0 + r, P.out_h);
         const uint2 v = mb_desc<CN>(mb_src<INTERP>(P, B.slot, x, y), w, h);
@@ -1056,26 +1055,6 @@
 #pragma unroll
         for (int k = 0; k < CN; k++) ((gi *)p)[k] = v[k];
     }
-}
-
-struct MbTarget {
-    int base[2], col[2];
-};
-static_assert(kBlendTileW == 32, "mb_bands: tile columns are found by shifts");
-
-__device__ __forceinline__ void mb_target(const KMbBandArgs &a, int s, int row, int tx, int col,
-                                          MbTarget &T, int k)
-{
-    T.base[k] = -1;
-    T.col[k] = 0;
-    if (tx < 0 || tx >= a.gxb) return;
-    const int bt = a.tile_bt[row * a.gxb + tx];
-    if (bt < 0) return;
-    const uint32_t mask = (uint32_t)a.list[2 + 2 * bt];
-    if (!((mask >> s) & 1u)) return;
-    const int j = __popc(mask & ((1u << s) - 1u));
-    T.base[k] = (bt * a.slots + j) * a.chunk;
-    T.col[k] = col;
 }
 
 __device__ __forceinline__ bool xcd_unit(int nx, int ny, int &x, int &y)
@@ -1113,7 +1092,7 @@
 template <int FR>
 constexpr int mb_lds_ops(int ph)
 {
-    return ((ph & 1) ? 2 * FR : 0) + (ph % 4 == 1 ? 2 * FR : 0) + (ph % 4 == 0 ? FR : 0) + 1;
+    return ((ph & 1) ? FR : 0) + (ph % 4 == 1 ? FR : 0) + (ph % 4 == 0 ? FR : 0) + 1;
 }
 template <int FR, int NL>
 constexpr int mb_lds_wait(int ph, bool first)
@@ -1162,22 +1141,13 @@
     const int W = P.out_w, H = P.out_h;
     const int w1 = (W + 1) / 2, h1 = (H + 1) / 2, w2 = (w1 + 1) / 2, h2 = (h1 + 1) / 2;
     const int Y0 = B.row * kBlendTileH, Y1 = Y0 / 2 - kMbO1, Y2 = Y0 / 4 - kMbO2;
+    const int rows = __builtin_amdgcn_readfirstlane(B.rows);
+    const int n1 = __builtin_amdgcn_readfirstlane(B.n1), n2 = __builtin_amdgcn_readfirstlane(B.n2);
     const int x = B.c0 + l;
-    MbTarget T1, T2;
-    T1.base[0] = T1.base[1] = T2.base[0] = T2.base[1] = -1;
-    T1.col[0] = T1.col[1] = T2.col[0] = T2.col[1] = 0;
-    if ((l & 1) == 0 && l >= 2 && l <= 61 && x >= 0 && (x >> 1) < w1) {
-        const int qx = x >> 1, tx = (qx + kMbOR) >> 4;
-        mb_target(a, B.slot, B.row, tx, qx - (tx * (kBlendTileW / 2) - kMbOR), T1, 0);
-        if (((qx + kMbOR) & 15) < kMbNRX - 16)
-            mb_target(a, B.slot, B.row, tx - 1, qx - ((tx - 1) * (kBlendTileW / 2) - kMbOR), T1, 1);
-    }
-    if ((l & 3) == 0 && l >= 8 && l <= 56 && x >= 0 && (x >> 2) < w2) {
-        const int z = x >> 2, tx = (z + kMbO2) >> 3;
-        mb_target(a, B.slot, B.row, tx, z - (tx * (kBlendTileW / 4) - kMbO2), T2, 0);
-        if (((z + kMbO2) & 7) < kMbN2X - 8)
-            mb_target(a, B.slot, B.row, tx - 1, z - ((tx - 1) * (kBlendTileW / 4) - kMbO2), T2, 1);
-    }
+    const bool t1 = (l & 1) == 0 && l >= 2 && l <= 60 && x >= 0 && (x >> 1) < w1 &&
+                    (x >> 1) >= B.q1lo && (x >> 1) <= B.q1hi;
+    const bool t2 = (l & 3) == 0 && l >= 8 && l <= 56 && x >= 0 && (x >> 2) < w2 &&
+                    (x >> 2) >= B.z2lo && (x >> 2) <= B.z2hi;
     int src[4];
 #pragma unroll
     for (int t = 0; t < 4; t++) {
@@ -1185,17 +1155,13 @@
         if (BR && q >= w1) q = 2 * w1 - 2 - q;
         src[t] = min(max(2 * q - B.c0, 0), kMbBandLanes - 1) * 4;
     }
-    uint32_t o1[2], o2[2];
-#pragma unroll
-    for (int k = 0; k < 2; k++) {
-        o1[k] = T1.base[k] < 0 ? 0u : (uint32_t)((T1.base[k] + fl0) * (kMbNRX * kMbNRY) +
-                                                 mb_g1_at(T1.col[k], 0)) * 8u;
-        o2[k] = T2.base[k] < 0 ? 0u : (uint32_t)((T2.base[k] + fl0) * (kMbN2X * kMbN2Y * CN) +
-                                                 mb_g2_at<CN>(T2.col[k], 0, 0)) * 4u;
-    }
+    constexpr uint32_t r1b = kMbBandN1X * 8u, r2b = kMbBandN2X * CN * 4u;
+    const uint32_t c1b = (uint32_t)n1 * r1b, c2b = (uint32_t)n2 * r2b;
+    const uint32_t o1 = t1 ? B.o1 + (uint32_t)fl0 * c1b + (uint32_t)((l >> 1) - 1) * 8u : 0u;
+    const uint32_t o2 = t2 ? B.o2 + (uint32_t)fl0 * c2b + (uint32_t)((l >> 2) - 2) * (CN * 4u) : 0u;
     typedef __attribute__((address_space(1))) uint8_t g8;
     g8 *const g1b = (g8 *)a.g1, *const g2b = (g8 *)a.g2;
-    const uint64_t *dsc = a.bdesc + (int64_t)bi * kMbBandDescRows * kMbBandLanes + l;
+    const uint64_t *dsc = a.bdesc + (int64_t)B.dsc * kMbBandLanes + l;
     const int nst = min(FR, a.nf - fl0);
     uint32_t Vl[FR][3], Vh[FR][3];
     int V2[FR][3][CN];
@@ -1243,26 +1209,18 @@
         if constexpr (ph & 1) {
 #pragma unroll
             for (int f = 0; f < FR; f++) {
-                const uint32_t ro =
-                    (uint32_t)(f * (kMbNRX * kMbNRY) + mb_g1_at(0, pend1 - kMbRS)) * 8u;
+                const uint32_t ro = (uint32_t)f * c1b + (uint32_t)(pend1 - kMbRS) * r1b;
                 typedef unsigned int u2v __attribute__((ext_vector_type(2)));
                 const u2v v = {p1l[f], p1h[f]};
-#pragma unroll
-                for (int k = 0; k < 2; k++)
-                    __builtin_amdgcn_raw_buffer_store_b64(
-                        v, rs1, (ok1 && f < nst && T1.base[k] >= 0) ? o1[k] + ro : none, 0, 0);
+                __builtin_amdgcn_raw_buffer_store_b64(v, rs1, (ok1 && f < nst && t1) ? o1 + ro : none,
+                                                      0, 0);
             }
         }
         if constexpr (ph % 4 == 1) {
 #pragma unroll
             for (int f = 0; f < FR; f++) {
-                const uint32_t ro =
-                    (uint32_t)(f * (kMbN2X * kMbN2Y * CN) + mb_g2_at<CN>(0, pend2, 0)) * 4u;
-#pragma unroll
-                for (int q = 0; q < 2; q++) {
-                    const uint32_t off = (ok2 && f < nst && T2.base[q] >= 0) ? o2[q] + ro : none;
-                    mb_buffer_store_ch<CN>(rs2, off, p2[f]);
-                }
+                const uint32_t ro = (uint32_t)f * c2b + (uint32_t)pend2 * r2b;
+                mb_buffer_store_ch<CN>(rs2, (ok2 && f < nst && t2) ? o2 + ro : none, p2[f]);
             }
         }
     };
@@ -1271,11 +1229,8 @@
 #pragma unroll
             for (int f = 0; f < FR; f++) {
                 if (f >= nst) break;
-                const uint32_t ro =
-                    (uint32_t)(f * (kMbNRX * kMbNRY) + mb_g1_at(0, pend1 - kMbRS)) * 8u;
-#pragma unroll
-                for (int k = 0; k < 2; k++)
-                    if (T1.base[k] >= 0) *(g2u *)(g1b + (o1[k] + ro)) = make_uint2(p1l[f], p1h[f]);
+                const uint32_t ro = (uint32_t)f * c1b + (uint32_t)(pend1 - kMbRS) * r1b;
+                if (t1) *(g2u *)(g1b + (o1 + ro)) = make_uint2(p1l[f], p1h[f]);
             }
             pend1 = -1;
         }
@@ -1283,11 +1238,8 @@
 #pragma unroll
             for (int f = 0; f < FR; f++) {
                 if (f >= nst) break;
-                const uint32_t ro =
-                    (uint32_t)(f * (kMbN2X * kMbN2Y * CN) + mb_g2_at<CN>(0, pend2, 0)) * 4u;
-#pragma unroll
-                for (int q = 0; q < 2; q++)
-                    if (T2.base[q] >= 0) mb_store_ch<CN>(g2b + (o2[q] + ro), p2[f]);
+                const uint32_t ro = (uint32_t)f * c2b + (uint32_t)pend2 * r2b;
+                if (t2) mb_store_ch<CN>(g2b + (o2 + ro), p2[f]);
             }
             pend2 = -1;
         }
@@ -1303,10 +1255,10 @@
         const int qy = Y1 + i;
         if constexpr (LD) {
             pend1 = i;
-            ok1 = qy >= 0 && qy < h1 && i >= kMbRS && i < kMbRS + kMbNRY;
+            ok1 = qy >= 0 && qy < h1 && i >= kMbRS && i < kMbRS + n1;
             p1l[f] = gl;
             p1h[f] = gh;
-        } else if (qy >= 0 && qy < h1 && i >= kMbRS && i < kMbRS + kMbNRY) {
+        } else if (qy >= 0 && qy < h1 && i >= kMbRS && i < kMbRS + n1) {
             pend1 = i;
             p1l[f] = gl;
             p1h[f] = gh;
@@ -1331,9 +1283,9 @@
             const int e = (i >> 1) - 2, zy = Y2 + e;
             if (LD) {
                 pend2 = e;
-                ok2 = e >= 0 && e < kMbN2Y && zy < h2;
-            }
-            if (LD || (e >= 0 && e < kMbN2Y && zy < h2)) {
+                ok2 = e >= 0 && e < n2 && zy < h2;
+            }
+            if (LD || (e >= 0 && e < n2 && zy < h2)) {
                 pend2 = e;
 #pragma unroll
                 for (int k = 0; k < CN; k++) {
@@ -1358,11 +1310,11 @@
     constexpr int NB = kMbBandBufs, A = kMbBandAhead, ND = kMbBandDescRing;
     uint64_t dq[ND];
     Win wq0[NB][FR], wq1[NB][FR];
-    const uint32_t *grp = a.bgrp + (int64_t)bi * kMbLdsGroups * kMbBandLanes + l;
+    const uint32_t *grp = a.bgrp + (int64_t)B.grp * kMbBandLanes + l;
     typedef __attribute__((address_space(3))) const uint32_t lu32;
     lds_u8 *const dring = ring + kMbLdsDescOff;
     constexpr int NL = kMbLdsDescRing;
-    const uint4 *d16 = a.bdesc16 + (int64_t)bi * kMbLdsDescRows * kMbBandLanes + l;
+    const uint4 *d16 = a.bdesc16 + (int64_t)B.d16 * kMbBandLanes + l;
     auto issue_desc = [&](int row) {
         __builtin_amdgcn_global_load_lds(d16 + row * kMbBandLanes,
                                          dring + (row % NL) * kMbBandLanes * 16, 16, 0, 0);
@@ -1395,7 +1347,7 @@
     }
 #pragma unroll
     for (int i = 0; i < A; i++) load_win(dq[i], wq0[i], wq1[i]);
-    for (int r12 = 0; r12 < kMbBandRows; r12 += 12) {
+    for (int r12 = 0; r12 < rows; r12 += 12) {
         static_for<12>([&](auto PHc) {
             constexpr int ph = decltype(PHc)::value;
             const int r = r12 + ph;
@@ -1698,6 +1650,31 @@
 #pragma unroll
     for (int j = 0; j < S; j++) {
         if (j >= ns) break;
+        if (a.src) {
+            const MbTileSrc T = a.src[bt * a.slots + j];
+            const cgu2 *s1 = (const cgu2 *)a.g1;
+            const cgi32 *s2 = (const cgi32 *)a.g2;
+#pragma unroll
+            for (int q = 0; q < N1; q++) {
+                const int e = min(tid + q * kMbBlThreads, kMbNRX * kMbNRY - 1);
+                const int ey = div_small<kMbNRX>(e), ex = e - ey * kMbNRX;
+                const int k = ex >= T.lo1[1] ? 1 : 0;
+                const int at = T.off1[k] + fl * T.cs1[k] + ey * kMbBandN1X + ex;
+                r1[j][q] = make_uint2(0u, 0u);
+                if (ex >= T.lo1[k] && ex <= T.hi1[k]) r1[j][q] = s1[at];
+            }
+#pragma unroll
+            for (int q = 0; q < N2; q++) {
+                const int e = min(tid + q * kMbBlThreads, kMbN2X * kMbN2Y * CN - 1);
+                const int en = e / CN, ch = e - en * CN;
+                const int ey = div_small<kMbN2X>(en), ex = en - ey * kMbN2X;
+                const int k = ex >= T.lo2[1] ? 1 : 0;
+                const int at = (T.off2[k] + fl * T.cs2[k] + ey * kMbBandN2X + ex) * CN + ch;
+                r2[j][q] = 0;
+                if (ex >= T.lo2[k] && ex <= T.hi2[k]) r2[j][q] = s2[at];
+            }
+            continue;
+        }
         const int64_t job = ((int64_t)bt * a.slots + j) * a.chunk + fl;
         const cgu2 *s1 = (const cgu2 *)a.g1 + job * (kMbNRX * kMbNRY);
         const cgi32 *s2 = (const cgi32 *)a.g2 + job * (kMbN2X * kMbN2Y * CN);
diff --git a/multicamera_stitching_amd/csrc/mcs_capi.cpp b/multicamera_stitching_amd/csrc/mcs_capi.cpp
--- a/multicamera_stitching_amd/csrc/mcs_capi.cpp
+++ b/multicamera_stitching_amd/csrc/mcs_capi.cpp
@@ -855,14 +855,15 @@
     const int64_t tiles = (int64_t)p->gx * p->gy;
     int lens_cams = 0;
     for (int c = 0; c < MCS_MAX_CAMS; c++) lens_cams += (p->kp.lens_mask >> c) & 1u;
-    const int64_t v[21] = {p->t.prepared ? 1 : 0, tiles, tiles - p->t.n_fallback, p->t.n_fallback,
+    const int64_t v[22] = {p->t.prepared ? 1 : 0, tiles, tiles - p->t.n_fallback, p->t.n_fallback,
                            tiles * (int64_t)(sizeof(mcs::TileHdr) +
                                              mcs::kTilePx * (mcs::kDescWords + 1) * 4),
                            p->blend, p->t.n_blend, p->t.mb_slots, p->t.n_degraded, p->t.n_bands,
                            p->t.n_bands_lds, p->t.n_big, p->t.mb_mixed_px, p->t.mb_r1,
                            p->t.dma_bytes, p->t.box_bytes, p->t.n_strips, p->t.sw_px,
-                           (int64_t)mcs::kSwCols * p->t.sw_jb, p->t.sw_desc_rows, lens_cams};
-    for (int i = 0; i < n; i++) stats[i] = i < 21 ? v[i] : 0;
+                           (int64_t)mcs::kSwCols * p->t.sw_jb, p->t.sw_desc_rows, lens_cams,
+                           p->t.mb_band_rows};
+    for (int i = 0; i < n; i++) stats[i] = i < 22 ? v[i] : 0;
     return MCS_OK;
 }
 
diff --git a/multicamera_stitching_amd/csrc/mcs_kparams.h b/multicamera_stitching_amd/csrc/mcs_kparams.h
--- a/multicamera_stitching_amd/csrc/mcs_kparams.h
+++ b/multicamera_stitching_amd/csrc/mcs_kparams.h
@@ -151,6 +151,7 @@
 constexpr int kMbN2X = kBlendTileW / 4 + 4, kMbN2Y = kBlendTileH / 4 + 4;
 constexpr int kMbNRX = kBlendTileW / 2 + 2, kMbNRY = kBlendTileH / 2 + 2;
 constexpr int kMbTilePx = kBlendTileW * kBlendTileH;
+constexpr int kMbO1 = 6, kMbO2 = 2, kMbOR = 1;
 constexpr int kMbTabRanges = 8;
 constexpr int kMbTabCounts = kMbTabRanges + 4 * kBlendSlots;
 constexpr int kMbTabLists = kMbTabCounts + kMbTilePx / 2 + (kMbNRX * kMbNRY + 1) / 2;
@@ -168,6 +169,11 @@
     int *list2;
     int mode, pad_;
 };
+struct MbTileSrc {
+    int off1[2], cs1[2], lo1[2], hi1[2];
+    int off2[2], cs2[2], lo2[2], hi2[2];
+};
+static_assert(sizeof(MbTileSrc) == 64, "MbTileSrc layout");
 struct KMbArgs {
     KParams P;
     const uint8_t *owner;
@@ -182,13 +188,23 @@
     int f0, nf;
     int list0;
     int n_list;
+    const MbTileSrc *src;
 };
 
 struct MbBand {
-    int slot, row, c0, pad_;
-};
+    int slot, row, c0;
+    int pad_;
+    int rows;
+    int n1, n2;
+    int q1lo, q1hi, z2lo, z2hi;
+    uint32_t o1, o2;
+    int dsc, grp, d16;
+};
+static_assert(sizeof(MbBand) == 64, "MbBand layout");
 constexpr int kMbBandLanes = 64;
+constexpr int kMbBandN1X = 30, kMbBandN2X = 13;
 constexpr int kMbBandRows = (kMbUsedY + 11) / 12 * 12;
+constexpr int kMbBandRows2 = (kMbUsedY + kBlendTileH + 11) / 12 * 12;
 #ifndef MCS_MB_BAND_AHEAD
 #define MCS_MB_BAND_AHEAD 2
 #endif
@@ -201,7 +217,6 @@
 constexpr int kMbBandDescRing = MCS_MB_DESC_RING;
 static_assert(12 % kMbBandDescRing == 0 && kMbBandDescRing >= kMbBandBufs,
               "band pass: descriptor ring must divide the 12-row body and hold the window rows");
-constexpr int kMbBandDescRows = kMbBandRows + kMbBandDescRing;
 constexpr int kMbBandStride = 52;
 #ifndef MCS_MB_BAND_FRAMES
 #define MCS_MB_BAND_FRAMES 2
@@ -228,30 +243,27 @@
 constexpr int kMbLdsRingBytes = kMbLdsRows * kMbLdsSpan;
 static_assert(kMbLdsRingBytes <= (1 << 14), "LDS band ring: offsets must fit the 14-bit field");
 constexpr int kMbLdsDescRing = MCS_MB_LDS_DESC;
-constexpr int kMbLdsDescRows = kMbBandRows + kMbLdsDescRing;
 constexpr int kMbLdsDescOff = kMbBandFrames * kMbLdsRingBytes;
 constexpr int kMbLdsBytes = kMbLdsDescOff + kMbLdsDescRing * kMbBandLanes * 16 + 16;
 static_assert(12 % kMbLdsDescRing == 0 && kMbLdsGLead >= 1 && kMbLdsGLead <= kMbLdsDescRing,
               "LDS band ring: descriptor ring divides the 12-row body; groups led by <= its rows");
-constexpr int kMbLdsGroups = kMbBandRows / 4 + kMbLdsLead / 4 + 3;
+constexpr int mb_lds_groups(int rows) { return rows / 4 + kMbLdsLead / 4 + 3; }
 static_assert(kMbLdsRows % 4 == 0 && kMbLdsLead % 4 == 0 && kMbLdsRows / 4 > kMbLdsLead / 4 + 1,
               "LDS band ring: whole groups, the prologue's groups never evicted by the loop's first");
 struct KMbBandArgs {
     KParams P;
-    const int *list;
-    const int *tile_bt;
     const MbBand *bands;
     uint64_t *bdesc;
     uint16_t *g1;
     int32_t *g2;
     const uint32_t *bgrp;
     const uint4 *bdesc16;
-    int slots, chunk, f0, nf;
-    int gxb;
+    int chunk, f0, nf;
     int band0;
     int n_in;
     int band1;
     int nb;
+    int pad_;
 };
 struct KBlendArgs {
     KParams P;
diff --git a/multicamera_stitching_amd/csrc/mcs_launch.cpp b/multicamera_stitching_amd/csrc/mcs_launch.cpp
--- a/multicamera_stitching_amd/csrc/mcs_launch.cpp
+++ b/multicamera_stitching_amd/csrc/mcs_launch.cpp
@@ -77,28 +77,26 @@
     a.nf = 0;
     a.list0 = 0;
     a.n_list = p->t.n_blend;
+    a.src = p->t.d_mbsrc;
 }
 
 void band_args(const mcs_plan *p, const mcs::KParams &P, mcs::KMbBandArgs &a)
 {
     a.P = P;
-    a.list = p->t.d_blist;
-    a.tile_bt = p->t.d_tile_bt;
     a.bands = p->t.d_bands;
     a.bdesc = p->t.d_bdesc;
     a.bgrp = p->t.d_bgrp;
     a.bdesc16 = p->t.d_bdesc16;
     a.g1 = p->t.d_mbg1;
     a.g2 = p->t.d_mbg2;
-    a.slots = p->t.mb_slots;
     a.chunk = p->t.mb_chunk;
     a.f0 = 0;
     a.nf = 0;
-    a.gxb = p->t.gxb;
     a.band0 = 0;
     a.n_in = p->t.n_bands_in;
     a.band1 = p->t.n_bands_in;
     a.nb = p->t.n_bands;
+    a.pad_ = 0;
 }
 
 static unsigned xcd_grid(int64_t n) { return 8u * (unsigned)((n + 7) / 8); }
diff --git a/multicamera_stitching_amd/csrc/mcs_plan_state.h b/multicamera_stitching_amd/csrc/mcs_plan_state.h
--- a/multicamera_stitching_amd/csrc/mcs_plan_state.h
+++ b/multicamera_stitching_amd/csrc/mcs_plan_state.h
@@ -39,6 +39,8 @@
         int mb_chunk = 0;
         int n_bands = 0, n_bands_in = 0, gxb = 0;
         mcs::MbBand *d_bands = nullptr;
+        mcs::MbTileSrc *d_mbsrc = nullptr;
+        int64_t mb_band_rows = 0;
         int *d_tile_bt = nullptr;
         uint64_t *d_bdesc = nullptr;
         uint32_t *d_bgrp = nullptr;
diff --git a/multicamera_stitching_amd/csrc/mcs_prepare.cpp b/multicamera_stitching_amd/csrc/mcs_prepare.cpp
--- a/multicamera_stitching_amd/csrc/mcs_prepare.cpp
+++ b/multicamera_stitching_amd/csrc/mcs_prepare.cpp
@@ -1,10 +1,13 @@
 #include <algorithm>
 #include <cstdio>
 #include <mutex>
+#include <string>
+#include <utility>
 #include <vector>
 
 #include "mcs_common.h"
 #include "mcs_plan_state.h"
+#include "mcs_band_plan.h"
 
 namespace mcs {
 namespace host {
@@ -126,29 +129,30 @@
     return out;
 }
 
-static int band_lds_tables(const Api *A, mcs_plan *p, std::vector<mcs::MbBand> &bands,
-                           hipStream_t s)
-{
+static int band_lds_tables(const Api *A, mcs_plan *p, mcs::MbBandPlan &bp, hipStream_t s)
+{
+    std::vector<mcs::MbBand> &bands = bp.bands;
     const size_t nb = bands.size();
-    const int C = p->fd.channels, R = mcs::kMbBandRows, DR = mcs::kMbBandDescRows;
-    const int L = mcs::kMbBandLanes, NG = mcs::kMbLdsGroups, K = mcs::kMbLdsRows;
+    const int C = p->fd.channels;
+    const int L = mcs::kMbBandLanes, K = mcs::kMbLdsRows;
     const int SP = mcs::kMbLdsSpan, D4 = mcs::kMbLdsLead / 4;
     p->t.n_bands_lds = 0;
-    std::vector<uint64_t> desc(nb * DR * L);
+    std::vector<uint64_t> desc((size_t)bp.dsc_rows * L);
     HIP_TRY(A->hipMemcpyAsync(desc.data(), p->t.d_bdesc, desc.size() * sizeof(uint64_t),
                               hipMemcpyDeviceToHost, s));
     HIP_TRY(A->hipStreamSynchronize(s));
-    std::vector<uint32_t> grp(nb * NG * L, 0u);
-    const int DL = mcs::kMbLdsDescRows;
-    std::vector<uint4> d16(nb * DL * L, make_uint4(0u, 0u, 0u, 0u));
+    std::vector<uint32_t> grp((size_t)bp.grp_rows * L, 0u);
+    std::vector<uint4> d16((size_t)bp.d16_rows * L, make_uint4(0u, 0u, 0u, 0u));
     auto issue = [&](int g) { return g <= D4 ? -mcs::kMbLdsDescRing : 4 * (g - D4 - 1); };
     for (size_t i = 0; i < nb; i++) {
         const int slot = bands[i].slot;
+        const int R = bands[i].rows;
+        const int DL = R + mcs::kMbLdsDescRing, NG = mcs::mb_lds_groups(R);
         const int w = slot == 0 ? p->kp.cam0_w : p->kp.st[slot - 1].src_w;
         const int h = slot == 0 ? p->kp.cam0_h : p->kp.st[slot - 1].src_h;
         const int64_t pitch = (int64_t)w * C, fb = pitch * h;
         if (pitch % 4 || pitch < SP) continue;
-        uint64_t *d = desc.data() + i * DR * L;
+        uint64_t *d = desc.data() + (size_t)bands[i].dsc * L;
         int y0 = INT32_MAX, y1 = -1;
         bool ok = true;
         for (int e = 0; e < R * L && ok; e++) {
@@ -185,7 +189,7 @@
             ok = issue(ghi[r]) <= r - mcs::kMbLdsGLead && issue(glo[r] + K / 4) >= r;
         if (!ok) continue;
        
-        uint32_t *gt = grp.data() + i * NG * L;
+        uint32_t *gt = grp.data() + (size_t)bands[i].grp * L;
         for (int g = 0; g < NG; g++)
             for (int l = 0; l < L; l++) {
                 const int y = 4 * g + l / 16, c = l % 16;
@@ -193,9 +197,9 @@
                 gt[g * L + l] = need ? (uint32_t)((int64_t)(y0 + y) * pitch + bs[y] + 16 * c)
                                      : 0xfffffff0u;
             }
-        for (int r = 0; r < DR; r++)
+        for (int r = 0; r < R; r++)
             for (int l = 0; l < L; l++) {
-                const uint64_t v = d[std::min(r, R - 1) * L + l];
+                const uint64_t v = d[r * L + l];
                 const uint32_t dx = (uint32_t)v, dy = (uint32_t)(v >> 32);
                 const int64_t oa = dx & 0x7fffffffu, cb = oa % pitch;
                 const int ya = (int)(oa / pitch) - y0, yb = ya + (int)(dx >> 31);
@@ -216,7 +220,7 @@
                                     (std::min(fx * yb, 65535u) << 16);
                 const int g = r / 4 + D4 + 1;
                 const uint32_t z = (r < R && r % 4 == 0 && g < NG) ? gt[g * L + l] : 0u;
-                d16[(i * DL + r) * L + l] = make_uint4(x | (sh << 14), wa, z, wb);
+                d16[((size_t)bands[i].d16 + r) * L + l] = make_uint4(x | (sh << 14), wa, z, wb);
             }
         bands[i].pad_ |= 1;
         p->t.n_bands_lds++;
@@ -232,6 +236,12 @@
                               hipMemcpyHostToDevice, s));
     HIP_TRY(A->hipStreamSynchronize(s));
     return MCS_OK;
+}
+
+static bool band_stacking()
+{
+    const char *e = getenv("MCS_MB_STACK");
+    return !(e && e[0] == '0');
 }
 
 static int prepare_bands(const Api *A, mcs_plan *p, const Kernels *k, hipStream_t s)
@@ -259,22 +269,16 @@
                                 words * sizeof(int), mcs::kMbTabCounts * sizeof(int), (size_t)n,
                                 hipMemcpyDeviceToHost, s));
     HIP_TRY(A->hipStreamSynchronize(s));
-    struct Need { int q1lo, q1hi, z2lo, z2hi; };
-    constexpr int kSlots = 32;
-    std::vector<std::vector<Need>> need((size_t)kSlots * gyb);
-    std::vector<int> tile_bt((size_t)p->t.gxb * gyb, -1);
+    std::vector<mcs::MbTileNeed> needs;
+    std::vector<int> need_at;
     for (int i = 0; i < n; i++) {
         const int t = list[1 + 2 * i];
-        const uint32_t mask = (uint32_t)list[2 + 2 * i];
-        tile_bt[t] = i;
-        const int Y0 = (t / p->t.gxb) * mcs::kBlendTileH;
         const int *c = cnt.data() + (size_t)i * mcs::kMbTabCounts + mcs::kMbTabRanges;
-        uint32_t m = mask;
-        for (int j = 0; m; j++, m &= m - 1) {
-            const int slot = __builtin_ctz(m);
-            Need q{c[4 * j], c[4 * j + 1], c[4 * j + 2], c[4 * j + 3]};
-            if (q.q1lo > q.q1hi && q.z2lo > q.z2hi) continue;
-            need[(size_t)slot * gyb + Y0 / mcs::kBlendTileH].push_back(q);
+        uint32_t m = (uint32_t)list[2 + 2 * i];
+        for (int j = 0; m && j < S; j++, m &= m - 1) {
+            needs.push_back(mcs::MbTileNeed{t, __builtin_ctz(m), c[4 * j], c[4 * j + 1],
+                                            c[4 * j + 2], c[4 * j + 3]});
+            need_at.push_back(i * S + j);
         }
     }
     p->t.mb_mixed_px = p->t.mb_r1 = 0;
@@ -282,46 +286,19 @@
         p->t.mb_mixed_px += cnt[(size_t)i * mcs::kMbTabCounts];
         p->t.mb_r1 += cnt[(size_t)i * mcs::kMbTabCounts + 1];
     }
-    std::vector<mcs::MbBand> bands;
-    const int big = 1 << 30;
-    for (int slot = 0; slot < kSlots; slot++)
-        for (int row = 0; row < gyb; row++) {
-            std::vector<Need> &v = need[(size_t)slot * gyb + row];
-            if (v.empty()) continue;
-            auto lo0 = [&](const Need &q) {
-                return std::min(q.z2lo <= q.z2hi ? 4 * q.z2lo : big,
-                                q.q1lo <= q.q1hi ? 2 * q.q1lo : big);
-            };
-            std::sort(v.begin(), v.end(), [&](const Need &a, const Need &b) {
-                return lo0(a) < lo0(b);
-            });
-            size_t i = 0;
-            while (i < v.size()) {
-                Need u = v[i++];
-                auto hi0 = [&](const Need &q) {
-                    return std::max(q.z2lo <= q.z2hi ? 4 * q.z2hi : -big,
-                                    q.q1lo <= q.q1hi ? 2 * q.q1hi : -big);
-                };
-                while (i < v.size() && lo0(v[i]) <= hi0(u) + 2 * mcs::kMbBandStride) {
-                    const Need &q = v[i++];
-                    if (q.q1lo <= q.q1hi)
-                        u.q1lo = std::min(u.q1lo, q.q1lo), u.q1hi = std::max(u.q1hi, q.q1hi);
-                    if (q.z2lo <= q.z2hi)
-                        u.z2lo = std::min(u.z2lo, q.z2lo), u.z2hi = std::max(u.z2hi, q.z2hi);
-                }
-                int c0 = std::min(u.z2lo <= u.z2hi ? 4 * (u.z2lo - 2) : big,
-                                  u.q1lo <= u.q1hi ? 2 * (u.q1lo - 1) : big);
-                c0 = c0 >= 0 ? c0 & ~3 : -((-c0 + 3) & ~3);
-                for (;;) {
-                    bands.push_back(mcs::MbBand{slot, row, c0, 0});
-                    const bool z_ok = u.z2lo > u.z2hi || c0 / 4 + 14 >= u.z2hi;
-                    const bool q_ok = u.q1lo > u.q1hi || c0 / 2 + 30 >= u.q1hi;
-                    if (z_ok && q_ok) break;
-                    c0 += mcs::kMbBandStride;
-                }
-            }
-        }
-    if (bands.empty()) return MCS_OK;
+    const bool stack = band_stacking();
+    mcs::MbBandPlan bp;
+    std::string err;
+    std::vector<std::pair<int, int>> single;
+    if (mcs::mb_plan_bands(W, H, C, p->t.mb_chunk, stack, needs, single, bp, err))
+        return mcs::fail(MCS_E_UNSUPPORTED, "%s", err.c_str());
+    if (bp.bands.empty()) return MCS_OK;
+    if (bp.g1_bytes + bp.g2_bytes > mcs::kMbScratchBytes) {
+        const int64_t per_f = (bp.g1_bytes + bp.g2_bytes) / p->t.mb_chunk;
+        int chunk = (int)std::max<int64_t>(1, mcs::kMbScratchBytes / per_f);
+        if (chunk > mcs::kMbLvFrames) chunk -= chunk % mcs::kMbLvFrames;
+        p->t.mb_chunk = chunk;
+    }
     {
         std::vector<char> early((size_t)p->gx * p->gy, 0);
         for (int i = 0; i < n; i++) {
@@ -348,33 +325,59 @@
         HIP_TRY(A->hipMemcpyAsync(p->t.d_order, order.data(), order.size() * sizeof(int),
                                   hipMemcpyHostToDevice, s));
     }
-    auto br = [&](const mcs::MbBand &b) {
-        return b.row * mcs::kBlendTileH - mcs::kBlendHalo + mcs::kMbFirst + mcs::kMbUsedY > H ||
-               b.c0 + mcs::kMbBandLanes > W;
+    auto build = [&]() -> int {
+        p->t.drop(A, &p->t.d_bands);
+        p->t.drop(A, &p->t.d_bdesc);
+        p->t.drop(A, &p->t.d_bgrp);
+        p->t.drop(A, &p->t.d_bdesc16);
+        if (mcs::mb_plan_bands(W, H, C, p->t.mb_chunk, stack, needs, single, bp, err))
+            return mcs::fail(MCS_E_UNSUPPORTED, "%s", err.c_str());
+        const size_t nb = bp.bands.size();
+        HIP_TRY(p->t.alloc(A, &p->t.d_bands, nb));
+        HIP_TRY(p->t.alloc(A, &p->t.d_bdesc, (size_t)bp.dsc_rows * mcs::kMbBandLanes));
+        HIP_TRY(A->hipMemcpyAsync(p->t.d_bands, bp.bands.data(), nb * sizeof(mcs::MbBand),
+                                  hipMemcpyHostToDevice, s));
+        p->t.n_bands = (int)nb;
+        p->t.n_bands_in = bp.n_in;
+        p->t.mb_band_rows = bp.rows;
+        mcs::KMbBandArgs a;
+        band_args(p, p->kp, a);
+        const int rc = launch_args(A, k->mb_bdesc[C][p->fd.interp], (unsigned)nb, 1, 256, 1, &a,
+                                   sizeof(a), s);
+        return rc ? rc : band_lds_tables(A, p, bp, s);
     };
-    std::stable_sort(bands.begin(), bands.end(),
-                     [](const mcs::MbBand &a, const mcs::MbBand &b) { return a.row < b.row; });
-    std::stable_partition(bands.begin(), bands.end(), [&](const mcs::MbBand &b) { return !br(b); });
-    p->t.n_bands_in = (int)(std::find_if(bands.begin(), bands.end(), br) - bands.begin());
-    const size_t nb = bands.size();
-    HIP_TRY(p->t.alloc(A, &p->t.d_bands, nb));
-    HIP_TRY(p->t.alloc(A, &p->t.d_tile_bt, tile_bt.size()));
-    HIP_TRY(p->t.alloc(A, &p->t.d_bdesc, nb * mcs::kMbBandDescRows * mcs::kMbBandLanes));
-    HIP_TRY(A->hipMemcpyAsync(p->t.d_bands, bands.data(), nb * sizeof(mcs::MbBand),
+    int rc = build();
+    if (rc) return rc;
+    std::vector<std::pair<int, int>> refused;
+    for (const mcs::MbBand &b : bp.bands)
+        if (b.rows != mcs::kMbBandRows && !(b.pad_ & 1)) refused.push_back({b.slot, b.row});
+    if (!refused.empty()) {
+        for (int slot = 0; slot < 32; slot++)
+            for (int row = 0; row < gyb; row++) single.push_back({slot, row});
+        rc = build();
+        if (rc) return rc;
+        auto ring = [&](int slot, int row) {
+            for (const mcs::MbBand &b : bp.bands)
+                if (b.slot == slot && b.row == row && !(b.pad_ & 1)) return false;
+            return true;
+        };
+        single.clear();
+        for (const auto &q : refused)
+            if (ring(q.first, q.second) && ring(q.first, q.second + 1)) single.push_back(q);
+        rc = build();
+        if (rc) return rc;
+    }
+    std::vector<mcs::MbTileSrc> src((size_t)n * S);
+    for (size_t i = 0; i < needs.size(); i++) src[need_at[i]] = bp.src[i];
+    HIP_TRY(p->t.alloc(A, &p->t.d_mbsrc, src.size()));
+    HIP_TRY(A->hipMemcpyAsync(p->t.d_mbsrc, src.data(), src.size() * sizeof(mcs::MbTileSrc),
                               hipMemcpyHostToDevice, s));
-    HIP_TRY(A->hipMemcpyAsync(p->t.d_tile_bt, tile_bt.data(), tile_bt.size() * sizeof(int),
-                              hipMemcpyHostToDevice, s));
-    p->t.n_bands = (int)nb;
-    mcs::KMbBandArgs a;
-    band_args(p, p->kp, a);
-    int rc = launch_args(A, k->mb_bdesc[C][p->fd.interp], (unsigned)nb, 1, 256, 1, &a, sizeof(a),
-                         s);
-    if (rc) return rc;
-    rc = band_lds_tables(A, p, bands, s);
-    if (rc) return rc;
-    const size_t slots = (size_t)n * S * p->t.mb_chunk;
-    HIP_TRY(A->hipMemsetAsync(p->t.d_mbg1, 0, slots * mcs::kMbNRX * mcs::kMbNRY * 8, s));
-    HIP_TRY(A->hipMemsetAsync(p->t.d_mbg2, 0, slots * mcs::kMbN2X * mcs::kMbN2Y * C * 4, s));
+    p->t.drop(A, &p->t.d_mbg1);
+    p->t.drop(A, &p->t.d_mbg2);
+    HIP_TRY(p->t.alloc(A, &p->t.d_mbg1, (size_t)bp.g1_bytes / sizeof(uint16_t)));
+    HIP_TRY(p->t.alloc(A, &p->t.d_mbg2, (size_t)bp.g2_bytes / sizeof(int32_t)));
+    HIP_TRY(A->hipMemsetAsync(p->t.d_mbg1, 0, (size_t)bp.g1_bytes, s));
+    HIP_TRY(A->hipMemsetAsync(p->t.d_mbg2, 0, (size_t)bp.g2_bytes, s));
     HIP_TRY(A->hipStreamSynchronize(s));
     return MCS_OK;
 }
```

After: 570,700 MPix/s (median of 2 runs). Within noise of the previous version (+1.9%).
